# XiaokunSun/SemanticHuman

Measured on AMD Instinct MI355X. Metric: training meshes/sec at 6890 verts, batch=64, higher is better.
Workload: dtype f32

## Files before the change

### include/sh_kernels.h

```cpp
#ifndef SH_KERNELS_H
#define SH_KERNELS_H

#include <stddef.h>
#include <stdint.h>

#ifdef __cplusplus
extern "C" {
#endif

typedef void* sh_stream_t;

#if defined(__GNUC__)
#define SH_API __attribute__((visibility("default")))
#else
#define SH_API
#endif

enum sh_status {
    SH_OK = 0,
    SH_ERR_INVALID_ARG = -1,
    SH_ERR_UNSUPPORTED = -2,
    SH_ERR_WORKSPACE = -3,
    SH_ERR_LAUNCH = -4
};

enum sh_act {
    SH_ACT_IDENTITY = 0,
    SH_ACT_RELU = 1,
    SH_ACT_ELU = 2,
    SH_ACT_LEAKY_RELU = 3,
    SH_ACT_SIGMOID = 4,
    SH_ACT_TANH = 5
};

SH_API int sh_version(void);
SH_API const char* sh_last_error(void);
SH_API const char* sh_build_id(void);

enum sh_mma_mode { SH_MMA_EXACT = 0, SH_MMA_SPLIT3 = 1, SH_MMA_PLANES3 = 2 };

SH_API int sh_clock_probe(unsigned long long* out, int n_workgroups, int iters, sh_stream_t stream);
SH_API int sh_profile_enable(int on);
SH_API int sh_profile_count(void);
SH_API int sh_profile_get(int i, char* name, int name_len, float* ms);

SH_API int sh_spiral_conv_fwd(const float* x, int64_t x_sv, int64_t x_sb,
                       const int32_t* table, const float* weight, const float* bias,
                       float* y, int64_t y_sv, int64_t y_sb,
                       int B, int R, int S, int Cin, int Cout, int act, int zero_row, int mma_mode,
                       sh_stream_t stream);

SH_API int sh_spiral_conv_bwd_data(const float* dpre, int64_t dp_sv, int64_t dp_sb,
                            const int32_t* table_t, const float* weight_t,
                            float* dx, int64_t dx_sv, int64_t dx_sb,
                            const float* yprev, int64_t yp_sv, int64_t yp_sb, int act_prev, int zero_row,
                            int B, int n_in, int S, int Cin, int Cout, int mma_mode,
                            sh_stream_t stream);
SH_API int sh_spiral_conv_bwd_data_z(const float* dpre, int64_t dp_sv, int64_t dp_sb, int dpre_zero_row, const int32_t* table_t,
                                     const float* weight_t, float* dx, int64_t dx_sv, int64_t dx_sb, const float* yprev,
                                     int64_t yp_sv, int64_t yp_sb, int act_prev, int zero_row, int B, int n_in, int S, int Cin,
                                     int Cout, int mma_mode, sh_stream_t stream);

SH_API int sh_weight_transpose(const float* weight, float* weight_t, int S, int Cin, int Cout, sh_stream_t stream);

SH_API size_t sh_spiral_conv_bwd_wgt_workspace(int B, int R, int S, int Cin, int Cout);
SH_API int sh_spiral_conv_bwd_wgt(const float* dpre, int64_t dp_sv, int64_t dp_sb,
                           const float* x, int64_t x_sv, int64_t x_sb, const int32_t* table,
                           float* dW, float* dbias, void* workspace, size_t workspace_bytes,
                           int B, int R, int S, int Cin, int Cout, int mma_mode,
                           sh_stream_t stream);

SH_API int sh_spiral_conv_bwd_wgt_presum(const float* dpre, int64_t dp_sv, int64_t dp_sb, const float* x, int64_t x_sv, int64_t x_sb,
                                         const int32_t* table, float* dW, float* dbias, void* workspace, size_t workspace_bytes,
                                         const int32_t* sum_rowptr, const int32_t* sum_col, const float* sum_val, float* sum_out,
                                         void* sum_out_planes, int sum_rows, int B, int R, int S, int Cin, int Cout, int mma_mode,
                                         sh_stream_t stream);

SH_API int sh_spiral_conv_bwd_wgt_reduce_multi(int n_layers, const void* const* workspaces, float* const* dW,
                                        float* const* dbias, const int* B, const int* R, const int* S,
                                        const int* Cin, const int* Cout, sh_stream_t stream);
SH_API int sh_weight_transpose_multi(int n_layers, const float* const* weight, float* const* weight_t,
                              const int* S, const int* Cin, const int* Cout, sh_stream_t stream);

SH_API int sh_act_backward(const float* dy, int64_t dy_sv, int64_t dy_sb,
                    const float* y, int64_t y_sv, int64_t y_sb,
                    float* dpre, int64_t dp_sv, int64_t dp_sb,
                    int B, int R, int C, int act, int zero_row, sh_stream_t stream);
SH_API int sh_act_backward_tr(const float* dy, int64_t dy_sv, int64_t dy_sb, const float* y, int64_t y_sv, int64_t y_sb,
                       float* dpre, int64_t dp_sv, int64_t dp_sb, int B, int R, int C, int act, int zero_row, int n_layers,
                       const float* const* weight, float* const* weight_t, const int* S, const int* Cin, const int* Cout,
                       sh_stream_t stream);

SH_API int sh_spmm(const int32_t* rowptr, const int32_t* col, const float* val,
            const float* x, int64_t x_sv, int64_t x_sb,
            float* y, int64_t y_sv, int64_t y_sb,
            const float* yprev, int64_t yp_sv, int64_t yp_sb, int act_prev, int zero_row,
            int B, int rows, int C, sh_stream_t stream);

typedef struct sh_csr_ref { const int32_t* rowptr; const int32_t* col; const float* val; } sh_csr_ref;
typedef struct sh_stack_step {
    int kind;
    int param;
    const int32_t* table;
    const int32_t* table_t;
    int R, S, n_in, cin, cout, act, zero_row;
    int n1, n2;
    sh_csr_ref sum1, sum2;
    sh_csr_ref m, mt;
    int m_rows, m_cols;
    int extend;
    const int32_t* rag_rows;
    const int32_t* rag_pos;
    int rag_L;
    const int32_t* fg_rows; const uint32_t* fg_pos; const int32_t* fg_out; int fg_n, fg_L;
    const int32_t* bg_rows; const uint32_t* bg_pos; const int32_t* bg_out; int bg_n, bg_L;
} sh_stack_step;

enum sh_stack_form {
    SH_FORM_FWD_P3 = 1,
    SH_FORM_FWD_GRP = 2,
    SH_FORM_FWD_IMG = 4,
    SH_FORM_FWD_IMG_ONLY = 8,
    SH_FORM_BWD_GIMG = 16,
    SH_FORM_BWD_THIN = 32,
    SH_FORM_BWD_P3 = 64,
    SH_FORM_BWD_RAG = 128,
    SH_FORM_BWD_GRP = 256,
    SH_FORM_BWD_RIDE = 512,
    SH_FORM_BWD_PRESUM_IMG = 1024,
    SH_FORM_BWD_P3W = 2048,
    SH_FORM_BWD_YIMG = 4096,
    SH_FORM_BWD_IN_IMG_ONLY = 8192,
    SH_FORM_BWD_GRAD_IMG_ONLY = 16384
};
SH_API int sh_stack_plan_f32(int n_steps, const sh_stack_step* steps, int c0, int B, int x_layout, int mma_mode, int keep_fp32,
                             int need_x_grad, int* forms);

SH_API int sh_stack_forward(int n_steps, const sh_stack_step* steps, const float* x, int x_layout, int rows0, int c0, int B,
                            const float* const* weights, const float* const* biases, float* const* outs, int out_layout,
                            int mma_mode, void* const* planes, const void* const* wfrag3, int keep_fp32, sh_stream_t stream);

SH_API int sh_stack_backward(int n_steps, const sh_stack_step* steps, const float* x, int x_layout, int rows0, int c0, int B,
                             const float* const* acts, const float* g, int out_layout, const float* const* weights,
                             float* const* gin, float* dpre_last, float* const* weight_t, void* const* workspace,
                             const size_t* workspace_bytes, float* const* dW, float* const* dbias, int need_x_grad,
                             int mma_mode, void* const* gin_planes, void* dpre_last_planes, const void* const* wfrag3_t,
                             const void* const* in_planes, int acts_fp32, sh_stream_t stream);

SH_API size_t sh_linear_workspace(int M, int N, int K);
SH_API int sh_linear_fwd(const float* x, const float* weight, const float* bias, float* y, int M, int N, int K,
                  void* workspace, size_t workspace_bytes, int mma_mode, sh_stream_t stream);
SH_API int sh_linear_bwd_data(const float* dy, const float* weight, float* dx, int M, int N, int K,
                       void* workspace, size_t workspace_bytes, int mma_mode, sh_stream_t stream);
SH_API int sh_linear_bwd_wgt(const float* dy, const float* x, float* dW, float* dbias, int M, int N, int K,
                      void* workspace, size_t workspace_bytes, int mma_mode, sh_stream_t stream);
SH_API int sh_linear_bwd_wgt_adam_ok(int M, int N, int K);
SH_API int sh_linear_bwd_wgt_adam(const void* dy, int dy_dtype, const void* x, int x_dtype, float* weight, void* weight_bf16, float* exp_avg,
                           float* exp_avg_sq, const float* step, const float* lr, double beta1, double beta2, double eps,
                           double weight_decay, float* dbias, int M, int N, int K, int mma_mode, sh_stream_t stream);

SH_API int sh_grouped_linear_fwd(int G, const float* x, int64_t x_rs, const int64_t* x_off, const float* const* w,
                          const float* const* bias, float* y, int64_t y_rs, const int64_t* y_off, int M,
                          const int* N, const int* K, sh_stream_t stream);
SH_API int sh_grouped_linear_bwd_data(int G, const float* dy, int64_t y_rs, const int64_t* y_off, const float* const* w,
                               float* dx, int64_t x_rs, const int64_t* x_off, int M, const int* N, const int* K,
                               sh_stream_t stream);
SH_API int sh_grouped_linear_bwd_wgt(int G, const float* dy, int64_t y_rs, const int64_t* y_off, const float* x,
                              int64_t x_rs, const int64_t* x_off, float* const* dW, float* const* dbias, int M,
                              const int* N, const int* K, sh_stream_t stream);

SH_API size_t sh_reduce_workspace(void);

SH_API int sh_l1_loss_fwd(const float* a, const float* b, int64_t n, float* loss, void* workspace, sh_stream_t stream);
SH_API int sh_l1_loss_bwd(const float* a, const float* b, int64_t n, const float* gscale, float* grad_b, sh_stream_t stream);

SH_API int sh_vertex_l2(const float* a, const float* b, int B, int N1, int N, float scale, float* out,
                 void* workspace, sh_stream_t stream);

SH_API int sh_edge_ratio_loss_fwd(const float* x_hat, const float* x, const int32_t* faces, int B, int N1, int F,
                           float* loss, void* workspace, sh_stream_t stream);
SH_API int sh_edge_ratio_loss_bwd(const float* x_hat, const float* x, const int32_t* faces,
                           const int32_t* vptr, const int32_t* vcorner, int B, int N1, int F,
                           const float* gscale, float* grad, sh_stream_t stream);

SH_API size_t sh_recon_loss_workspace(void);
SH_API int sh_recon_loss_fwd(const float* x_hat, const float* x, const int32_t* faces, int B, int N1, int F, float edge_w,
                      float* total, float* parts, void* workspace, sh_stream_t stream);
SH_API int sh_recon_loss_bwd(const float* x_hat, const float* x, const int32_t* vptr, const int32_t* vnbr, int B, int N1, int F,
                      float edge_w, const float* gscale, float* grad, sh_stream_t stream);

SH_API int sh_part_pairdist_tile_rows(void);
SH_API int sh_part_pairdist_loss_fwd(const float* x_rec, const float* x_gt, const float* bone, const float* scale,
                              const int32_t* part_ptr, const int32_t* part_vert, const int32_t* tile_ptr,
                              const int32_t* flags, const float* w_part, int B, int N1, int P, int T, int max_part,
                              int w_mode, float w_threshold, int relat, float* loss, float* part_sum, float* part_cnt,
                              void* workspace, size_t workspace_bytes, sh_stream_t stream);
SH_API int sh_part_pairdist_loss_bwd(const float* x_rec, const float* x_gt, const float* bone, const float* scale,
                              const int32_t* part_ptr, const int32_t* part_vert, const int32_t* tile_ptr,
                              const int32_t* flags, const float* w_part, int B, int N1, int P, int T, int max_part,
                              int w_mode, float w_threshold, int relat, const float* part_cnt, const float* gscale,
                              float* grad, sh_stream_t stream);
SH_API int sh_part_pairdist_loss_fwd_grad(const float* x_rec, const float* x_gt, const float* bone, const float* scale,
                                   const int32_t* part_ptr, const int32_t* part_vert, const int32_t* tile_ptr, const int32_t* flags,
                                   const float* w_part, int B, int N1, int P, int T, int max_part, int w_mode, float w_threshold,
                                   int relat, float* loss, float* part_sum, float* part_cnt, float* grad_raw, void* workspace,
                                   size_t workspace_bytes, sh_stream_t stream);
SH_API int sh_part_pairdist_loss_bwd_scale(const float* grad_raw, const int32_t* part_ptr, const int32_t* part_vert,
                                   const float* w_part, const float* part_cnt, const float* gscale, int B, int N1, int P,
                                   int n_part_verts, float* grad, sh_stream_t stream);

SH_API int sh_measure_girth(const float* v, int64_t v_sb, const int32_t* ring_ptr, const int32_t* ring_a,
                     const int32_t* ring_b, const float* ring_f, int B, int P, float* girth, sh_stream_t stream);
SH_API int sh_bone_length(const float* kps, const int32_t* bones, int B, int K, int P, float* length, sh_stream_t stream);
SH_API int sh_measure_girth_bwd(const float* v, int64_t v_sb, const int32_t* ring_ptr, const int32_t* ring_a, const int32_t* ring_b,
                                const float* ring_f, const int32_t* pt_ring, const int32_t* vt_ptr, const int32_t* vt_pt,
                                const float* vt_w, int n_vt, const float* g_girth, int B, int P, int rows, float* g_v, sh_stream_t stream);
SH_API int sh_bone_length_bwd(const float* kps, const int32_t* bones, const int32_t* jt_ptr, const int32_t* jt_bone, const float* jt_w,
                              int n_jt, const float* g_len, int B, int K, int P, float* g_kps, sh_stream_t stream);
SH_API int sh_joint_regress_bwd(const float* g_kps, const float* J, int B, int N, int K, int rows, float* g_x, sh_stream_t stream);

SH_API int sh_nearest_points_chunks(int B, int nq, int nt);
SH_API size_t sh_nearest_points_workspace(int B, int nq, int nt, int chunks);
SH_API int sh_nearest_points(const float* q, int64_t q_sb, int nq, const int32_t* q_count, const float* t, int64_t t_sb, int nt,
                             const int32_t* t_count, const uint8_t* t_mask, int64_t mask_sb, int B, int chunks, int32_t* idx,
                             float* d2, void* workspace, size_t workspace_bytes, sh_stream_t stream);
SH_API int sh_chamfer_fwd(const float* d2_sm, int M, const int32_t* s_count, const float* d2_ms, int rows, int n,
                          const uint8_t* v_mask, int64_t mask_sb, float tau2, float w_ms, int B, float* loss, int32_t* counts,
                          sh_stream_t stream);
SH_API int sh_chamfer_bwd(const float* x, int64_t x_sb, int rows, int n, const float* s, int64_t s_sb, int M, const int32_t* s_count,
                          const int32_t* idx_sm, const float* d2_sm, const int32_t* idx_ms, const float* d2_ms, const uint8_t* v_mask,
                          int64_t mask_sb, const int32_t* counts, float tau2, float w_ms, const float* gL, int B, float* g_x,
                          sh_stream_t stream);

#define SH_SURFACE_MARGIN (1.0f + 0x1p-10f)
SH_API int sh_nearest_surface_chunks(int B, int nq, int nF);
SH_API size_t sh_nearest_surface_workspace(int B, int nq, int nF, int chunks);
SH_API int sh_nearest_surface(const float* q, int64_t q_sb, int nq, const int32_t* q_count, const float* x, int64_t x_sb, int n,
                              const int32_t* faces, int nF, const uint8_t* v_mask, int64_t mask_sb, const float* bound, int B,
                              int chunks, int cull, int32_t* face, float* d2, float* uv, uint64_t* stats, void* workspace,
                              size_t workspace_bytes, sh_stream_t stream);
SH_API int sh_chamfer_surface_bwd(const float* x, int64_t x_sb, int rows, int n, const float* s, int64_t s_sb, int M,
                                  const int32_t* s_count, const int32_t* faces, int nF, const int32_t* face, const float* d2,
                                  const float* uv, const int32_t* idx_ms, const float* d2_ms, const uint8_t* v_mask, int64_t mask_sb,
                                  const int32_t* counts, float tau2, float w_ms, const float* gL, int B, float* g_x,
                                  sh_stream_t stream);

SH_API int sh_vertex_normals(const float* x, int64_t x_sb, int n, const int32_t* faces, int nF, const int32_t* vf_ptr,
                             const int32_t* vf_idx, int B, float* normals, sh_stream_t stream);
SH_API int sh_nearest_points_gated(const float* q, int64_t q_sb, int nq, const int32_t* q_count, const float* qn, int64_t qn_sb,
                                   const float* t, int64_t t_sb, int nt, const int32_t* t_count, const float* tn, int64_t tn_sb,
                                   const uint8_t* t_mask, int64_t mask_sb, float cos_min, int B, int chunks, int32_t* idx, float* d2,
                                   void* workspace, size_t workspace_bytes, sh_stream_t stream);

SH_API int sh_face_normals(const float* x, int64_t x_sb, int n, const int32_t* faces, int nF, int B, float* normals,
                           sh_stream_t stream);
SH_API size_t sh_nearest_surface_gated_workspace(int B, int nq, int nF, int chunks);
SH_API int sh_nearest_surface_gated(const float* q, int64_t q_sb, int nq, const int32_t* q_count, const float* qn, int64_t qn_sb,
                                    const float* x, int64_t x_sb, int n, const int32_t* faces, int nF, const float* fn,
                                    const uint8_t* v_mask, int64_t mask_sb, float cos_min, const float* bound, int B, int chunks,
                                    int cull, int32_t* face, float* d2, float* uv, uint64_t* stats, void* workspace,
                                    size_t workspace_bytes, sh_stream_t stream);

#define SH_CLOUD_K_MIN 3
#define SH_CLOUD_K_MAX 64
#define SH_CLOUD_JACOBI_SWEEPS 8
#define SH_CLOUD_RANK_MIN 1e-12
SH_API int sh_cloud_normals(const float* s, int64_t s_sb, int M, const int32_t* count, int B, int k, const float* view,
                            int64_t view_sb, int64_t view_ps, float* nrm, float* var, float* r2, int32_t* cnt, void* workspace,
                            size_t workspace_bytes, sh_stream_t stream);

SH_API size_t sh_vertex_visibility_workspace(int B, int n, int nF, int chunks);
SH_API int sh_vertex_visibility(const float* x, int64_t x_sb, int n, const int32_t* faces, int nF, const float* tn, const float* view,
                                float cos_g, const uint8_t* mask, int64_t mask_sb, int B, int chunks, void* workspace,
                                size_t workspace_bytes, uint8_t* vis, sh_stream_t stream);

enum sh_align_mode { SH_ALIGN_TRANSLATION = 0, SH_ALIGN_RIGID = 1, SH_ALIGN_SIMILARITY = 2 };
#define SH_ALIGN_RANGE 2048
#define SH_ALIGN_PARTIAL 19
#define SH_ALIGN_MOMENTS 20
#define SH_ALIGN_JACOBI_SWEEPS 12
SH_API int sh_align_ranges(int M, int n, float w_ms);
SH_API size_t sh_align_partials_bytes(int B, int M, int n, float w_ms);
SH_API int sh_align_moments(const float* s, int64_t s_sb, int M, const int32_t* s_count, const float* x, int64_t x_sb, int rows, int n,
                            const uint8_t* v_mask, int64_t mask_sb, const int32_t* idx_sm, const float* d2_sm, const int32_t* idx_ms,
                            const float* d2_ms, float tau2, float w_ms, int B, double* partials, size_t partials_bytes,
                            sh_stream_t stream);
SH_API int sh_align_moments_surface(const float* s, int64_t s_sb, int M, const int32_t* s_count, const float* x, int64_t x_sb, int rows,
                                    int n, const uint8_t* v_mask, int64_t mask_sb, const int32_t* faces, int nF, const int32_t* face,
                                    const float* uv, const float* d2, const int32_t* idx_ms, const float* d2_ms, float tau2, float w_ms,
                                    int B, double* partials, size_t partials_bytes, sh_stream_t stream);
SH_API int sh_align_solve(const double* partials, int M, int n, const int32_t* s_count, float w_ms, int mode, int B,
                          const float* pose_in, const float* scale_in, float* pose_out, float* scale_out, float* inc, double* mom,
                          sh_stream_t stream);
SH_API int sh_transform_points(const float* src, int64_t src_sb, int M, const int32_t* count, const float* pose, int B, float* dst,
                               sh_stream_t stream);
#define SH_ALIGN_PLANE_PARTIAL 38
#define SH_ALIGN_PLANE_SYSTEM 37
#define SH_ALIGN_PLANE_PIVOT_MIN 1e-12
SH_API size_t sh_align_plane_partials_bytes(int B, int M, int n, float w_ms);
SH_API int sh_align_plane_moments(const float* s, int64_t s_sb, int M, const int32_t* s_count, const float* x, int64_t x_sb, int rows,
                                  int n, const uint8_t* v_mask, int64_t mask_sb, const float* tn, const int32_t* idx_sm,
                                  const float* d2_sm, const int32_t* idx_ms, const float* d2_ms, float tau2, float w_ms, int B,
                                  double* partials, size_t partials_bytes, sh_stream_t stream);
SH_API int sh_align_plane_moments_surface(const float* s, int64_t s_sb, int M, const int32_t* s_count, const float* x, int64_t x_sb,
                                          int rows, int n, const uint8_t* v_mask, int64_t mask_sb, const float* tn,
                                          const int32_t* faces, int nF, const int32_t* face, const float* uv, const float* d2,
                                          const int32_t* idx_ms, const float* d2_ms, float tau2, float w_ms, int B, double* partials,
                                          size_t partials_bytes, sh_stream_t stream);
SH_API int sh_align_plane_solve(const double* partials, int M, int n, const int32_t* s_count, float w_ms, int mode, int B,
                                const float* pose_in, const float* scale_in, float* pose_out, float* scale_out, double* sys,
                                int32_t* solved, sh_stream_t stream);

enum sh_robust { SH_ROBUST_NONE = 0, SH_ROBUST_GEMAN_MCCLURE = 1, SH_ROBUST_HUBER = 2 };
SH_API int sh_chamfer_fwd_robust(const float* d2_sm, int M, const int32_t* s_count, const float* d2_ms, int rows, int n,
                                 const uint8_t* v_mask, int64_t mask_sb, float tau2, float w_ms, int B, float* loss, int32_t* counts,
                                 sh_stream_t stream, int robust, float scale2);
SH_API int sh_chamfer_bwd_robust(const float* x, int64_t x_sb, int rows, int n, const float* s, int64_t s_sb, int M,
                                 const int32_t* s_count, const int32_t* idx_sm, const float* d2_sm, const int32_t* idx_ms,
                                 const float* d2_ms, const uint8_t* v_mask, int64_t mask_sb, const int32_t* counts, float tau2,
                                 float w_ms, const float* gL, int B, float* g_x, sh_stream_t stream, int robust, float scale2);
SH_API int sh_chamfer_surface_bwd_robust(const float* x, int64_t x_sb, int rows, int n, const float* s, int64_t s_sb, int M,
                                         const int32_t* s_count, const int32_t* faces, int nF, const int32_t* face, const float* d2,
                                         const float* uv, const int32_t* idx_ms, const float* d2_ms, const uint8_t* v_mask,
                                         int64_t mask_sb, const int32_t* counts, float tau2, float w_ms, const float* gL, int B,
                                         float* g_x, sh_stream_t stream, int robust, float scale2);
SH_API int sh_align_moments_robust(const float* s, int64_t s_sb, int M, const int32_t* s_count, const float* x, int64_t x_sb, int rows,
                                   int n, const uint8_t* v_mask, int64_t mask_sb, const int32_t* idx_sm, const float* d2_sm,
                                   const int32_t* idx_ms, const float* d2_ms, float tau2, float w_ms, int B, double* partials,
                                   size_t partials_bytes, sh_stream_t stream, int robust, float scale2);
SH_API int sh_align_moments_surface_robust(const float* s, int64_t s_sb, int M, const int32_t* s_count, const float* x, int64_t x_sb,
                                           int rows, int n, const uint8_t* v_mask, int64_t mask_sb, const int32_t* faces, int nF,
                                           const int32_t* face, const float* uv, const float* d2, const int32_t* idx_ms,
                                           const float* d2_ms, float tau2, float w_ms, int B, double* partials, size_t partials_bytes,
                                           sh_stream_t stream, int robust, float scale2);
SH_API int sh_align_plane_moments_robust(const float* s, int64_t s_sb, int M, const int32_t* s_count, const float* x, int64_t x_sb,
                                         int rows, int n, const uint8_t* v_mask, int64_t mask_sb, const float* tn, const int32_t* idx_sm,
                                         const float* d2_sm, const int32_t* idx_ms, const float* d2_ms, float tau2, float w_ms, int B,
                                         double* partials, size_t partials_bytes, sh_stream_t stream, int robust, float scale2);
SH_API int sh_align_plane_moments_surface_robust(const float* s, int64_t s_sb, int M, const int32_t* s_count, const float* x,
                                                 int64_t x_sb, int rows, int n, const uint8_t* v_mask, int64_t mask_sb, const float* tn,
                                                 const int32_t* faces, int nF, const int32_t* face, const float* uv, const float* d2,
                                                 const int32_t* idx_ms, const float* d2_ms, float tau2, float w_ms, int B,
                                                 double* partials, size_t partials_bytes, sh_stream_t stream, int robust,
                                                 float scale2);

enum sh_norm_flags {
    SH_NORM_ZEROMEAN = 1, SH_NORM_ZEROROOT = 2, SH_NORM_ONELENGTH = 4, SH_NORM_SMALL = 8, SH_NORM_GASS = 16, SH_NORM_NORMAL = 32
};
SH_API int sh_dataset_normalize(const float* raw, float* out, int n, int N, int dummy_rows, unsigned flags,
                         const float* j_root, const float* mean, const float* stdv, const float* center,
                         const float* scale, sh_stream_t stream);
SH_API int sh_gather_meshes(const float* src, int64_t row_elems, const int64_t* idx, int b, float* out, sh_stream_t stream);

SH_API int sh_adam_step(int n_tensors, float* const* params, const float* const* grads, float* const* exp_avg,
                 float* const* exp_avg_sq, float* const* steps, const int64_t* numel, const float* lr,
                 double beta1, double beta2, double eps, double weight_decay, sh_stream_t stream);
SH_API int sh_adam_bump(int n_tensors, float* const* steps, sh_stream_t stream);

SH_API int sh_joint_regress(const float* x, int64_t x_bs, const float* J, int B, int N, int K, float* kps, sh_stream_t stream);
SH_API int sh_joint_l1_loss_fwd(const float* x, int64_t x_bs, const float* J, const int32_t* keep, const float* target, int B,
                                int N, int K, int Kk, float* kps, float* loss, sh_stream_t stream);
SH_API int sh_joint_l1_loss_bwd(const float* kps, const int32_t* keep, const float* target, const float* J, int B, int N1, int N,
                                int K, int Kk, const float* gscale, float* grad, sh_stream_t stream);
SH_API int sh_part_volume_loss_fwd(const float* x_rec, const float* x_gt, int64_t x_bs, const int32_t* faces,
                                   const int32_t* pf_ptr, const int32_t* pf, int B, int P, float* vol, float* loss,
                                   sh_stream_t stream);
SH_API int sh_part_volume_loss_bwd(const float* x_rec, int64_t x_bs, const int32_t* faces, const int32_t* face_slot,
                                   const int32_t* vptr, const int32_t* vcorner, const float* vol, int B, int P, int N1,
                                   const float* gscale, float* grad, sh_stream_t stream);
SH_API int sh_zpart_reg(const float* z, const float* measure, const int32_t* part_idx, const int32_t* measure_idx, int B, int P,
                        int L, int M, int n, int relat, float* loss, float* dz, const float* gscale, sh_stream_t stream);
SH_API int sh_kps2skl(const float* kps, int B, int J, const int32_t* i0, const int32_t* i1, const int32_t* i2, int n_bones, int mode,
                      float* out, sh_stream_t stream);
SH_API int sh_skl2kps(const float* skl, int B, int n_bones, int mode, const int32_t* head, const int32_t* tail, int n_joints,
                      const int32_t* keep, int n_keep, float* out, sh_stream_t stream);
SH_API int sh_weighted_sum(int n, const float* const* terms, const float* weights, float* out, const float* gscale, float* grads,
                           sh_stream_t stream);

enum sh_dtype { SH_DTYPE_F32 = 0, SH_DTYPE_BF16 = 1 };

SH_API size_t sh_conv_wfrag_bytes(int S, int Cg, int Nout);
SH_API int sh_conv_wfrag_prep_multi(int n_layers, const float* const* weight, void* const* wfrag, const int* S,
                                    const int* Cin, const int* Cout, const int* transpose, sh_stream_t stream);

SH_API int sh_spiral_conv_fwd_bf16(const void* x, int x_dtype, int64_t x_sv, int64_t x_sb, const int32_t* table,
                                   const void* wfrag, const float* bias, void* y, int y_dtype, int64_t y_sv, int64_t y_sb,
                                   int B, int R, int S, int Cin, int Cout, int act, int zero_row, sh_stream_t stream);
SH_API int sh_spiral_conv_bwd_data_bf16(const void* dpre, int dp_dtype, int64_t dp_sv, int64_t dp_sb,
                                        const int32_t* table_t, const void* wfrag_t, void* dx, int dx_dtype,
                                        int64_t dx_sv, int64_t dx_sb, const void* yprev, int64_t yp_sv, int64_t yp_sb,
                                        int act_prev, int zero_row, int B, int n_in, int S, int Cin, int Cout,
                                        sh_stream_t stream);

SH_API int sh_spiral_conv_bwd_wgt_thin_ok(int B, int n_in, int S, int Cin, int Cout, int path_dtype);
SH_API int sh_spiral_conv_bwd_wgt_thin(const float* dpre_ext, int64_t dp_sv, int64_t dp_sb, const void* x, int x_dtype, int64_t x_sv,
                                int64_t x_sb, const int32_t* table_t, void* workspace, size_t workspace_bytes,
                                const float* weight, void* dx, int64_t dx_sv, int64_t dx_sb, void* dx_planes, int act_prev,
                                int zero_prev, int B, int R, int n_in, int S, int Cin, int Cout, int path_dtype, sh_stream_t stream);

SH_API size_t sh_spiral_conv_bwd_wgt_workspace_bf16(int B, int R, int S, int Cin, int Cout);
SH_API int sh_spiral_conv_bwd_wgt_bf16(const void* dpre, int dp_dtype, int64_t dp_sv, int64_t dp_sb, const void* x, int x_dtype,
                                       int64_t x_sv, int64_t x_sb, const int32_t* table, void* workspace,
                                       size_t workspace_bytes, int B, int R, int S, int Cin, int Cout, sh_stream_t stream);
SH_API int sh_spiral_conv_bwd_wgt_reduce_multi_bf16(int n_layers, const void* const* workspaces, float* const* dW,
                                                    float* const* dbias, const int* B, const int* R, const int* S,
                                                    const int* Cin, const int* Cout, sh_stream_t stream);

SH_API size_t sh_linear_workspace_bf16(int M, int N, int K);
SH_API int sh_cast_f32_to_bf16(const float* src, void* dst, int64_t n, sh_stream_t stream);
SH_API int sh_linear_fwd_bf16(const void* x, int x_dtype, const void* weight_bf16, const float* bias, void* y, int y_dtype,
                              int M, int N, int K, void* workspace, size_t workspace_bytes, sh_stream_t stream);
SH_API int sh_linear_bwd_data_bf16(const void* dy, int dy_dtype, const void* weight_bf16, void* dx, int dx_dtype, int M, int N,
                                   int K, void* workspace, size_t workspace_bytes, sh_stream_t stream);
SH_API int sh_linear_bwd_wgt_bf16(const void* dy, int dy_dtype, const void* x, int x_dtype, float* dW, float* dbias, int M,
                                  int N, int K, sh_stream_t stream);

SH_API int sh_spmm_bf16(const int32_t* rowptr, const int32_t* col, const float* val, const void* x, int64_t x_sv, int64_t x_sb,
                        void* y, int64_t y_sv, int64_t y_sb, const void* yprev, int64_t yp_sv, int64_t yp_sb, int act_prev,
                        int zero_row, int B, int rows, int C, sh_stream_t stream);
SH_API int sh_act_backward_bf16(const void* dy, int64_t dy_sv, int64_t dy_sb, const void* y, int64_t y_sv, int64_t y_sb,
                                void* dpre, int64_t dp_sv, int64_t dp_sb, int B, int R, int C, int act, int zero_row,
                                sh_stream_t stream);

SH_API int sh_adam_step_bf16(int n_tensors, float* const* params, const float* const* grads, float* const* exp_avg,
                             float* const* exp_avg_sq, float* const* steps, void* const* shadow_bf16, const int64_t* numel,
                             const float* lr, double beta1, double beta2, double eps, double weight_decay, sh_stream_t stream);

SH_API int sh_stack_forward_bf16(int n_steps, const sh_stack_step* steps, const void* x, int x_dtype, int x_layout, int rows0,
                                 int c0, int B, const float* const* weights, const float* const* biases, void* const* wfrag,
                                 int wfrag_ready, void* const* outs, int out_dtype, int out_layout, sh_stream_t stream);
SH_API int sh_stack_backward_bf16(int n_steps, const sh_stack_step* steps, const void* x, int x_dtype, int x_layout, int rows0,
                                  int c0, int B, const void* const* acts, const void* g, int out_dtype, int out_layout,
                                  const float* const* weights, void* const* gin, int gx_dtype, void* dpre_last,
                                  void* const* wfrag_t, int wfrag_ready, void* const* workspace,
                                  const size_t* workspace_bytes, float* const* dW, float* const* dbias, int need_x_grad,
                                  sh_stream_t stream);

SH_API size_t sh_p3_bytes(int rows, int B, int C);
SH_API int sh_to_p3(const float* x, int64_t x_sv, int64_t x_sb, void* planes, int B, int rows, int C, sh_stream_t stream);
SH_API size_t sh_conv_wfrag3_bytes(int S, int Cg, int Nout);
SH_API int sh_conv_wfrag3_prep_multi(int n_layers, const float* const* weight, void* const* wfrag3, const int* S, const int* Cin,
                                     const int* Cout, const int* transpose, sh_stream_t stream);
SH_API int sh_spiral_conv_p3_ok(int B, int S, int Cg, int Nout);
SH_API int sh_spiral_conv_p3_kind(int B, int S, int Cg, int Nout);
SH_API int64_t sh_p3_launch_count(void);
SH_API int sh_spmm_p3(const int32_t* rowptr, const int32_t* col, const float* val, const float* x, int64_t x_sv, int64_t x_sb,
                      float* y, int64_t y_sv, int64_t y_sb, void* y_planes, const float* yprev, int64_t yp_sv, int64_t yp_sb,
                      int act_prev, int zero_row, int B, int rows, int C, sh_stream_t stream);
SH_API int sh_spiral_conv_fwd_img(const float* x, int64_t x_sv, int64_t x_sb, const int32_t* table, const float* weight,
                                  const float* bias, float* y, int64_t y_sv, int64_t y_sb, void* y_planes, int B, int R, int S, int Cin,
                                  int Cout, int act, int zero_row, int mma_mode, sh_stream_t stream);
SH_API int sh_act_backward_tr_img(const float* dy, int64_t dy_sv, int64_t dy_sb, const float* y, int64_t y_sv, int64_t y_sb, float* dpre,
                                  int64_t dp_sv, int64_t dp_sb, void* dpre_planes, int B, int R, int C, int act, int zero_row, int n_layers,
                                  const float* const* weight, float* const* weight_t, const int* S, const int* Cin, const int* Cout,
                                  sh_stream_t stream);
SH_API int sh_spiral_conv_fwd_p3(const void* xp, const int32_t* table, const void* wfrag3, const float* bias, float* y, int64_t y_sv,
                                 int64_t y_sb, void* yp, int B, int R, int S, int Cin, int Cout, int act, int zero_row,
                                 sh_stream_t stream);
SH_API int sh_spiral_conv_bwd_data_p3(const void* dprep, int dpre_zero_row, const float* dpre_f32, int64_t dp_sv, int64_t dp_sb,
                                      int n_image_rows, const int32_t* table_t, const void* wfrag3_t, float* dx, int64_t dx_sv,
                                      int64_t dx_sb, void* dxp, const float* yprev, int64_t yp_sv, int64_t yp_sb,
                                      const void* yprev_planes, int act_prev, int zero_row, int B, int n_in, int S, int Cin, int Cout,
                                      sh_stream_t stream);

SH_API int sh_spiral_conv_p3_rag_ok(int B, int S, int Cg, int Nout, int rag_L);
SH_API int sh_spiral_conv_bwd_data_p3_rag(const void* dprep, const int32_t* rag_rows, const int32_t* rag_pos, int rag_L, const void* wfrag3_t,
                                          float* dx, int64_t dx_sv, int64_t dx_sb, void* dxp, const float* yprev, int64_t yp_sv,
                                          int64_t yp_sb, const void* yprev_planes, int act_prev, int zero_row, int B, int n_in, int S,
                                          int Cin, int Cout, sh_stream_t stream);

SH_API int sh_spiral_conv_p3_grp_ok(int B, int S, int Cg, int Nout, int g_L);
SH_API int sh_spiral_conv_p3_grp_members(int B, int S, int Cg, int Nout);
SH_API int sh_spiral_conv_p3_grp_pays(int B, int n_groups);
SH_API int sh_spiral_conv_p3_grp(const void* xp, const int32_t* g_rows, const uint32_t* g_pos, const int32_t* g_out, int n_groups, int g_L,
                                 const void* wfrag3, const float* bias, float* y, int64_t y_sv, int64_t y_sb, void* yp, const float* yprev,
                                 int64_t yp_sv, int64_t yp_sb, const void* yprev_planes, int act, int zero_row, int backward, int B, int R,
                                 int S, int Cg, int Nout, sh_stream_t stream);

SH_API int sh_spiral_conv_bf16_rag_ok(int B, int S, int Cg, int Nout, int rag_L);
SH_API int sh_spiral_conv_bwd_data_bf16_rag(const void* dpre, int64_t dp_sv, int64_t dp_sb, const int32_t* rag_rows, const int32_t* rag_pos,
                                            int rag_L, const void* wfrag_t, void* dx, int64_t dx_sv, int64_t dx_sb, const void* yprev,
                                            int64_t yp_sv, int64_t yp_sb, int act_prev, int zero_row, int B, int n_in, int S, int Cin,
                                            int Cout, sh_stream_t stream);

SH_API int sh_spiral_conv_bwd_wgt_p3_ok(int B, int R, int S, int Cin, int Cout);
SH_API size_t sh_spiral_conv_bwd_wgt_p3_workspace(int B, int R, int S, int Cin, int Cout);
SH_API int sh_spiral_conv_bwd_wgt_p3(const void* dpre_planes, int dpre_zero_row, const void* x_planes, const int32_t* table, void* workspace,
                                     size_t workspace_bytes, int B, int R, int S, int Cin, int Cout, sh_stream_t stream);
SH_API int sh_spiral_conv_bwd_wgt_p3_presum(const void* dpre_planes, int dpre_zero_row, const void* x_planes, const int32_t* table,
                                            void* workspace, size_t workspace_bytes, const float* dpre, int64_t dp_sv, int64_t dp_sb,
                                            const int32_t* sum_rowptr, const int32_t* sum_col, const float* sum_val, float* sum_out,
                                            void* sum_out_planes, int sum_rows, int B, int R, int S, int Cin, int Cout,
                                            sh_stream_t stream);
SH_API int sh_spiral_conv_bwd_wgt_reduce_multi_kinds(int n_layers, const void* const* workspaces, float* const* dW, float* const* dbias,
                                                     const int* B, const int* R, const int* S, const int* Cin, const int* Cout,
                                                     const int* kinds, sh_stream_t stream);

#ifdef __cplusplus
}
#endif
#endif
```

### semantichuman_amd/_lib.py

```python
from __future__ import annotations

import ctypes
import os
from ctypes import c_char_p, c_float, c_int, c_int64, c_size_t, c_void_p

_HERE = os.path.dirname(os.path.abspath(__file__))
LIB_PATH = os.environ.get("SH_KERNEL_LIB") or os.path.join(_HERE, "lib", "libsh_kernels.so")

ACT_IDS = {"identity": 0, "relu": 1, "elu": 2, "leaky_relu": 3, "sigmoid": 4, "tanh": 5}

_P, _I, _L = c_void_p, c_int, c_int64
SIGNATURES = {
    "sh_version": (c_int, []),
    "sh_last_error": (c_char_p, []),
    "sh_build_id": (c_char_p, []),
    "sh_clock_probe": (c_int, [_P, _I, _I, _P]),
    "sh_profile_enable": (c_int, [_I]),
    "sh_profile_count": (c_int, []),
    "sh_profile_get": (c_int, [_I, c_char_p, _I, ctypes.POINTER(c_float)]),
    "sh_spiral_conv_fwd": (c_int, [_P, _L, _L, _P, _P, _P, _P, _L, _L, _I, _I, _I, _I, _I, _I, _I, _I, _P]),
    "sh_spiral_conv_bwd_data": (c_int, [_P, _L, _L, _P, _P, _P, _L, _L, _P, _L, _L, _I, _I, _I, _I, _I, _I, _I, _I, _P]),
    "sh_spiral_conv_bwd_data_z": (c_int, [_P, _L, _L, _I, _P, _P, _P, _L, _L, _P, _L, _L, _I, _I, _I, _I, _I, _I, _I, _I, _P]),
    "sh_weight_transpose": (c_int, [_P, _P, _I, _I, _I, _P]),
    "sh_spiral_conv_bwd_wgt_workspace": (c_size_t, [_I, _I, _I, _I, _I]),
    "sh_spiral_conv_bwd_wgt": (c_int, [_P, _L, _L, _P, _L, _L, _P, _P, _P, _P, c_size_t, _I, _I, _I, _I, _I, _I, _P]),
    "sh_spiral_conv_bwd_wgt_presum": (c_int, [_P, _L, _L, _P, _L, _L, _P, _P, _P, _P, c_size_t, _P, _P, _P, _P, _P, _I, _I, _I, _I, _I, _I, _I, _P]),
    "sh_spiral_conv_bwd_wgt_reduce_multi": (c_int, [_I, _P, _P, _P, _P, _P, _P, _P, _P, _P]),
    "sh_weight_transpose_multi": (c_int, [_I, _P, _P, _P, _P, _P, _P]),
    "sh_act_backward": (c_int, [_P, _L, _L, _P, _L, _L, _P, _L, _L, _I, _I, _I, _I, _I, _P]),
    "sh_act_backward_tr": (c_int, [_P, _L, _L, _P, _L, _L, _P, _L, _L, _I, _I, _I, _I, _I, _I, _P, _P, _P, _P, _P, _P]),
    "sh_spmm": (c_int, [_P, _P, _P, _P, _L, _L, _P, _L, _L, _P, _L, _L, _I, _I, _I, _I, _I, _P]),
    "sh_stack_plan_f32": (c_int, [_I, _P, _I, _I, _I, _I, _I, _I, _P]),
    "sh_stack_forward": (c_int, [_I, _P, _P, _I, _I, _I, _I, _P, _P, _P, _I, _I, _P, _P, _I, _P]),
    "sh_stack_backward": (c_int, [_I, _P, _P, _I, _I, _I, _I, _P, _P, _I, _P, _P, _P, _P, _P, _P, _P, _P, _I, _I, _P, _P, _P, _P, _I, _P]),
    "sh_linear_workspace": (c_size_t, [_I, _I, _I]),
    "sh_linear_fwd": (c_int, [_P, _P, _P, _P, _I, _I, _I, _P, c_size_t, _I, _P]),
    "sh_linear_bwd_data": (c_int, [_P, _P, _P, _I, _I, _I, _P, c_size_t, _I, _P]),
    "sh_linear_bwd_wgt": (c_int, [_P, _P, _P, _P, _I, _I, _I, _P, c_size_t, _I, _P]),
    "sh_linear_bwd_wgt_adam_ok": (c_int, [_I, _I, _I]),
    "sh_linear_bwd_wgt_adam": (c_int, [_P, _I, _P, _I] + [_P] * 6 + [ctypes.c_double] * 4 + [_P, _I, _I, _I, _I, _P]),
    "sh_adam_bump": (c_int, [_I, _P, _P]),
    "sh_grouped_linear_fwd": (c_int, [_I, _P, _L, _P, _P, _P, _P, _L, _P, _I, _P, _P, _P]),
    "sh_grouped_linear_bwd_data": (c_int, [_I, _P, _L, _P, _P, _P, _L, _P, _I, _P, _P, _P]),
    "sh_grouped_linear_bwd_wgt": (c_int, [_I, _P, _L, _P, _P, _L, _P, _P, _P, _I, _P, _P, _P]),
    "sh_reduce_workspace": (c_size_t, []),
    "sh_l1_loss_fwd": (c_int, [_P, _P, _L, _P, _P, _P]),
    "sh_l1_loss_bwd": (c_int, [_P, _P, _L, _P, _P, _P]),
    "sh_vertex_l2": (c_int, [_P, _P, _I, _I, _I, c_float, _P, _P, _P]),
    "sh_edge_ratio_loss_fwd": (c_int, [_P, _P, _P, _I, _I, _I, _P, _P, _P]),
    "sh_edge_ratio_loss_bwd": (c_int, [_P, _P, _P, _P, _P, _I, _I, _I, _P, _P, _P]),
    "sh_spiral_conv_bwd_wgt_thin_ok": (c_int, [_I, _I, _I, _I, _I, _I]),
    "sh_spiral_conv_bwd_wgt_thin": (c_int, [_P, _L, _L, _P, _I, _L, _L, _P, _P, c_size_t, _P, _P, _L, _L, _P, _I, _I, _I, _I, _I, _I, _I, _I, _I, _P]),
    "sh_recon_loss_workspace": (c_size_t, []),
    "sh_recon_loss_fwd": (c_int, [_P, _P, _P, _I, _I, _I, c_float, _P, _P, _P, _P]),
    "sh_recon_loss_bwd": (c_int, [_P, _P, _P, _P, _I, _I, _I, c_float, _P, _P, _P]),
    "sh_part_pairdist_tile_rows": (c_int, []),
    "sh_part_pairdist_loss_fwd": (c_int, [_P] * 9 + [_I] * 6 + [c_float, _I, _P, _P, _P, _P, c_size_t, _P]),
    "sh_part_pairdist_loss_bwd": (c_int, [_P] * 9 + [_I] * 6 + [c_float, _I, _P, _P, _P, _P]),
    "sh_part_pairdist_loss_fwd_grad": (c_int, [_P] * 9 + [_I] * 6 + [c_float, _I, _P, _P, _P, _P, _P, c_size_t, _P]),
    "sh_part_pairdist_loss_bwd_scale": (c_int, [_P] * 6 + [_I] * 4 + [_P, _P]),
    "sh_measure_girth": (c_int, [_P, _L, _P, _P, _P, _P, _I, _I, _P, _P]),
    "sh_bone_length": (c_int, [_P, _P, _I, _I, _I, _P, _P]),
    "sh_measure_girth_bwd": (c_int, [_P, _L, _P, _P, _P, _P, _P, _P, _P, _P, _I, _P, _I, _I, _I, _P, _P]),
    "sh_bone_length_bwd": (c_int, [_P, _P, _P, _P, _P, _I, _P, _I, _I, _I, _P, _P]),
    "sh_joint_regress_bwd": (c_int, [_P, _P, _I, _I, _I, _I, _P, _P]),
    "sh_nearest_points_chunks": (c_int, [_I, _I, _I]),
    "sh_nearest_points_workspace": (c_size_t, [_I, _I, _I, _I]),
    "sh_nearest_points": (c_int, [_P, _L, _I, _P, _P, _L, _I, _P, _P, _L, _I, _I, _P, _P, _P, c_size_t, _P]),
    "sh_chamfer_fwd": (c_int, [_P, _I, _P, _P, _I, _I, _P, _L, c_float, c_float, _I, _P, _P, _P]),
    "sh_chamfer_bwd": (c_int, [_P, _L, _I, _I, _P, _L, _I, _P, _P, _P, _P, _P, _P, _L, _P, c_float, c_float, _P, _I, _P, _P]),
    "sh_nearest_surface_chunks": (c_int, [_I, _I, _I]),
    "sh_nearest_surface_workspace": (c_size_t, [_I, _I, _I, _I]),
    "sh_nearest_surface": (c_int, [_P, _L, _I, _P, _P, _L, _I, _P, _I, _P, _L, _P, _I, _I, _I, _P, _P, _P, _P, _P, c_size_t, _P]),
    "sh_chamfer_surface_bwd": (c_int, [_P, _L, _I, _I, _P, _L, _I, _P, _P, _I, _P, _P, _P, _P, _P, _P, _L, _P, c_float, c_float, _P, _I, _P, _P]),
    "sh_vertex_normals": (c_int, [_P, _L, _I, _P, _I, _P, _P, _I, _P, _P]),
    "sh_nearest_points_gated": (c_int, [_P, _L, _I, _P, _P, _L, _P, _L, _I, _P, _P, _L, _P, _L, c_float, _I, _I, _P, _P, _P, c_size_t, _P]),
    "sh_face_normals": (c_int, [_P, _L, _I, _P, _I, _I, _P, _P]),
    "sh_nearest_surface_gated_workspace": (c_size_t, [_I, _I, _I, _I]),
    "sh_nearest_surface_gated": (c_int, [_P, _L, _I, _P, _P, _L, _P, _L, _I, _P, _I, _P, _P, _L, c_float, _P, _I, _I, _I, _P, _P, _P, _P, _P,
                                         c_size_t, _P]),
    "sh_cloud_normals": (c_int, [_P, _L, _I, _P, _I, _I, _P, _L, _L, _P, _P, _P, _P, _P, c_size_t, _P]),
    "sh_vertex_visibility_workspace": (c_size_t, [_I, _I, _I, _I]),
    "sh_vertex_visibility": (c_int, [_P, _L, _I, _P, _I, _P, _P, c_float, _P, _L, _I, _I, _P, c_size_t, _P, _P]),
    "sh_align_ranges": (c_int, [_I, _I, c_float]),
    "sh_align_partials_bytes": (c_size_t, [_I, _I, _I, c_float]),
    "sh_align_moments": (c_int, [_P, _L, _I, _P, _P, _L, _I, _I, _P, _L, _P, _P, _P, _P, c_float, c_float, _I, _P, c_size_t, _P]),
    "sh_align_moments_surface": (c_int, [_P, _L, _I, _P, _P, _L, _I, _I, _P, _L, _P, _I, _P, _P, _P, _P, _P, c_float, c_float, _I, _P, c_size_t, _P]),
    "sh_align_solve": (c_int, [_P, _I, _I, _P, c_float, _I, _I, _P, _P, _P, _P, _P, _P, _P]),
    "sh_transform_points": (c_int, [_P, _L, _I, _P, _P, _I, _P, _P]),
    "sh_align_plane_partials_bytes": (c_size_t, [_I, _I, _I, c_float]),
    "sh_align_plane_moments": (c_int, [_P, _L, _I, _P, _P, _L, _I, _I, _P, _L, _P, _P, _P, _P, _P, c_float, c_float, _I, _P, c_size_t, _P]),
    "sh_align_plane_moments_surface": (c_int, [_P, _L, _I, _P, _P, _L, _I, _I, _P, _L, _P, _P, _I, _P, _P, _P, _P, _P, c_float, c_float, _I, _P,
                                               c_size_t, _P]),
    "sh_align_plane_solve": (c_int, [_P, _I, _I, _P, c_float, _I, _I, _P, _P, _P, _P, _P, _P, _P]),
    "sh_chamfer_fwd_robust": (c_int, [_P, _I, _P, _P, _I, _I, _P, _L, c_float, c_float, _I, _P, _P, _P, _I, c_float]),
    "sh_chamfer_bwd_robust": (c_int, [_P, _L, _I, _I, _P, _L, _I, _P, _P, _P, _P, _P, _P, _L, _P, c_float, c_float, _P, _I, _P, _P, _I, c_float]),
    "sh_chamfer_surface_bwd_robust": (c_int, [_P, _L, _I, _I, _P, _L, _I, _P, _P, _I, _P, _P, _P, _P, _P, _P, _L, _P, c_float, c_float, _P, _I, _P, _P,
                                              _I, c_float]),
    "sh_align_moments_robust": (c_int, [_P, _L, _I, _P, _P, _L, _I, _I, _P, _L, _P, _P, _P, _P, c_float, c_float, _I, _P, c_size_t, _P, _I, c_float]),
    "sh_align_moments_surface_robust": (c_int, [_P, _L, _I, _P, _P, _L, _I, _I, _P, _L, _P, _I, _P, _P, _P, _P, _P, c_float, c_float, _I, _P, c_size_t, _P,
                                                _I, c_float]),
    "sh_align_plane_moments_robust": (c_int, [_P, _L, _I, _P, _P, _L, _I, _I, _P, _L, _P, _P, _P, _P, _P, c_float, c_float, _I, _P, c_size_t, _P, _I,
                                              c_float]),
    "sh_align_plane_moments_surface_robust": (c_int, [_P, _L, _I, _P, _P, _L, _I, _I, _P, _L, _P, _P, _I, _P, _P, _P, _P, _P, c_float, c_float, _I, _P,
                                                      c_size_t, _P, _I, c_float]),
    "sh_dataset_normalize": (c_int, [_P, _P, _I, _I, _I, ctypes.c_uint, _P, _P, _P, _P, _P, _P]),
    "sh_gather_meshes": (c_int, [_P, _L, _P, _I, _P, _P]),
    "sh_adam_step": (c_int, [_I, _P, _P, _P, _P, _P, _P, _P] + [ctypes.c_double] * 4 + [_P]),
    "sh_joint_regress": (c_int, [_P, _L, _P, _I, _I, _I, _P, _P]),
    "sh_joint_l1_loss_fwd": (c_int, [_P, _L, _P, _P, _P, _I, _I, _I, _I, _P, _P, _P]),
    "sh_joint_l1_loss_bwd": (c_int, [_P, _P, _P, _P, _I, _I, _I, _I, _I, _P, _P, _P]),
    "sh_part_volume_loss_fwd": (c_int, [_P, _P, _L, _P, _P, _P, _I, _I, _P, _P, _P]),
    "sh_part_volume_loss_bwd": (c_int, [_P, _L, _P, _P, _P, _P, _P, _I, _I, _I, _P, _P, _P]),
    "sh_zpart_reg": (c_int, [_P, _P, _P, _P, _I, _I, _I, _I, _I, _I, _P, _P, _P, _P]),
    "sh_kps2skl": (c_int, [_P, _I, _I, _P, _P, _P, _I, _I, _P, _P]),
    "sh_skl2kps": (c_int, [_P, _I, _I, _I, _P, _P, _I, _P, _I, _P, _P]),
    "sh_weighted_sum": (c_int, [_I, _P, _P, _P, _P, _P, _P]),
    "sh_conv_wfrag_bytes": (c_size_t, [_I, _I, _I]),
    "sh_conv_wfrag_prep_multi": (c_int, [_I, _P, _P, _P, _P, _P, _P, _P]),
    "sh_spiral_conv_fwd_bf16": (c_int, [_P, _I, _L, _L, _P, _P, _P, _P, _I, _L, _L, _I, _I, _I, _I, _I, _I, _I, _P]),
    "sh_spiral_conv_bwd_data_bf16": (c_int, [_P, _I, _L, _L, _P, _P, _P, _I, _L, _L, _P, _L, _L, _I, _I, _I, _I, _I, _I, _I, _P]),
    "sh_spiral_conv_bwd_wgt_workspace_bf16": (c_size_t, [_I, _I, _I, _I, _I]),
    "sh_spiral_conv_bwd_wgt_bf16": (c_int, [_P, _I, _L, _L, _P, _I, _L, _L, _P, _P, c_size_t, _I, _I, _I, _I, _I, _P]),
    "sh_spiral_conv_bwd_wgt_reduce_multi_bf16": (c_int, [_I, _P, _P, _P, _P, _P, _P, _P, _P, _P]),
    "sh_linear_workspace_bf16": (c_size_t, [_I, _I, _I]),
    "sh_cast_f32_to_bf16": (c_int, [_P, _P, _L, _P]),
    "sh_linear_fwd_bf16": (c_int, [_P, _I, _P, _P, _P, _I, _I, _I, _I, _P, c_size_t, _P]),
    "sh_linear_bwd_data_bf16": (c_int, [_P, _I, _P, _P, _I, _I, _I, _I, _P, c_size_t, _P]),
    "sh_linear_bwd_wgt_bf16": (c_int, [_P, _I, _P, _I, _P, _P, _I, _I, _I, _P]),
    "sh_spmm_bf16": (c_int, [_P, _P, _P, _P, _L, _L, _P, _L, _L, _P, _L, _L, _I, _I, _I, _I, _I, _P]),
    "sh_act_backward_bf16": (c_int, [_P, _L, _L, _P, _L, _L, _P, _L, _L, _I, _I, _I, _I, _I, _P]),
    "sh_adam_step_bf16": (c_int, [_I, _P, _P, _P, _P, _P, _P, _P, _P] + [ctypes.c_double] * 4 + [_P]),
    "sh_stack_forward_bf16": (c_int, [_I, _P, _P, _I, _I, _I, _I, _I, _P, _P, _P, _I, _P, _I, _I, _P]),
    "sh_stack_backward_bf16": (c_int, [_I, _P, _P, _I, _I, _I, _I, _I, _P, _P, _I, _I, _P, _P, _I, _P, _P, _I, _P, _P, _P, _P, _I, _P]),
    "sh_p3_bytes": (c_size_t, [_I, _I, _I]),
    "sh_to_p3": (c_int, [_P, _L, _L, _P, _I, _I, _I, _P]),
    "sh_conv_wfrag3_bytes": (c_size_t, [_I, _I, _I]),
    "sh_conv_wfrag3_prep_multi": (c_int, [_I, _P, _P, _P, _P, _P, _P, _P]),
    "sh_spiral_conv_p3_ok": (c_int, [_I, _I, _I, _I]),
    "sh_spiral_conv_p3_kind": (c_int, [_I, _I, _I, _I]),
    "sh_p3_launch_count": (c_int64, []),
    "sh_spiral_conv_fwd_img": (c_int, [_P, _L, _L, _P, _P, _P, _P, _L, _L, _P, _I, _I, _I, _I, _I, _I, _I, _I, _P]),
    "sh_act_backward_tr_img": (c_int, [_P, _L, _L, _P, _L, _L, _P, _L, _L, _P, _I, _I, _I, _I, _I, _I, _P, _P, _P, _P, _P, _P]),
    "sh_spmm_p3": (c_int, [_P, _P, _P, _P, _L, _L, _P, _L, _L, _P, _P, _L, _L, _I, _I, _I, _I, _I, _P]),
    "sh_spiral_conv_fwd_p3": (c_int, [_P, _P, _P, _P, _P, _L, _L, _P, _I, _I, _I, _I, _I, _I, _I, _P]),
    "sh_spiral_conv_bwd_data_p3": (c_int, [_P, _I, _P, _L, _L, _I, _P, _P, _P, _L, _L, _P, _P, _L, _L, _P, _I, _I, _I, _I, _I, _I, _I, _P]),
    "sh_spiral_conv_p3_rag_ok": (c_int, [_I, _I, _I, _I, _I]),
    "sh_spiral_conv_bf16_rag_ok": (c_int, [_I, _I, _I, _I, _I]),
    "sh_spiral_conv_p3_grp_ok": (c_int, [_I, _I, _I, _I, _I]),
    "sh_spiral_conv_p3_grp_members": (c_int, [_I, _I, _I, _I]),
    "sh_spiral_conv_p3_grp_pays": (c_int, [_I, _I]),
    "sh_spiral_conv_p3_grp": (c_int, [_P, _P, _P, _P, _I, _I, _P, _P, _P, _L, _L, _P, _P, _L, _L, _P, _I, _I, _I, _I, _I, _I, _I, _I, _P]),
    "sh_spiral_conv_bwd_data_bf16_rag": (c_int, [_P, _L, _L, _P, _P, _I, _P, _P, _L, _L, _P, _L, _L, _I, _I, _I, _I, _I, _I, _I, _P]),
    "sh_spiral_conv_bwd_data_p3_rag": (c_int, [_P, _P, _P, _I, _P, _P, _L, _L, _P, _P, _L, _L, _P, _I, _I, _I, _I, _I, _I, _I, _P]),
    "sh_spiral_conv_bwd_wgt_p3_ok": (c_int, [_I, _I, _I, _I, _I]),
    "sh_spiral_conv_bwd_wgt_p3_workspace": (c_size_t, [_I, _I, _I, _I, _I]),
    "sh_spiral_conv_bwd_wgt_p3": (c_int, [_P, _I, _P, _P, _P, c_size_t, _I, _I, _I, _I, _I, _P]),
    "sh_spiral_conv_bwd_wgt_p3_presum": (c_int, [_P, _I, _P, _P, _P, c_size_t, _P, _L, _L, _P, _P, _P, _P, _P, _I, _I, _I, _I, _I, _I, _P]),
    "sh_spiral_conv_bwd_wgt_reduce_multi_kinds": (c_int, [_I, _P, _P, _P, _P, _P, _P, _P, _P, _P, _P]),
}
DTYPE_IDS = {"float32": 0, "bfloat16": 1}
FORM = {name: 1 << k for k, name in enumerate(["fwd_p3", "fwd_grp", "fwd_img", "fwd_img_only", "bwd_gimg", "bwd_thin", "bwd_p3", "bwd_rag",
                                                "bwd_grp", "bwd_ride", "bwd_presum_img", "bwd_p3w", "bwd_yimg", "bwd_in_img_only",
                                                "bwd_grad_img_only"])}



class CsrRef(ctypes.Structure):
    _fields_ = [("rowptr", c_void_p), ("col", c_void_p), ("val", c_void_p)]


class StackStep(ctypes.Structure):
    _fields_ = [("kind", c_int), ("param", c_int), ("table", c_void_p), ("table_t", c_void_p),
                ("R", c_int), ("S", c_int), ("n_in", c_int), ("cin", c_int), ("cout", c_int), ("act", c_int), ("zero_row", c_int),
                ("n1", c_int), ("n2", c_int), ("sum1", CsrRef), ("sum2", CsrRef), ("m", CsrRef), ("mt", CsrRef),
                ("m_rows", c_int), ("m_cols", c_int), ("extend", c_int),
                ("rag_rows", c_void_p), ("rag_pos", c_void_p), ("rag_L", c_int),
                ("fg_rows", c_void_p), ("fg_pos", c_void_p), ("fg_out", c_void_p), ("fg_n", c_int), ("fg_L", c_int),
                ("bg_rows", c_void_p), ("bg_pos", c_void_p), ("bg_out", c_void_p), ("bg_n", c_int), ("bg_L", c_int)]


_lib = None


class KernelLibraryError(RuntimeError):
    pass


def load(path: str | None = None):
    global _lib
    if _lib is not None and path is None:
        return _lib
    p = path or LIB_PATH
    if not os.path.exists(p):
        raise KernelLibraryError(
            "semantichuman_amd: HIP kernel library not found at %s. Build it with "
            "`python -c 'import __graft_entry__ as g; g.build()'` (or `make -C semantichuman_amd/csrc`). "
            "There is no CPU fallback." % p)
    try:
        lib = ctypes.CDLL(p)
    except OSError as e:
        raise KernelLibraryError("semantichuman_amd: cannot load %s: %s" % (p, e)) from e
    for name, (res, args) in SIGNATURES.items():
        try:
            fn = getattr(lib, name)
        except AttributeError as e:
            raise KernelLibraryError("semantichuman_amd: %s does not export %s" % (p, name)) from e
        fn.restype, fn.argtypes = res, args
    if path is None:
        _lib = lib
    return lib


def check(rc: int, what: str):
    if rc != 0:
        msg = load().sh_last_error()
        raise RuntimeError("%s failed (status %d): %s" % (what, rc, msg.decode() if msg else ""))


def stream_ptr():
    import torch
    return c_void_p(torch.cuda.current_stream().cuda_stream)


def profile_enable(on: bool):
    check(load().sh_profile_enable(1 if on else 0), "sh_profile_enable")


def profile_records():
    lib = load()
    out = []
    buf = ctypes.create_string_buffer(128)
    ms = c_float(0)
    for i in range(lib.sh_profile_count()):
        check(lib.sh_profile_get(i, buf, 128, ctypes.byref(ms)), "sh_profile_get")
        out.append((buf.value.decode(), ms.value))
    return out


def profile_records_by_kernel():
    return [(n.split("|")[0], n.split("|")[1] if "|" in n else "", ms) for n, ms in profile_records()]


def build_id() -> str:
    return load().sh_build_id().decode()


def env_overrides() -> dict:
    return {k: v for k, v in sorted(os.environ.items()) if k.startswith("SH_") and not k.startswith(("SH_BENCH_", "SH_KERNEL_LIB"))}


MMA_MODES = {"exact": 0, "split3": 1, "planes3": 2}


def _mma_default() -> str:
    v = os.environ.get("SH_F32_MMA", "exact").strip().lower()
    if v in MMA_MODES:
        return v
    return {"0": "exact", "1": "split3", "2": "planes3"}.get(v, "exact")


_mma_mode = _mma_default()


def set_f32_mma_mode(mode: str):
    global _mma_mode
    if mode not in MMA_MODES:
        raise ValueError("f32 mma mode must be one of %s" % sorted(MMA_MODES))
    _mma_mode = mode


def get_f32_mma_mode() -> str:
    return _mma_mode


def mma_id(mode: str | None = None) -> int:
    return MMA_MODES[_mma_mode if mode is None else mode]


def ptr(t):
    return c_void_p(0 if t is None else t.data_ptr())
```

### semantichuman_amd/csrc/p3_conv.hip

```cpp
#include "sh_bf16.h"

#include <atomic>
#include <type_traits>

namespace {

std::atomic<long> g_p3_launches{0};

struct P3Params {
    const char* xp; long x_vb, x_bgb;
    const int* table;
    const u32x4* wfrag;
    const float* bias;
    float* y; long y_sv, y_sb;
    char* yp; long yp_vb, yp_bgb;
    const float* yprev; long yv_sv, yv_sb;
    const char* yprev_img; long yvi_vb, yvi_bgb;
    const int* rag_rows; const int* rag_pos; int rag_L;
    const int* g_rows; const unsigned* g_pos; const int* g_out; int g_L, n_grp;
    int B, R, S, Cg, Nout, nks, nt_tot, ncg;
    int act, zero_row;
    int n_vg, n_tiles, nsplit;
    int skip_row;
    const float* xf; long xf_sv, xf_sb; int n_img;
};

#ifndef P3_BUDGET
#define P3_BUDGET 88
#endif
#ifndef P3_DCAP
#define P3_DCAP 4
#endif
constexpr int p3_depth(int NT, int RT) {
    const int d = (P3_BUDGET - NT * RT * 4 - 12) / (RT * 12);
    return d < 2 ? 2 : d > P3_DCAP ? P3_DCAP : d;
}

__device__ __forceinline__ f32x4 p3_quad_from_image(const char* img, long vb, long bgb, int v, int bs, int r16, int c0, int nch) {
    const bool o16 = nch == 16;
    const char* src = img + (long)v * vb + (long)bs * bgb +
                      (o16 ? ((c0 >> 3) * 16 + r16) * 16 : (c0 >> 5) * 3072 + (((c0 & 31) >> 3) * 16 + r16) * 16) + ((c0 >> 2) & 1) * 8;
    const int opb = o16 ? 512 : 1024;
    const u32x2 h = *reinterpret_cast<const u32x2*>(src), m = *reinterpret_cast<const u32x2*>(src + opb), l = *reinterpret_cast<const u32x2*>(src + 2 * opb);
    f32x4 y;
#pragma unroll
    for (int i = 0; i < 2; ++i) {
        y[2 * i] = (__builtin_bit_cast(float, h[i] << 16) + __builtin_bit_cast(float, m[i] << 16)) + __builtin_bit_cast(float, l[i] << 16);
        y[2 * i + 1] = (__builtin_bit_cast(float, h[i] & 0xFFFF0000u) + __builtin_bit_cast(float, m[i] & 0xFFFF0000u)) +
                       __builtin_bit_cast(float, l[i] & 0xFFFF0000u);
    }
    return y;
}

template <int J, int D, class F>
__device__ __forceinline__ bool p3_ring_steps(int ks, int nks, F&& f) {
    f(std::integral_constant<int, J>{}, ks + J);
    if constexpr (J + 1 < D) {
        if (ks + J + 1 >= nks) return false;
        return p3_ring_steps<J + 1, D>(ks, nks, f);
    } else {
        return true;
    }
}

#ifndef P3_WAVES_PER_EU
#define P3_WAVES_PER_EU 4
#endif
#ifndef P3_ABLATE
#define P3_ABLATE 0
#endif
template <int NT, int RT, bool C16, bool BWD, int NP, bool F32R = false>
__global__ __launch_bounds__(1024) __attribute__((amdgpu_waves_per_eu(P3_WAVES_PER_EU, 8))) void conv_p3_kernel(const P3Params p) {
    constexpr int D = p3_depth(NT, RT);
    extern __shared__ __attribute__((aligned(16))) char smem[];
    const u32x4* Wl = reinterpret_cast<const u32x4*>(smem);
    const int tid = threadIdx.x, lane = tid & 63, wave = tid >> 6, nw = blockDim.x >> 6;
    const int xcd = blockIdx.x & 7, li = blockIdx.x >> 3;
    const int nwg_x = ((int)gridDim.x - xcd + 7) >> 3;
    const int slice = li % p.nsplit, lj = li / p.nsplit;
    const int ngrp = nwg_x / p.nsplit;
    const int q8 = p.n_tiles >> 3, r8 = p.n_tiles & 7;
    const int t_begin = xcd < r8 ? xcd * (q8 + 1) : r8 * (q8 + 1) + (xcd - r8) * q8;
    const int t_end = t_begin + (xcd < r8 ? q8 + 1 : q8);
    const int stride = ngrp * nw;
    const int r16 = lane & 15, kq = lane >> 4;
    const int S = p.S, sl = lane < S ? lane : S - 1;
    const f32x4 zero4 = {0.f, 0.f, 0.f, 0.f};

    const unsigned rowmul = (unsigned)(p.x_vb >> 4);
    const int skip_key = F32R ? p.skip_row : (int)((unsigned)p.skip_row * rowmul);
    auto load_table = [&](int t, int (&tv)[RT]) {
        const int tt = t < t_end ? t : (t_end > 0 ? t_end - 1 : 0);
        const int vg = tt % p.n_vg;
#pragma unroll
        for (int m = 0; m < RT; ++m) {
            const int v = vg * RT + m < p.R ? vg * RT + m : p.R - 1;
            tv[m] = F32R ? p.table[(long)v * S + sl] : (int)((unsigned)p.table[(long)v * S + sl] * rowmul);
        }
    };

    int t = t_begin + lj * nw + wave;
    int tv[RT], tvn[RT];
    load_table(t, tv);
    {
        typedef __attribute__((address_space(3))) char* lptr_t;
        const unsigned wl_lds = __builtin_amdgcn_readfirstlane((unsigned)(uintptr_t)(lptr_t)smem);
        const int nfrag = p.nks * NT * 3;
        for (int f = __builtin_amdgcn_readfirstlane(wave); f < nfrag; f += nw) {
            const int pl = f % 3, n = (f / 3) % NT, ks = f / (3 * NT);
            const char* src = reinterpret_cast<const char*>(p.wfrag + (((long)ks * p.nt_tot + slice * NT + n) * 3 + pl) * 64 + lane);
            asm volatile("s_mov_b32 m0, %1\n\ts_nop 0\n\tglobal_load_lds_dwordx4 %0, off" : : "v"(src), "s"(__builtin_amdgcn_readfirstlane(wl_lds + (unsigned)f * 1024u)) : "memory", "m0");
        }
        asm volatile("s_waitcnt vmcnt(0)" ::: "memory");
    }
    __syncthreads();
    constexpr int PB = C16 ? 512 : 1024;
    for (; t < t_end; t += stride) {
        load_table(t + stride, tvn);
        const int bs = t / p.n_vg, vg = t - bs * p.n_vg;
        const int v0 = vg * RT;
        const char* xl = p.xp + (long)bs * p.x_bgb + (C16 ? ((kq & 1) * 16 + r16) * 16 : lane * 16);

        int ls = 0, lc = 0;
        u32x4 ring[D][RT][3];
        auto issue = [&](u32x4 (&a)[RT][3]) {
            if constexpr (!C16) {
                const int s = ls < S ? ls : S - 1;
#pragma unroll
                for (int m = 0; m < RT; ++m) {
                    const int row = __builtin_amdgcn_readlane(tv[m], s);
                    const bool f32row = F32R && row >= p.n_img;
                    const char* src = f32row ? reinterpret_cast<const char*>(p.xf + (long)row * p.xf_sv + (long)(bs * 16 + r16) * p.xf_sb + lc * 32 + kq * 8)
                                             : xl + (F32R ? (long)row * p.x_vb : (long)((unsigned long)(unsigned)row << 4)) + (long)lc * 3072;
                    const int o1 = f32row ? 16 : PB, o2 = f32row ? 0 : 2 * PB;
                    if constexpr (P3_ABLATE == 1) {
                        a[m][0] = a[m][1] = a[m][2] = (u32x4){(unsigned)row, (unsigned)lane, (unsigned)lc, 0x3f803f80u};
                    } else {
                    a[m][0] = *reinterpret_cast<const u32x4*>(src);
                    a[m][1] = *reinterpret_cast<const u32x4*>(src + o1);
                    a[m][2] = *reinterpret_cast<const u32x4*>(src + o2);
                    }
                }
                if (++lc >= p.ncg) { lc = 0; ++ls; }
            } else {
                const int s0 = ls < S ? ls : S - 1, s1 = ls + 1 < S ? ls + 1 : S - 1;
#pragma unroll
                for (int m = 0; m < RT; ++m) {
                    const int r0 = __builtin_amdgcn_readlane(tv[m], s0), r1 = __builtin_amdgcn_readlane(tv[m], s1);
                    const int row = (kq & 2) ? r1 : r0;
                    const bool f32row = F32R && row >= p.n_img;
                    const char* src = f32row ? reinterpret_cast<const char*>(p.xf + (long)row * p.xf_sv + (long)(bs * 16 + r16) * p.xf_sb + (kq & 1) * 8)
                                             : xl + (F32R ? (long)row * p.x_vb : (long)((unsigned long)(unsigned)row << 4));
                    const int o1 = f32row ? 16 : PB, o2 = f32row ? 0 : 2 * PB;
                    a[m][0] = *reinterpret_cast<const u32x4*>(src);
                    a[m][1] = *reinterpret_cast<const u32x4*>(src + o1);
                    a[m][2] = *reinterpret_cast<const u32x4*>(src + o2);
                }
                ls += 2;
            }
        };
        f32x4 acc[RT][NT];
#pragma unroll
        for (int m = 0; m < RT; ++m)
#pragma unroll
            for (int n = 0; n < NT; ++n) acc[m][n] = zero4;
        int cs = 0, cc = 0;
        auto compute = [&](int ks, u32x4 (&a)[RT][3]) {
            bool live[RT];
            bool any = false;
            const int cs_was = cs;
#pragma unroll
            for (int m = 0; m < RT; ++m) {
                live[m] = true;
                if constexpr (BWD) {
                    if (p.skip_row >= 0) {
                        if constexpr (!C16) {
                            live[m] = __builtin_amdgcn_readlane(tv[m], cs) != skip_key;
                        } else {
                            const int s1 = cs + 1 < S ? cs + 1 : cs;
                            live[m] = __builtin_amdgcn_readlane(tv[m], cs) != skip_key || __builtin_amdgcn_readlane(tv[m], s1) != skip_key;
                        }
                    }
                }
                any = any || live[m];
            }
            if constexpr (BWD) {
                if constexpr (C16) { cs += 2; if (cs >= S) cs = S - 1; }
                else if (++cc >= p.ncg) { cc = 0; if (cs + 1 < S) ++cs; }
            }
            if (!any) return;
#pragma unroll
            for (int m = 0; m < RT; ++m) {
                if constexpr (F32R) {
                    bool f32row;
                    if constexpr (!C16) {
                        f32row = __builtin_amdgcn_readlane(tv[m], cs_was) >= p.n_img;
                    } else {
                        const int s1 = cs_was + 1 < S ? cs_was + 1 : cs_was;
                        const int r0 = __builtin_amdgcn_readlane(tv[m], cs_was), r1 = __builtin_amdgcn_readlane(tv[m], s1);
                        f32row = ((kq & 2) ? r1 : r0) >= p.n_img;
                    }
                    if (__builtin_amdgcn_ballot_w64(f32row)) {
                        u32x4 h, mm, l;
                        sh_split3(*reinterpret_cast<const f32x4*>(&a[m][0]), *reinterpret_cast<const f32x4*>(&a[m][1]), h, mm, l);
                        if (f32row) { a[m][0] = h; a[m][1] = mm; a[m][2] = l; }
                    }
                }
            }
            if constexpr (P3_ABLATE == 2) {
#pragma unroll
                for (int m = 0; m < RT; ++m) acc[m][0][0] += __builtin_bit_cast(float, a[m][0][0] ^ a[m][1][1] ^ a[m][2][2]);
                return;
            }
            const u32x4* wk = Wl + ((long)ks * NT) * 192 + lane;
#pragma unroll
            for (int n = 0; n < NT; ++n) {
                u32x4 r0, r1, r2;
                if constexpr (P3_ABLATE == 4) {
                    r0 = (u32x4){(unsigned)lane, 0x3f803f80u, (unsigned)n, 1u}; r1 = r0; r2 = r0;
                } else {
                    r0 = wk[n * 192]; r1 = wk[n * 192 + 64]; r2 = wk[n * 192 + 128];
                }
                if constexpr (P3_ABLATE == 3) {
#pragma unroll
                    for (int m = 0; m < RT; ++m) acc[m][n][0] += __builtin_bit_cast(float, r0[0] ^ r1[1] ^ r2[2] ^ a[m][0][0] ^ a[m][1][1] ^ a[m][2][2]);
                    continue;
                }
                const bf16x8 wh = *reinterpret_cast<const bf16x8*>(&r0), wm = *reinterpret_cast<const bf16x8*>(&r1),
                             wl = *reinterpret_cast<const bf16x8*>(&r2);
#pragma unroll
                for (int m = 0; m < RT; ++m) {
                    if (RT > 1 && !live[m]) continue;
                    const bf16x8 xh = *reinterpret_cast<const bf16x8*>(&a[m][0]), xm = *reinterpret_cast<const bf16x8*>(&a[m][1]),
                                 xl2 = *reinterpret_cast<const bf16x8*>(&a[m][2]);
                    f32x4 c = acc[m][n];
                    if constexpr (NP == 9) {
                        c = __builtin_amdgcn_mfma_f32_16x16x32_bf16(wl, xl2, c, 0, 0, 0);
                        c = __builtin_amdgcn_mfma_f32_16x16x32_bf16(wl, xm, c, 0, 0, 0);
                        c = __builtin_amdgcn_mfma_f32_16x16x32_bf16(wm, xl2, c, 0, 0, 0);
                    }
                    c = __builtin_amdgcn_mfma_f32_16x16x32_bf16(wl, xh, c, 0, 0, 0);
                    c = __builtin_amdgcn_mfma_f32_16x16x32_bf16(wh, xl2, c, 0, 0, 0);
                    c = __builtin_amdgcn_mfma_f32_16x16x32_bf16(wm, xm, c, 0, 0, 0);
                    c = __builtin_amdgcn_mfma_f32_16x16x32_bf16(wm, xh, c, 0, 0, 0);
                    c = __builtin_amdgcn_mfma_f32_16x16x32_bf16(wh, xm, c, 0, 0, 0);
                    c = __builtin_amdgcn_mfma_f32_16x16x32_bf16(wh, xh, c, 0, 0, 0);
                    acc[m][n] = c;
                }
            }
        };

#pragma unroll
        for (int d = 0; d < D - 1; ++d) issue(ring[d]);
        auto step = [&](auto J, int ks) {
            constexpr int j = decltype(J)::value;
            issue(ring[(j + D - 1) % D]);
            __builtin_amdgcn_sched_barrier(0);
            compute(ks, ring[j]);
        };
        for (int ks = 0; ks < p.nks; ks += D)
            if (!p3_ring_steps<0, D>(ks, p.nks, step)) break;

        const int b = bs * 16 + r16;
#pragma unroll
        for (int m = 0; m < RT; ++m) {
            const int v = v0 + m;
            if (v >= p.R || b >= p.B) continue;
            const bool zero = v == p.zero_row;
#pragma unroll
            for (int n = 0; n < NT; ++n) {
                const int c0 = (slice * NT + n) * 16 + kq * 4;
                if (c0 >= p.Nout) continue;
                f32x4 a = acc[m][n];
                if (!BWD) {
                    if (p.bias) a += *reinterpret_cast<const f32x4*>(p.bias + c0);
                    a = sh_act_fwd4(a, p.act);
                } else if (p.yprev_img) {
                    const f32x4 yv = p3_quad_from_image(p.yprev_img, p.yvi_vb, p.yvi_bgb, v, bs, r16, c0, p.Nout);
#pragma unroll
                    for (int j = 0; j < 4; ++j) a[j] *= sh_act_grad_from_out(yv[j], p.act);
                } else if (p.yprev) {
                    const f32x4 yv = *reinterpret_cast<const f32x4*>(p.yprev + (long)v * p.yv_sv + (long)b * p.yv_sb + c0);
#pragma unroll
                    for (int j = 0; j < 4; ++j) a[j] *= sh_act_grad_from_out(yv[j], p.act);
                }
                if (zero) a = zero4;
                if (p.y) *reinterpret_cast<f32x4*>(p.y + (long)v * p.y_sv + (long)b * p.y_sb + c0) = a;
                if (p.yp) {
                    u32x2 h, mm, l;
                    sh_split3_quad(a, h, mm, l);
                    const bool o16 = p.Nout == 16;
                    char* dst = p.yp + (long)v * p.yp_vb + (long)bs * p.yp_bgb +
                                (o16 ? ((c0 >> 3) * 16 + r16) * 16 : (c0 >> 5) * 3072 + (((c0 & 31) >> 3) * 16 + r16) * 16) + (kq & 1) * 8;
                    const int opb = o16 ? 512 : 1024;
                    *reinterpret_cast<u32x2*>(dst) = h;
                    *reinterpret_cast<u32x2*>(dst + opb) = mm;
                    *reinterpret_cast<u32x2*>(dst + 2 * opb) = l;
                }
            }
        }
#pragma unroll
        for (int m = 0; m < RT; ++m) tv[m] = tvn[m];
    }
}

template <int NT, int NP>
__global__ __launch_bounds__(1024) __attribute__((amdgpu_waves_per_eu(P3_WAVES_PER_EU, 8))) void conv_p3r_kernel(const P3Params p) {
    constexpr int D = p3_depth(NT, 1);
    extern __shared__ __attribute__((aligned(16))) char smem[];
    const u32x4* Wl = reinterpret_cast<const u32x4*>(smem);
    const int tid = threadIdx.x, lane = tid & 63, wave = tid >> 6, nw = blockDim.x >> 6;
    const int xcd = blockIdx.x & 7, li = blockIdx.x >> 3;
    const int nwg_x = ((int)gridDim.x - xcd + 7) >> 3;
    const int slice = li % p.nsplit, lj = li / p.nsplit;
    const int ngrp = nwg_x / p.nsplit;
    const int q8 = p.n_tiles >> 3, r8 = p.n_tiles & 7;
    const int t_begin = xcd < r8 ? xcd * (q8 + 1) : r8 * (q8 + 1) + (xcd - r8) * q8;
    const int t_end = t_begin + (xcd < r8 ? q8 + 1 : q8);
    const int stride = ngrp * nw;
    const int r16 = lane & 15, kq = lane >> 4;
    const int Lp = p.rag_L, ll = lane < Lp ? lane : Lp - 1;
    const f32x4 zero4 = {0.f, 0.f, 0.f, 0.f};
    const unsigned rowmul = (unsigned)(p.x_vb >> 4);
    auto load_list = [&](int t, int& rows, int& pos) {
        const int tt = t < t_end ? t : (t_end > 0 ? t_end - 1 : 0);
        const int v = tt % p.n_vg;
        rows = (int)((unsigned)p.rag_rows[(long)v * Lp + ll] * rowmul);
        pos = lane < Lp ? p.rag_pos[(long)v * Lp + ll] : -1;
    };
    int t = t_begin + lj * nw + wave;
    int tv, tp, tvn, tpn;
    load_list(t, tv, tp);
    {
        typedef __attribute__((address_space(3))) char* lptr_t;
        const unsigned wl_lds = __builtin_amdgcn_readfirstlane((unsigned)(uintptr_t)(lptr_t)smem);
        const int nfrag = p.nks * NT * 3;
        for (int f = __builtin_amdgcn_readfirstlane(wave); f < nfrag; f += nw) {
            const int pl = f % 3, n = (f / 3) % NT, ks = f / (3 * NT);
            const char* src = reinterpret_cast<const char*>(p.wfrag + (((long)ks * p.nt_tot + slice * NT + n) * 3 + pl) * 64 + lane);
            asm volatile("s_mov_b32 m0, %1\n\ts_nop 0\n\tglobal_load_lds_dwordx4 %0, off" : : "v"(src), "s"(__builtin_amdgcn_readfirstlane(wl_lds + (unsigned)f * 1024u)) : "memory", "m0");
        }
        asm volatile("s_waitcnt vmcnt(0)" ::: "memory");
    }
    __syncthreads();
    for (; t < t_end; t += stride) {
        load_list(t + stride, tvn, tpn);
        const int bs = t / p.n_vg, v = t - bs * p.n_vg;
        const char* xl = p.xp + (long)bs * p.x_bgb + lane * 16;
        const int L = __builtin_popcountll(__builtin_amdgcn_ballot_w64(tp >= 0));
        const int nks = L * p.ncg;
        int lj2 = 0, lc = 0;
        u32x4 ring[D][3];
        auto issue = [&](u32x4 (&a)[3]) {
            const int j = lj2 < L ? lj2 : (L > 0 ? L - 1 : 0);
            const int row = __builtin_amdgcn_readlane(tv, j);
            const char* src = xl + (long)((unsigned long)(unsigned)row << 4) + (long)lc * 3072;
            a[0] = *reinterpret_cast<const u32x4*>(src);
            a[1] = *reinterpret_cast<const u32x4*>(src + 1024);
            a[2] = *reinterpret_cast<const u32x4*>(src + 2048);
            if (++lc >= p.ncg) { lc = 0; ++lj2; }
        };
        f32x4 acc[NT];
#pragma unroll
        for (int n = 0; n < NT; ++n) acc[n] = zero4;
        int cj = 0, cc = 0;
        auto compute = [&](u32x4 (&a)[3]) {
            const int s = __builtin_amdgcn_readlane(tp, cj);
            const u32x4* wk = Wl + ((long)(s * p.ncg + cc) * NT) * 192 + lane;
            if (++cc >= p.ncg) { cc = 0; ++cj; }
            const bf16x8 xh = *reinterpret_cast<const bf16x8*>(&a[0]), xm = *reinterpret_cast<const bf16x8*>(&a[1]),
                         xl2 = *reinterpret_cast<const bf16x8*>(&a[2]);
#pragma unroll
            for (int n = 0; n < NT; ++n) {
                const u32x4 r0 = wk[n * 192], r1 = wk[n * 192 + 64], r2 = wk[n * 192 + 128];
                const bf16x8 wh = *reinterpret_cast<const bf16x8*>(&r0), wm = *reinterpret_cast<const bf16x8*>(&r1),
                             wl = *reinterpret_cast<const bf16x8*>(&r2);
                f32x4 c = acc[n];
                if constexpr (NP == 9) {
                    c = __builtin_amdgcn_mfma_f32_16x16x32_bf16(wl, xl2, c, 0, 0, 0);
                    c = __builtin_amdgcn_mfma_f32_16x16x32_bf16(wl, xm, c, 0, 0, 0);
                    c = __builtin_amdgcn_mfma_f32_16x16x32_bf16(wm, xl2, c, 0, 0, 0);
                }
                c = __builtin_amdgcn_mfma_f32_16x16x32_bf16(wl, xh, c, 0, 0, 0);
                c = __builtin_amdgcn_mfma_f32_16x16x32_bf16(wh, xl2, c, 0, 0, 0);
                c = __builtin_amdgcn_mfma_f32_16x16x32_bf16(wm, xm, c, 0, 0, 0);
                c = __builtin_amdgcn_mfma_f32_16x16x32_bf16(wm, xh, c, 0, 0, 0);
                c = __builtin_amdgcn_mfma_f32_16x16x32_bf16(wh, xm, c, 0, 0, 0);
                c = __builtin_amdgcn_mfma_f32_16x16x32_bf16(wh, xh, c, 0, 0, 0);
                acc[n] = c;
            }
        };
#pragma unroll
        for (int d = 0; d < D - 1; ++d) issue(ring[d]);
        auto step = [&](auto J, int ks) {
            constexpr int j = decltype(J)::value;
            issue(ring[(j + D - 1) % D]);
            __builtin_amdgcn_sched_barrier(0);
            compute(ring[j]);
        };
        for (int ks = 0; ks < nks; ks += D)
            if (!p3_ring_steps<0, D>(ks, nks, step)) break;

        const int b = bs * 16 + r16;
        if (v < p.R && b < p.B) {
            const bool zero = v == p.zero_row;
#pragma unroll
            for (int n = 0; n < NT; ++n) {
                const int c0 = (slice * NT + n) * 16 + kq * 4;
                if (c0 >= p.Nout) continue;
                f32x4 a = acc[n];
                if (p.yprev_img) {
                    const f32x4 yv = p3_quad_from_image(p.yprev_img, p.yvi_vb, p.yvi_bgb, v, bs, r16, c0, p.Nout);
#pragma unroll
                    for (int j = 0; j < 4; ++j) a[j] *= sh_act_grad_from_out(yv[j], p.act);
                } else if (p.yprev) {
                    const f32x4 yv = *reinterpret_cast<const f32x4*>(p.yprev + (long)v * p.yv_sv + (long)b * p.yv_sb + c0);
#pragma unroll
                    for (int j = 0; j < 4; ++j) a[j] *= sh_act_grad_from_out(yv[j], p.act);
                }
                if (zero) a = zero4;
                if (p.y) *reinterpret_cast<f32x4*>(p.y + (long)v * p.y_sv + (long)b * p.y_sb + c0) = a;
                if (p.yp) {
                    u32x2 h, mm, l;
                    sh_split3_quad(a, h, mm, l);
                    const bool o16 = p.Nout == 16;
                    char* dst = p.yp + (long)v * p.yp_vb + (long)bs * p.yp_bgb +
                                (o16 ? ((c0 >> 3) * 16 + r16) * 16 : (c0 >> 5) * 3072 + (((c0 & 31) >> 3) * 16 + r16) * 16) + (kq & 1) * 8;
                    const int opb = o16 ? 512 : 1024;
                    *reinterpret_cast<u32x2*>(dst) = h;
                    *reinterpret_cast<u32x2*>(dst + opb) = mm;
                    *reinterpret_cast<u32x2*>(dst + 2 * opb) = l;
                }
            }
        }
        tv = tvn; tp = tpn;
    }
}

template <int NT, int G, bool BWD, int NP, bool C16 = false>
__global__ __launch_bounds__(1024) __attribute__((amdgpu_waves_per_eu(P3_WAVES_PER_EU, 8))) void conv_p3g_kernel(const P3Params p) {
    constexpr int D = p3_depth(NT * G, 1) < 3 ? 3 : p3_depth(NT * G, 1);
    constexpr int PB = C16 ? 512 : 1024;
    extern __shared__ __attribute__((aligned(16))) char smem[];
    const u32x4* Wl = reinterpret_cast<const u32x4*>(smem);
    const int tid = threadIdx.x, lane = tid & 63, wave = tid >> 6, nw = blockDim.x >> 6;
    const int xcd = blockIdx.x & 7, li = blockIdx.x >> 3;
    const int nwg_x = ((int)gridDim.x - xcd + 7) >> 3;
    const int slice = li % p.nsplit, lj = li / p.nsplit;
    const int ngrp = nwg_x / p.nsplit;
    const int q8 = p.n_tiles >> 3, r8 = p.n_tiles & 7;
    const int t_begin = xcd < r8 ? xcd * (q8 + 1) : r8 * (q8 + 1) + (xcd - r8) * q8;
    const int t_end = t_begin + (xcd < r8 ? q8 + 1 : q8);
    const int stride = ngrp * nw;
    const int r16 = lane & 15, kq = lane >> 4;
    const int Lp = p.g_L, ll = lane < Lp ? lane : Lp - 1;
    const f32x4 zero4 = {0.f, 0.f, 0.f, 0.f};
    const unsigned rowmul = (unsigned)(p.x_vb >> 4);
    auto load_list = [&](int t, int& rows, unsigned& pos) {
        const int tt = t < t_end ? t : (t_end > 0 ? t_end - 1 : 0);
        const int g = tt % p.n_vg;
        rows = (int)((unsigned)p.g_rows[(long)g * Lp + ll] * rowmul);
        pos = lane < Lp ? p.g_pos[(long)g * Lp + ll] : 0xFFFFFFFFu;
    };
    int t = t_begin + lj * nw + wave;
    int tv, tvn;
    unsigned tp, tpn;
    load_list(t, tv, tp);
    {
        typedef __attribute__((address_space(3))) char* lptr_t;
        const unsigned wl_lds = __builtin_amdgcn_readfirstlane((unsigned)(uintptr_t)(lptr_t)smem);
        const int nfrag = p.nks * NT * 3;
        for (int f = __builtin_amdgcn_readfirstlane(wave); f < nfrag; f += nw) {
            const int pl = f % 3, n = (f / 3) % NT, ks = f / (3 * NT);
            const char* src = reinterpret_cast<const char*>(p.wfrag + (((long)ks * p.nt_tot + slice * NT + n) * 3 + pl) * 64 + lane);
            asm volatile("s_mov_b32 m0, %1\n\ts_nop 0\n\tglobal_load_lds_dwordx4 %0, off" : : "v"(src), "s"(__builtin_amdgcn_readfirstlane(wl_lds + (unsigned)f * 1024u)) : "memory", "m0");
        }
        asm volatile("s_waitcnt vmcnt(0)" ::: "memory");
    }
    __syncthreads();
    for (; t < t_end; t += stride) {
        load_list(t + stride, tvn, tpn);
        const int bs = t / p.n_vg, grp = t - bs * p.n_vg;
        const char* xl = p.xp + (long)bs * p.x_bgb + (C16 ? ((kq & 1) * 16 + r16) * 16 : lane * 16);
        const int L = __builtin_popcountll(__builtin_amdgcn_ballot_w64(tp != 0xFFFFFFFFu));
        const int nks = C16 ? (L + 1) >> 1 : L * p.ncg;
        int lj2 = 0, lc = 0;
        u32x4 ring[D][3];
        auto issue = [&](u32x4 (&a)[3]) {
            const int j = lj2 < L ? lj2 : (L > 0 ? L - 1 : 0);
            int row = __builtin_amdgcn_readlane(tv, j);
            if constexpr (C16) {
                const int j1 = lj2 + 1 < L ? lj2 + 1 : j;
                const int row1 = __builtin_amdgcn_readlane(tv, j1);
                row = (kq & 2) ? row1 : row;
            }
            const char* src = xl + (long)((unsigned long)(unsigned)row << 4) + (C16 ? 0L : (long)lc * 3072);
            a[0] = *reinterpret_cast<const u32x4*>(src);
            a[1] = *reinterpret_cast<const u32x4*>(src + PB);
            a[2] = *reinterpret_cast<const u32x4*>(src + 2 * PB);
            if constexpr (C16) lj2 += 2;
            else if (++lc >= p.ncg) { lc = 0; ++lj2; }
        };
        f32x4 acc[G][NT];
#pragma unroll
        for (int g = 0; g < G; ++g)
#pragma unroll
            for (int n = 0; n < NT; ++n) acc[g][n] = zero4;
        int cj = 0, cc = 0;
        auto compute = [&](u32x4 (&a)[3]) {
            const unsigned pk = (unsigned)__builtin_amdgcn_readlane((int)tp, cj);
            unsigned pk1 = 0xFFFFFFFFu;
            const int ccw = cc;
            if constexpr (C16) {
                if (cj + 1 < L) pk1 = (unsigned)__builtin_amdgcn_readlane((int)tp, cj + 1);
                cj += 2;
            } else if (++cc >= p.ncg) { cc = 0; ++cj; }
            bf16x8 xh = *reinterpret_cast<const bf16x8*>(&a[0]), xm = *reinterpret_cast<const bf16x8*>(&a[1]),
                   xl2 = *reinterpret_cast<const bf16x8*>(&a[2]);
#pragma unroll
            for (int g = 0; g < G; ++g) {
                const int s = (int)((pk >> (8 * g)) & 0xFFu);
                const u32x4* wk;
                if constexpr (C16) {
                    const int s1 = (int)((pk1 >> (8 * g)) & 0xFFu);
                    if (s == 0xFF && s1 == 0xFF) continue;
                    const int q = (kq & 2) ? (s1 == 0xFF ? 0 : s1) : (s == 0xFF ? 0 : s);
                    wk = Wl + ((long)(q >> 1) * NT) * 192 + (r16 + 16 * (2 * (q & 1) + (kq & 1)));
                    if (s == 0xFF || s1 == 0xFF) {
                        const bool dead = (kq & 2) ? s1 == 0xFF : s == 0xFF;
                        const u32x4 z = {0u, 0u, 0u, 0u};
                        const u32x4 h4 = dead ? z : a[0], m4 = dead ? z : a[1], l4 = dead ? z : a[2];
                        xh = *reinterpret_cast<const bf16x8*>(&h4); xm = *reinterpret_cast<const bf16x8*>(&m4); xl2 = *reinterpret_cast<const bf16x8*>(&l4);
                    } else {
                        xh = *reinterpret_cast<const bf16x8*>(&a[0]); xm = *reinterpret_cast<const bf16x8*>(&a[1]); xl2 = *reinterpret_cast<const bf16x8*>(&a[2]);
                    }
                } else {
                    if (s == 0xFF) continue;
                    wk = Wl + ((long)(s * p.ncg + ccw) * NT) * 192 + lane;
                }
#pragma unroll
                for (int n = 0; n < NT; ++n) {
                    const u32x4 r0 = wk[n * 192], r1 = wk[n * 192 + 64], r2 = wk[n * 192 + 128];
                    const bf16x8 wh = *reinterpret_cast<const bf16x8*>(&r0), wm = *reinterpret_cast<const bf16x8*>(&r1),
                                 wl = *reinterpret_cast<const bf16x8*>(&r2);
                    f32x4 c = acc[g][n];
                    if constexpr (NP == 9) {
                        c = __builtin_amdgcn_mfma_f32_16x16x32_bf16(wl, xl2, c, 0, 0, 0);
                        c = __builtin_amdgcn_mfma_f32_16x16x32_bf16(wl, xm, c, 0, 0, 0);
                        c = __builtin_amdgcn_mfma_f32_16x16x32_bf16(wm, xl2, c, 0, 0, 0);
                    }
                    c = __builtin_amdgcn_mfma_f32_16x16x32_bf16(wl, xh, c, 0, 0, 0);
                    c = __builtin_amdgcn_mfma_f32_16x16x32_bf16(wh, xl2, c, 0, 0, 0);
                    c = __builtin_amdgcn_mfma_f32_16x16x32_bf16(wm, xm, c, 0, 0, 0);
                    c = __builtin_amdgcn_mfma_f32_16x16x32_bf16(wm, xh, c, 0, 0, 0);
                    c = __builtin_amdgcn_mfma_f32_16x16x32_bf16(wh, xm, c, 0, 0, 0);
                    c = __builtin_amdgcn_mfma_f32_16x16x32_bf16(wh, xh, c, 0, 0, 0);
                    acc[g][n] = c;
                }
            }
        };
#pragma unroll
        for (int d = 0; d < D - 1; ++d) issue(ring[d]);
        auto step = [&](auto J, int ks) {
            constexpr int j = decltype(J)::value;
            issue(ring[(j + D - 1) % D]);
            __builtin_amdgcn_sched_barrier(0);
            compute(ring[j]);
        };
        for (int ks = 0; ks < nks; ks += D)
            if (!p3_ring_steps<0, D>(ks, nks, step)) break;

        const int b = bs * 16 + r16;
#pragma unroll
        for (int g = 0; g < G; ++g) {
            const int v = p.g_out[(long)grp * 4 + g];
            if (v < 0 || v >= p.R || b >= p.B) continue;
            const bool zero = v == p.zero_row;
#pragma unroll
            for (int n = 0; n < NT; ++n) {
                const int c0 = (slice * NT + n) * 16 + kq * 4;
                if (c0 >= p.Nout) continue;
                f32x4 a = acc[g][n];
                if (!BWD) {
                    if (p.bias) a += *reinterpret_cast<const f32x4*>(p.bias + c0);
                    a = sh_act_fwd4(a, p.act);
                } else if (p.yprev_img) {
                    const f32x4 yv = p3_quad_from_image(p.yprev_img, p.yvi_vb, p.yvi_bgb, v, bs, r16, c0, p.Nout);
#pragma unroll
                    for (int j = 0; j < 4; ++j) a[j] *= sh_act_grad_from_out(yv[j], p.act);
                } else if (p.yprev) {
                    const f32x4 yv = *reinterpret_cast<const f32x4*>(p.yprev + (long)v * p.yv_sv + (long)b * p.yv_sb + c0);
#pragma unroll
                    for (int j = 0; j < 4; ++j) a[j] *= sh_act_grad_from_out(yv[j], p.act);
                }
                if (zero) a = zero4;
                if (p.y) *reinterpret_cast<f32x4*>(p.y + (long)v * p.y_sv + (long)b * p.y_sb + c0) = a;
                if (p.yp) {
                    u32x2 h, mm, l;
                    sh_split3_quad(a, h, mm, l);
                    const bool o16 = p.Nout == 16;
                    char* dst = p.yp + (long)v * p.yp_vb + (long)bs * p.yp_bgb +
                                (o16 ? ((c0 >> 3) * 16 + r16) * 16 : (c0 >> 5) * 3072 + (((c0 & 31) >> 3) * 16 + r16) * 16) + (kq & 1) * 8;
                    const int opb = o16 ? 512 : 1024;
                    *reinterpret_cast<u32x2*>(dst) = h;
                    *reinterpret_cast<u32x2*>(dst + opb) = mm;
                    *reinterpret_cast<u32x2*>(dst + 2 * opb) = l;
                }
            }
        }
        tv = tvn; tp = tpn;
    }
}

constexpr int P3S_NT = 4, P3S_KC = 4;

template <int RT, bool BWD, int NP, int NT = P3S_NT>
__global__ __launch_bounds__(1024 / RT) void conv_p3s_kernel(const P3Params p) {
    constexpr int D = P3S_KC, WAVES = 16 / RT, WF = P3S_KC * NT * 3 / WAVES;
    static_assert(WF * WAVES == P3S_KC * NT * 3, "a chunk's fragments must divide evenly over the waves");
    extern __shared__ __attribute__((aligned(16))) char smem[];
    u32x4* Wl = reinterpret_cast<u32x4*>(smem);
    constexpr int CHUNK_PIECES = P3S_KC * NT * 192;
    const int tid = threadIdx.x, lane = tid & 63, wave = tid >> 6;
    const int xcd = blockIdx.x & 7, li = blockIdx.x >> 3;
    const int nwg_x = ((int)gridDim.x - xcd + 7) >> 3;
    const int slice = li % p.nsplit, lj = li / p.nsplit;
    const int ngrp = nwg_x / p.nsplit;
    const int q8 = p.n_tiles >> 3, r8 = p.n_tiles & 7;
    const int t_begin = xcd < r8 ? xcd * (q8 + 1) : r8 * (q8 + 1) + (xcd - r8) * q8;
    const int t_end = t_begin + (xcd < r8 ? q8 + 1 : q8);
    const int stride = ngrp * WAVES;
    const int r16 = lane & 15, kq = lane >> 4;
    const int S = p.S, sl = lane < S ? lane : S - 1;
    const f32x4 zero4 = {0.f, 0.f, 0.f, 0.f};
    const int nch = p.nks / P3S_KC;
    int wsrc[WF], wdst[WF];
#pragma unroll
    for (int j = 0; j < WF; ++j) {
        const int f = WF * wave + j, pl = f % 3, n = (f / 3) % NT, kk = f / (3 * NT);
        wsrc[j] = ((kk * p.nt_tot + slice * NT + n) * 3 + pl) * 64 + lane;
        wdst[j] = f * 64 + lane;
    }
    const int wchunk = P3S_KC * p.nt_tot * 192;
    const unsigned rowmul = (unsigned)(p.x_vb >> 4);
    const int skip_key = (int)((unsigned)p.skip_row * rowmul);
    const int rounds = (t_end - t_begin - lj * WAVES + stride - 1) / stride;
    int t = t_begin + lj * WAVES + wave;
    for (int rd = 0; rd < rounds; ++rd, t += stride) {
        const bool live = t < t_end;
        const int tt = live ? t : t_end - 1;
        const int bs = tt / p.n_vg, vg = tt - bs * p.n_vg;
        const int v0 = vg * RT;
        int tv[RT];
#pragma unroll
        for (int m = 0; m < RT; ++m) tv[m] = (int)((unsigned)p.table[(long)(v0 + m < p.R ? v0 + m : p.R - 1) * S + sl] * rowmul);
        const char* xl = p.xp + (long)bs * p.x_bgb + lane * 16;
        int ls = 0, lc = 0;
        u32x4 ring[D][RT][3];
        auto issue = [&](u32x4 (&a)[RT][3]) {
            const int s = ls < S ? ls : S - 1;
#pragma unroll
            for (int m = 0; m < RT; ++m) {
                const int row = __builtin_amdgcn_readlane(tv[m], s);
                const bool f32row = false;
                const char* src = f32row ? reinterpret_cast<const char*>(p.xf + (long)row * p.xf_sv + (long)(bs * 16 + r16) * p.xf_sb + lc * 32 + kq * 8)
                                         : xl + (long)((unsigned long)(unsigned)row << 4) + (long)lc * 3072;
                const int o1 = f32row ? 16 : 1024, o2 = f32row ? 0 : 2048;
                a[m][0] = *reinterpret_cast<const u32x4*>(src);
                a[m][1] = *reinterpret_cast<const u32x4*>(src + o1);
                a[m][2] = *reinterpret_cast<const u32x4*>(src + o2);
            }
            if (++lc >= p.ncg) { lc = 0; ++ls; }
        };
        f32x4 acc[RT][NT];
#pragma unroll
        for (int m = 0; m < RT; ++m)
#pragma unroll
            for (int n = 0; n < NT; ++n) acc[m][n] = zero4;
        int cs = 0, cc = 0;
        auto compute = [&](const u32x4* wk, u32x4 (&a)[RT][3]) {
            bool live[RT];
            bool any = false;
#pragma unroll
            for (int m = 0; m < RT; ++m) {
                const int row = BWD ? __builtin_amdgcn_readlane(tv[m], cs) : 0;
                live[m] = !BWD || p.skip_row < 0 || row != skip_key;
                any = any || live[m];
            }
            if (BWD && ++cc >= p.ncg) { cc = 0; if (cs + 1 < S) ++cs; }
            if (!any) return;
            constexpr int PW[9] = {2, 2, 1, 2, 0, 1, 1, 0, 0}, PX[9] = {2, 1, 2, 0, 2, 1, 0, 1, 0};
#pragma unroll
            for (int n = 0; n < NT; ++n) {
                const u32x4 r0 = wk[n * 192], r1 = wk[n * 192 + 64], r2 = wk[n * 192 + 128];
                const bf16x8 w[3] = {*reinterpret_cast<const bf16x8*>(&r0), *reinterpret_cast<const bf16x8*>(&r1),
                                     *reinterpret_cast<const bf16x8*>(&r2)};
#pragma unroll
                for (int m = 0; m < RT; ++m) {
                    if (RT > 1 && !live[m]) continue;
                    f32x4 c = acc[m][n];
#pragma unroll
                    for (int q = 9 - NP; q < 9; ++q)
                        c = __builtin_amdgcn_mfma_f32_16x16x32_bf16(w[PW[q]], *reinterpret_cast<const bf16x8*>(&a[m][PX[q]]), c, 0, 0, 0);
                    acc[m][n] = c;
                }
            }
        };
        u32x4 wreg[WF];
#pragma unroll
        for (int j = 0; j < WF; ++j) wreg[j] = p.wfrag[wsrc[j]];
#pragma unroll
        for (int d = 0; d < D - 1; ++d) issue(ring[d]);
#pragma unroll
        for (int j = 0; j < WF; ++j) Wl[wdst[j]] = wreg[j];
        __syncthreads();
        for (int c = 0; c < nch; ++c) {
            const bool more = c + 1 < nch;
            if (more) {
#pragma unroll
                for (int j = 0; j < WF; ++j) wreg[j] = p.wfrag[wsrc[j] + (c + 1) * wchunk];
            }
            const u32x4* wb = Wl + (c & 1) * CHUNK_PIECES + lane;
            auto step = [&](auto J, int) {
                constexpr int j = decltype(J)::value;
                issue(ring[(j + D - 1) % D]);
                __builtin_amdgcn_sched_barrier(0);
                compute(wb + j * NT * 192, ring[j]);
            };
            p3_ring_steps<0, D>(0, D, step);
            if (more) {
                u32x4* wn = Wl + ((c + 1) & 1) * CHUNK_PIECES;
#pragma unroll
                for (int j = 0; j < WF; ++j) wn[wdst[j]] = wreg[j];
            }
            __syncthreads();
        }
        const int b = bs * 16 + r16;
#pragma unroll
        for (int m = 0; m < RT; ++m) {
            const int v = v0 + m;
            if (!live || v >= p.R || b >= p.B) continue;
            const bool zero = v == p.zero_row;
#pragma unroll
            for (int n = 0; n < NT; ++n) {
                const int c0 = (slice * NT + n) * 16 + kq * 4;
                if (c0 >= p.Nout) continue;
                f32x4 a = acc[m][n];
                if (!BWD) {
                    if (p.bias) a += *reinterpret_cast<const f32x4*>(p.bias + c0);
                    a = sh_act_fwd4(a, p.act);
                } else if (p.yprev_img) {
                    const f32x4 yv = p3_quad_from_image(p.yprev_img, p.yvi_vb, p.yvi_bgb, v, bs, r16, c0, p.Nout);
#pragma unroll
                    for (int j = 0; j < 4; ++j) a[j] *= sh_act_grad_from_out(yv[j], p.act);
                } else if (p.yprev) {
                    const f32x4 yv = *reinterpret_cast<const f32x4*>(p.yprev + (long)v * p.yv_sv + (long)b * p.yv_sb + c0);
#pragma unroll
                    for (int j = 0; j < 4; ++j) a[j] *= sh_act_grad_from_out(yv[j], p.act);
                }
                if (zero) a = zero4;
                if (p.y) *reinterpret_cast<f32x4*>(p.y + (long)v * p.y_sv + (long)b * p.y_sb + c0) = a;
                if (p.yp) {
                    u32x2 h, mm, l;
                    sh_split3_quad(a, h, mm, l);
                    const bool o16 = p.Nout == 16;
                    char* dst = p.yp + (long)v * p.yp_vb + (long)bs * p.yp_bgb +
                                (o16 ? ((c0 >> 3) * 16 + r16) * 16 : (c0 >> 5) * 3072 + (((c0 & 31) >> 3) * 16 + r16) * 16) + (kq & 1) * 8;
                    const int opb = o16 ? 512 : 1024;
                    *reinterpret_cast<u32x2*>(dst) = h;
                    *reinterpret_cast<u32x2*>(dst + opb) = mm;
                    *reinterpret_cast<u32x2*>(dst + 2 * opb) = l;
                }
            }
        }
    }
}

struct ToP3Args { const float* x; long sv, sb; char* out; int nbg, C; long total; };
__global__ __launch_bounds__(256) void to_p3_kernel(const ToP3Args a) {
    const long q = (long)blockIdx.x * 256 + threadIdx.x;
    if (q >= a.total) return;
    int l, kb, cbase; long blk; char* d; int pb;
    if (a.C == 16) {
        l = (int)(q & 31); blk = q >> 5; kb = l >> 4; cbase = kb * 8;
        d = a.out + blk * 1536 + l * 16; pb = 512;
    } else {
        l = (int)(q & 63); const long f = q >> 6; const int ncg = a.C >> 5;
        blk = f / ncg; const int cg = (int)(f - blk * ncg); kb = l >> 4; cbase = cg * 32 + kb * 8;
        d = a.out + f * 3072 + l * 16; pb = 1024;
    }
    const long v = blk / a.nbg; const int bg = (int)(blk - v * a.nbg), r = l & 15;
    const float* s = a.x + v * a.sv + (long)(bg * 16 + r) * a.sb + cbase;
    const f32x4 lo = *reinterpret_cast<const f32x4*>(s), hi = *reinterpret_cast<const f32x4*>(s + 4);
    u32x4 h, m, lw;
    sh_split3(lo, hi, h, m, lw);
    *reinterpret_cast<u32x4*>(d) = h;
    *reinterpret_cast<u32x4*>(d + pb) = m;
    *reinterpret_cast<u32x4*>(d + 2 * pb) = lw;
}

constexpr int WF3_MAX = 24;
struct WFrag3Args {
    const float* w[WF3_MAX]; u32x4* out[WF3_MAX];
    int S[WF3_MAX], Cin[WF3_MAX], Cout[WF3_MAX], tr[WF3_MAX], nks[WF3_MAX], nt_tot[WF3_MAX], block0[WF3_MAX + 1];
    int nd;
};
__global__ __launch_bounds__(256) void wfrag3_prep_kernel(const WFrag3Args a) {
    int d = 0;
    while (d + 1 < a.nd && a.block0[d + 1] <= (int)blockIdx.x) ++d;
    const long i = (long)((int)blockIdx.x - a.block0[d]) * 256 + threadIdx.x;
    const long total = (long)a.nks[d] * a.nt_tot[d] * 64;
    if (i >= total) return;
    const int lane = (int)(i & 63), f = (int)(i >> 6), nt = f % a.nt_tot[d], ks = f / a.nt_tot[d];
    const int S = a.S[d], Cin = a.Cin[d], Cout = a.Cout[d], tr = a.tr[d];
    const int Cg = tr ? Cout : Cin, Nout = tr ? Cin : Cout;
    const int row = nt * 16 + (lane & 15), k0 = 32 * ks + 8 * (lane >> 4);
    const float* w = a.w[d];
    float v[8];
#pragma unroll
    for (int j = 0; j < 8; ++j) {
        const int k = k0 + j;
        const int s = k / Cg, c = k - s * Cg;
        v[j] = 0.f;
        if (row < Nout && s < S) {
            const int co = tr ? c : row, ci = tr ? row : c;
            v[j] = w[(long)co * S * Cin + (long)s * Cin + ci];
        }
    }
    u32x4 h, m, l;
    sh_split3((f32x4){v[0], v[1], v[2], v[3]}, (f32x4){v[4], v[5], v[6], v[7]}, h, m, l);
    u32x4* o = a.out[d] + (long)f * 192 + lane;
    o[0] = h; o[64] = m; o[128] = l;
}

int p3_num_cus() {
    static int n = 0;
    if (!n) {
        int dev = 0;
        hipDeviceProp_t prop;
        if (hipGetDevice(&dev) == hipSuccess && hipGetDeviceProperties(&prop, dev) == hipSuccess) n = prop.multiProcessorCount;
        if (n <= 0) n = 256;
    }
    return n;
}

struct P3Geom { int nks, nt_tot, nt, nsplit; };
inline P3Geom p3_geom(int S, int Cg, int Nout) {
    const ShFragGeom g = sh_frag_geom(S, Cg, Nout);
    P3Geom r{g.nks, g.nt_tot, g.nt_tot > 8 ? 8 : g.nt_tot, 1};
    r.nsplit = g.nt_tot / r.nt;
    while (r.nt > 1 && (long)g.nks * r.nt * 3 > 150) { r.nt >>= 1; r.nsplit <<= 1; }
    return r;
}
inline bool p3s_shape_ok(int S, int Cg, int Nout) {
    static const int on = sh_env_int("SH_P3_STREAM", 1, 0, 1);
    static const int pad_on = sh_env_int("SH_P3S_PAD", 1, 0, 1), nt2_on = sh_env_int("SH_P3S_NT2", 1, 0, 1);
    if (!on || Cg % 32 || !(Nout % 64 == 0 || (nt2_on && Nout == 32))) return false;
    const ShFragGeom g = sh_frag_geom(S, Cg, Nout);
    return (pad_on || g.nks % P3S_KC == 0) && (Nout == 32 || g.nt_tot % P3S_NT == 0);
}
inline bool p3_resident_ok(int S, int Cg, int Nout) {
    const P3Geom g = p3_geom(S, Cg, Nout);
    static const int max_split = sh_env_int("SH_P3_MAX_SPLIT", 1, 1, 8);
    const bool built = Cg == 16 ? g.nt <= 2 : (g.nt == 1 || g.nt == 2 || g.nt == 4 || g.nt == 8);
    return (long)g.nks * g.nt * 3 <= 150 && g.nsplit <= max_split && built;
}
inline int p3_nks(int S, int Cg, int Nout) {
    const ShFragGeom g = sh_frag_geom(S, Cg, Nout);
    if (p3_resident_ok(S, Cg, Nout) || !p3s_shape_ok(S, Cg, Nout)) return g.nks;
    return (g.nks + P3S_KC - 1) / P3S_KC * P3S_KC;
}
inline bool p3_shape_ok(int B, int S, int Cg, int Nout) {
    if (B <= 0 || B % 16 || S <= 0 || S > 64 || Nout % 4) return false;
    if (!(Cg == 16 || (Cg > 0 && Cg % 32 == 0))) return false;
    return p3_resident_ok(S, Cg, Nout) || p3s_shape_ok(S, Cg, Nout);
}

template <int RT, bool BWD, int NP, int NT = P3S_NT>
int launch_p3s(P3Params& p, hipStream_t st) {
    auto kern = conv_p3s_kernel<RT, BWD, NP, NT>;
    constexpr int WAVES = 16 / RT;
    const size_t smem = (size_t)2 * P3S_KC * NT * 3072;
    static bool attr_set = false;
    if (!attr_set) {
        if (hipFuncSetAttribute(reinterpret_cast<const void*>(kern), hipFuncAttributeMaxDynamicSharedMemorySize, 160 * 1024) != hipSuccess) {
            (void)hipGetLastError();
            sh_set_error("conv_p3s: cannot raise the dynamic LDS limit to %zu bytes", smem);
            return SH_ERR_LAUNCH;
        }
        attr_set = true;
    }
    p.nsplit = p.nt_tot / NT;
    p.n_vg = sh_cdiv(p.R, RT);
    const long tiles = (long)p.n_vg * (p.B / 16);
    SH_REQUIRE(tiles < (1L << 30), SH_ERR_UNSUPPORTED, "conv_p3s: %ld work items", tiles);
    p.n_tiles = (int)tiles;
    long groups = (tiles + WAVES - 1) / WAVES;
    const long cap = (long)p3_num_cus() / p.nsplit;
    if (groups > cap) groups = cap;
    if (groups < 8) groups = 8;
    groups = (groups + 7) / 8 * 8;
    const int grid = (int)groups * p.nsplit;
    ShProfScope ps(st, "conv_p3s_kernel<%d, %s, %d, %d>|R=%d B=%d K=%d N=%d grid=%dx%d f32=%d", RT, BWD ? "true" : "false", NP, NT, p.R, p.B,
                   p.S * p.Cg, p.Nout, grid, WAVES * 64, p.y ? 1 : 0);
    SH_LAUNCH_PS(ps, kern, dim3(grid), dim3(WAVES * 64), smem, st, p);
    SH_CHECK_LAUNCH("conv_p3s");
    g_p3_launches.fetch_add(1, std::memory_order_relaxed);
    return SH_OK;
}
template <bool BWD, int NP>
int dispatch_p3s(P3Params& p, hipStream_t st) {
    static const int rt = sh_env_int("SH_P3S_RT", 2, 1, 2);
    if (p.nt_tot == 2) return launch_p3s<2, BWD, NP, 2>(p, st);
    return rt == 2 ? launch_p3s<2, BWD, NP>(p, st) : launch_p3s<1, BWD, NP>(p, st);
}

template <int NT, int RT, bool C16, bool BWD, int NP, bool F32R = false>
int launch_p3(P3Params& p, hipStream_t st) {
    auto kern = conv_p3_kernel<NT, RT, C16, BWD, NP, F32R>;
    const size_t smem = (size_t)p.nks * NT * 3072;
    static size_t attr_set = 0;
    if (smem > 65536 && smem > attr_set) {
        if (hipFuncSetAttribute(reinterpret_cast<const void*>(kern), hipFuncAttributeMaxDynamicSharedMemorySize, 160 * 1024) != hipSuccess) {
            (void)hipGetLastError();
            sh_set_error("conv_p3: cannot raise the dynamic LDS limit to %zu bytes", smem);
            return SH_ERR_LAUNCH;
        }
        attr_set = 160 * 1024;
    }
    p.n_vg = sh_cdiv(p.R, RT);
    const long tiles = (long)p.n_vg * (p.B / 16);
    SH_REQUIRE(tiles < (1L << 30), SH_ERR_UNSUPPORTED, "conv_p3: %ld work items", tiles);
    p.n_tiles = (int)tiles;
    const int per_cu = smem <= 36 * 1024 ? 4 : smem <= 76 * 1024 ? 2 : 1;
    static const int waves_cu = sh_env_int("SH_P3_WAVES_CU", 4 * P3_WAVES_PER_EU, 16, 32);
    int nw = waves_cu / per_cu;
    if (nw > 16) nw = 16;
    while (nw > 4 && (nw & 1) == 0 && (long)p3_num_cus() * per_cu * (nw >> 1) >= tiles * p.nsplit) nw >>= 1;
    long groups = (tiles + nw - 1) / nw;
    const long cap = (long)p3_num_cus() * per_cu / p.nsplit;
    if (groups > cap) groups = cap;
    if (groups < 8) groups = 8;
    groups = (groups + 7) / 8 * 8;
    const int grid = (int)groups * p.nsplit;
    ShProfScope ps(st, "conv_p3_kernel<%d, %d, %s, %s, %d, %s>|R=%d B=%d K=%d N=%d grid=%dx%d f32=%d", NT, RT, C16 ? "true" : "false",
                   BWD ? "true" : "false", NP, F32R ? "true" : "false", p.R, p.B, p.S * p.Cg, p.Nout, grid, nw * 64, p.y ? 1 : 0);
    SH_LAUNCH_PS(ps, kern, dim3(grid), dim3(nw * 64), smem, st, p);
    SH_CHECK_LAUNCH("conv_p3");
    g_p3_launches.fetch_add(1, std::memory_order_relaxed);
    return SH_OK;
}

template <int NT, int NP>
int launch_p3r(P3Params& p, hipStream_t st) {
    auto kern = conv_p3r_kernel<NT, NP>;
    const size_t smem = (size_t)p.nks * NT * 3072;
    static size_t attr_set = 0;
    if (smem > 65536 && smem > attr_set) {
        if (hipFuncSetAttribute(reinterpret_cast<const void*>(kern), hipFuncAttributeMaxDynamicSharedMemorySize, 160 * 1024) != hipSuccess) {
            (void)hipGetLastError();
            sh_set_error("conv_p3r: cannot raise the dynamic LDS limit to %zu bytes", smem);
            return SH_ERR_LAUNCH;
        }
        attr_set = 160 * 1024;
    }
    p.n_vg = p.R;
    const long tiles = (long)p.n_vg * (p.B / 16);
    SH_REQUIRE(tiles < (1L << 30), SH_ERR_UNSUPPORTED, "conv_p3r: %ld work items", tiles);
    p.n_tiles = (int)tiles;
    const int per_cu = smem <= 36 * 1024 ? 4 : smem <= 76 * 1024 ? 2 : 1;
    static const int waves_cu = sh_env_int("SH_P3_WAVES_CU", 4 * P3_WAVES_PER_EU, 16, 32);
    int nw = waves_cu / per_cu;
    if (nw > 16) nw = 16;
    while (nw > 4 && (nw & 1) == 0 && (long)p3_num_cus() * per_cu * (nw >> 1) >= tiles * p.nsplit) nw >>= 1;
    long groups = (tiles + nw - 1) / nw;
    const long cap = (long)p3_num_cus() * per_cu / p.nsplit;
    if (groups > cap) groups = cap;
    if (groups < 8) groups = 8;
    groups = (groups + 7) / 8 * 8;
    const int grid = (int)groups * p.nsplit;
    ShProfScope ps(st, "conv_p3r_kernel<%d, %d>|R=%d B=%d K=%d N=%d grid=%dx%d L=%d f32=%d", NT, NP, p.R, p.B, p.S * p.Cg, p.Nout, grid, nw * 64, p.rag_L, p.y ? 1 : 0);
    SH_LAUNCH_PS(ps, kern, dim3(grid), dim3(nw * 64), smem, st, p);
    SH_CHECK_LAUNCH("conv_p3r");
    g_p3_launches.fetch_add(1, std::memory_order_relaxed);
    return SH_OK;
}

template <int NT, int G, bool BWD, int NP, bool C16 = false>
int launch_p3g(P3Params& p, hipStream_t st) {
    auto kern = conv_p3g_kernel<NT, G, BWD, NP, C16>;
    const size_t smem = (size_t)p.nks * NT * 3072;
    static size_t attr_set = 0;
    if (smem > 65536 && smem > attr_set) {
        if (hipFuncSetAttribute(reinterpret_cast<const void*>(kern), hipFuncAttributeMaxDynamicSharedMemorySize, 160 * 1024) != hipSuccess) {
            (void)hipGetLastError();
            sh_set_error("conv_p3g: cannot raise the dynamic LDS limit to %zu bytes", smem);
            return SH_ERR_LAUNCH;
        }
        attr_set = 160 * 1024;
    }
    p.n_vg = p.n_grp;
    const long tiles = (long)p.n_grp * (p.B / 16);
    SH_REQUIRE(tiles < (1L << 30), SH_ERR_UNSUPPORTED, "conv_p3g: %ld work items", tiles);
    p.n_tiles = (int)tiles;
    const int per_cu = smem <= 36 * 1024 ? 4 : smem <= 76 * 1024 ? 2 : 1;
    static const int waves_cu = sh_env_int("SH_P3_WAVES_CU", 4 * P3_WAVES_PER_EU, 16, 32);
    int nw = waves_cu / per_cu;
    if (nw > 16) nw = 16;
    while (nw > 4 && (nw & 1) == 0 && (long)p3_num_cus() * per_cu * (nw >> 1) >= tiles * p.nsplit) nw >>= 1;
    long groups = (tiles + nw - 1) / nw;
    const long cap = (long)p3_num_cus() * per_cu / p.nsplit;
    if (groups > cap) groups = cap;
    if (groups < 8) groups = 8;
    groups = (groups + 7) / 8 * 8;
    const int grid = (int)groups * p.nsplit;
    ShProfScope ps(st, "conv_p3g_kernel<%d, %d, %s, %d, %s>|R=%d B=%d K=%d N=%d grid=%dx%d groups=%d L=%d f32=%d", NT, G, BWD ? "true" : "false", NP,
                   C16 ? "true" : "false", p.R, p.B, p.S * p.Cg, p.Nout, grid, nw * 64, p.n_grp, p.g_L, p.y ? 1 : 0);
    SH_LAUNCH_PS(ps, kern, dim3(grid), dim3(nw * 64), smem, st, p);
    SH_CHECK_LAUNCH("conv_p3g");
    g_p3_launches.fetch_add(1, std::memory_order_relaxed);
    return SH_OK;
}

template <bool C16, bool BWD, int NP, bool F32R = false>
int dispatch_p3_nt(P3Params& p, int nt, hipStream_t st) {
    const long tiles16 = (long)p.R * (p.B / 16);
    const long fill = 2L * p3_num_cus() * 16;
    static const int rt_force = sh_env_int("SH_P3_RT", 0, 0, 2);
    const bool two = rt_force ? rt_force == 2 : tiles16 / 2 >= fill;
    if (nt == 1) return two ? launch_p3<1, 2, C16, BWD, NP, F32R>(p, st) : launch_p3<1, 1, C16, BWD, NP, F32R>(p, st);
    if (nt == 2) return two ? launch_p3<2, 2, C16, BWD, NP, F32R>(p, st) : launch_p3<2, 1, C16, BWD, NP, F32R>(p, st);
    if constexpr (!C16) {
        if (nt == 4) return two ? launch_p3<4, 2, C16, BWD, NP, F32R>(p, st) : launch_p3<4, 1, C16, BWD, NP, F32R>(p, st);
        if (nt == 8) return launch_p3<8, 1, C16, BWD, NP, F32R>(p, st);
    }
    sh_set_error("conv_p3: %d channel tiles per workgroup with %d gathered channels is not built", nt, p.Cg);
    return SH_ERR_UNSUPPORTED;
}

template <bool BWD>
int dispatch_p3(P3Params& p, hipStream_t st) {
    SH_REQUIRE(p3_shape_ok(p.B, p.S, p.Cg, p.Nout), SH_ERR_UNSUPPORTED,
               "conv_p3: B=%d S=%d gathered channels=%d output channels=%d is outside the three-plane kernels (sh_spiral_conv_p3_ok)",
               p.B, p.S, p.Cg, p.Nout);
    const P3Geom g = p3_geom(p.S, p.Cg, p.Nout);
    p.nks = g.nks; p.nt_tot = g.nt_tot; p.nsplit = g.nsplit; p.ncg = p.Cg / 32;
    const int nbg = p.B / 16;
    p.x_bgb = p.Cg == 16 ? 1536 : (long)p.ncg * 3072;
    p.x_vb = p.x_bgb * nbg;
    if (p.yp) {
        SH_REQUIRE(p.Nout == 16 || p.Nout % 32 == 0, SH_ERR_UNSUPPORTED, "conv_p3: a plane image has 16 or a multiple of 32 channels (%d)", p.Nout);
        p.yp_bgb = p.Nout == 16 ? 1536 : (long)(p.Nout / 32) * 3072;
        p.yp_vb = p.yp_bgb * nbg;
    }
    SH_REQUIRE(p.y || p.yp, SH_ERR_INVALID_ARG, "conv_p3: no output");
    SH_REQUIRE(((reinterpret_cast<uintptr_t>(p.xp) | reinterpret_cast<uintptr_t>(p.yp) | reinterpret_cast<uintptr_t>(p.y) |
                 reinterpret_cast<uintptr_t>(p.yprev) | reinterpret_cast<uintptr_t>(p.bias)) & 15) == 0 &&
               ((p.y_sv | p.y_sb | p.yv_sv | p.yv_sb) & 3) == 0, SH_ERR_INVALID_ARG, "conv_p3: tensors must be 16-byte aligned with strides %% 4 == 0");
    static const int np = sh_env_int("SH_P3_NP", 6, 6, 9);
    if (!p3_resident_ok(p.S, p.Cg, p.Nout)) {
        p.nks = p3_nks(p.S, p.Cg, p.Nout);
        SH_REQUIRE(!p.xf, SH_ERR_UNSUPPORTED, "conv_p3: the weight-streaming form takes imaged rows only (sh_spiral_conv_p3_kind() == 2)");
        return np == 9 ? dispatch_p3s<BWD, 9>(p, st) : dispatch_p3s<BWD, 6>(p, st);
    }
    if constexpr (BWD) {
        if (p.xf) {
            SH_REQUIRE(np == 6, SH_ERR_UNSUPPORTED, "conv_p3: fp32 rows are built for the six-product form (SH_P3_NP=6)");
            return p.Cg == 16 ? dispatch_p3_nt<true, true, 6, true>(p, g.nt, st) : dispatch_p3_nt<false, true, 6, true>(p, g.nt, st);
        }
    }
    if (p.Cg == 16) return np == 9 ? dispatch_p3_nt<true, BWD, 9>(p, g.nt, st) : dispatch_p3_nt<true, BWD, 6>(p, g.nt, st);
    return np == 9 ? dispatch_p3_nt<false, BWD, 9>(p, g.nt, st) : dispatch_p3_nt<false, BWD, 6>(p, g.nt, st);
}

}

extern "C" {

size_t sh_p3_bytes(int rows, int B, int C) {
    if (rows <= 0 || B <= 0 || B % 16 || !(C == 16 || (C > 0 && C % 32 == 0))) return 0;
    return (size_t)rows * (B / 16) * (C == 16 ? 1536 : (size_t)(C / 32) * 3072);
}

int sh_to_p3(const float* x, int64_t x_sv, int64_t x_sb, void* planes, int B, int rows, int C, sh_stream_t stream) {
    SH_REQUIRE(x && planes && rows > 0, SH_ERR_INVALID_ARG, "sh_to_p3: null pointer or no rows");
    SH_REQUIRE(sh_p3_bytes(rows, B, C) > 0, SH_ERR_UNSUPPORTED, "sh_to_p3: B=%d C=%d has no plane image (B %% 16 == 0; C == 16 or C %% 32 == 0)", B, C);
    SH_REQUIRE(((reinterpret_cast<uintptr_t>(x) | reinterpret_cast<uintptr_t>(planes)) & 15) == 0 && ((x_sv | x_sb) & 3) == 0,
               SH_ERR_INVALID_ARG, "sh_to_p3: tensors must be 16-byte aligned with strides %% 4 == 0");
    ToP3Args a{x, (long)x_sv, (long)x_sb, static_cast<char*>(planes), B / 16, C, (long)rows * (B / 16) * (C == 16 ? 32 : (C / 32) * 64)};
    hipStream_t st = static_cast<hipStream_t>(stream);
    const long blocks = (a.total + 255) / 256;
    SH_REQUIRE(blocks < (1L << 31), SH_ERR_UNSUPPORTED, "sh_to_p3: tensor too large");
    ShProfScope ps(st, "to_p3_kernel|rows=%d B=%d C=%d", rows, B, C);
    SH_LAUNCH_PS(ps, to_p3_kernel, dim3((unsigned)blocks), dim3(256), 0, st, a);
    SH_CHECK_LAUNCH("to_p3");
    return SH_OK;
}

size_t sh_conv_wfrag3_bytes(int S, int Cg, int Nout) {
    if (S <= 0 || Cg <= 0 || Nout <= 0) return 0;
    const ShFragGeom g = sh_frag_geom(S, Cg, Nout);
    return (size_t)p3_nks(S, Cg, Nout) * g.nt_tot * 3072;
}

int sh_conv_wfrag3_prep_multi(int n_layers, const float* const* weight, void* const* wfrag3, const int* S, const int* Cin,
                              const int* Cout, const int* transpose, sh_stream_t stream) {
    SH_REQUIRE(n_layers > 0 && weight && wfrag3 && S && Cin && Cout && transpose, SH_ERR_INVALID_ARG, "sh_conv_wfrag3_prep_multi: bad argument");
    hipStream_t st = static_cast<hipStream_t>(stream);
    for (int l0 = 0; l0 < n_layers; l0 += WF3_MAX) {
        WFrag3Args a{};
        a.nd = n_layers - l0 < WF3_MAX ? n_layers - l0 : WF3_MAX;
        int blocks = 0;
        for (int i = 0; i < a.nd; ++i) {
            const int k = l0 + i;
            SH_REQUIRE(weight[k] && wfrag3[k] && S[k] > 0 && Cin[k] > 0 && Cout[k] > 0, SH_ERR_INVALID_ARG,
                       "sh_conv_wfrag3_prep_multi: bad layer %d", k);
            SH_REQUIRE((reinterpret_cast<uintptr_t>(wfrag3[k]) & 15) == 0, SH_ERR_INVALID_ARG, "sh_conv_wfrag3_prep_multi: wfrag3 %d misaligned", k);
            const int Cg = transpose[k] ? Cout[k] : Cin[k];
            SH_REQUIRE(Cg % 8 == 0, SH_ERR_UNSUPPORTED, "sh_conv_wfrag3_prep_multi: %d gathered channels", Cg);
            const ShFragGeom g = transpose[k] ? sh_frag_geom(S[k], Cout[k], Cin[k]) : sh_frag_geom(S[k], Cin[k], Cout[k]);
            a.w[i] = weight[k]; a.out[i] = static_cast<u32x4*>(wfrag3[k]);
            const int nks = transpose[k] ? p3_nks(S[k], Cout[k], Cin[k]) : p3_nks(S[k], Cin[k], Cout[k]);
            a.S[i] = S[k]; a.Cin[i] = Cin[k]; a.Cout[i] = Cout[k]; a.tr[i] = transpose[k] ? 1 : 0; a.nks[i] = nks; a.nt_tot[i] = g.nt_tot;
            a.block0[i] = blocks;
            blocks += (nks * g.nt_tot * 64 + 255) / 256;
        }
        a.block0[a.nd] = blocks;
        ShProfScope ps(st, "wfrag3_prep_kernel|layers=%d", a.nd);
        SH_LAUNCH_PS(ps, wfrag3_prep_kernel, dim3(blocks), dim3(256), 0, st, a);
        SH_CHECK_LAUNCH("wfrag3_prep");
    }
    return SH_OK;
}

int64_t sh_p3_launch_count(void) { return (int64_t)g_p3_launches.load(std::memory_order_relaxed); }

int sh_spiral_conv_p3_ok(int B, int S, int Cg, int Nout) { return p3_shape_ok(B, S, Cg, Nout) ? 1 : 0; }
int sh_spiral_conv_p3_kind(int B, int S, int Cg, int Nout) {
    if (!p3_shape_ok(B, S, Cg, Nout)) return 0;
    return p3_resident_ok(S, Cg, Nout) ? 1 : 2;
}

int sh_spiral_conv_fwd_p3(const void* xp, const int32_t* table, const void* wfrag3, const float* bias, float* y, int64_t y_sv,
                          int64_t y_sb, void* yp, int B, int R, int S, int Cin, int Cout, int act, int zero_row, sh_stream_t stream) {
    SH_REQUIRE(xp && table && wfrag3, SH_ERR_INVALID_ARG, "sh_spiral_conv_fwd_p3: null pointer");
    SH_REQUIRE(B > 0 && R > 0 && S > 0 && Cin > 0 && Cout > 0, SH_ERR_INVALID_ARG, "sh_spiral_conv_fwd_p3: non-positive size");
    SH_REQUIRE(act >= SH_ACT_IDENTITY && act <= SH_ACT_TANH, SH_ERR_INVALID_ARG, "sh_spiral_conv_fwd_p3: unknown activation %d", act);
    P3Params p{};
    p.xp = static_cast<const char*>(xp); p.table = table; p.wfrag = static_cast<const u32x4*>(wfrag3); p.bias = bias;
    p.y = y; p.y_sv = y_sv; p.y_sb = y_sb; p.yp = static_cast<char*>(yp);
    p.B = B; p.R = R; p.S = S; p.Cg = Cin; p.Nout = Cout; p.act = act; p.zero_row = zero_row; p.skip_row = -1; p.n_img = 0x7fffffff;
    return dispatch_p3<false>(p, static_cast<hipStream_t>(stream));
}

int sh_spiral_conv_bwd_data_p3(const void* dprep, int dpre_zero_row, const float* dpre_f32, int64_t dp_sv, int64_t dp_sb, int n_image_rows,
                               const int32_t* table_t, const void* wfrag3_t, float* dx, int64_t dx_sv, int64_t dx_sb, void* dxp,
                               const float* yprev, int64_t yp_sv, int64_t yp_sb, const void* yprev_planes, int act_prev, int zero_row, int B,
                               int n_in, int S, int Cin, int Cout, sh_stream_t stream) {
    SH_REQUIRE(dprep && table_t && wfrag3_t, SH_ERR_INVALID_ARG, "sh_spiral_conv_bwd_data_p3: null pointer");
    SH_REQUIRE(B > 0 && n_in > 0 && S > 0 && Cin > 0 && Cout > 0, SH_ERR_INVALID_ARG, "sh_spiral_conv_bwd_data_p3: non-positive size");
    SH_REQUIRE(act_prev >= SH_ACT_IDENTITY && act_prev <= SH_ACT_TANH, SH_ERR_INVALID_ARG, "sh_spiral_conv_bwd_data_p3: unknown activation");
    P3Params p{};
    p.xp = static_cast<const char*>(dprep); p.table = table_t; p.wfrag = static_cast<const u32x4*>(wfrag3_t); p.bias = nullptr;
    p.y = dx; p.y_sv = dx_sv; p.y_sb = dx_sb; p.yp = static_cast<char*>(dxp);
    p.yprev = yprev; p.yv_sv = yp_sv; p.yv_sb = yp_sb;
    if (yprev_planes) {
        SH_REQUIRE(sh_p3_bytes(1, B, Cin) && (reinterpret_cast<uintptr_t>(yprev_planes) & 15) == 0, SH_ERR_UNSUPPORTED,
                   "sh_spiral_conv_bwd_data_p3: B=%d Cin=%d has no plane image (yprev_planes)", B, Cin);
        p.yprev_img = static_cast<const char*>(yprev_planes);
        p.yvi_bgb = Cin == 16 ? 1536 : (long)(Cin / 32) * 3072; p.yvi_vb = p.yvi_bgb * (B / 16);
    }
    p.B = B; p.R = n_in; p.S = S; p.Cg = Cout; p.Nout = Cin; p.act = act_prev; p.zero_row = zero_row;
    static const int skip_on = sh_env_int("SH_P3_SKIP", 1, 0, 1);
    p.skip_row = skip_on ? dpre_zero_row : -1;
    p.n_img = 0x7fffffff;
    if (dpre_f32) {
        SH_REQUIRE(n_image_rows >= 0 && (reinterpret_cast<uintptr_t>(dpre_f32) & 15) == 0 && ((dp_sv | dp_sb) & 3) == 0, SH_ERR_INVALID_ARG,
                   "sh_spiral_conv_bwd_data_p3: the fp32 gradient must be 16-byte aligned with strides %% 4 == 0");
        p.xf = dpre_f32; p.xf_sv = dp_sv; p.xf_sb = dp_sb; p.n_img = n_image_rows;
    }
    return dispatch_p3<true>(p, static_cast<hipStream_t>(stream));
}

int sh_spiral_conv_p3_rag_ok(int B, int S, int Cg, int Nout, int rag_L) {
    return p3_shape_ok(B, S, Cg, Nout) && p3_resident_ok(S, Cg, Nout) && p3_geom(S, Cg, Nout).nt <= 4 && Cg % 32 == 0 && rag_L > 0 && rag_L <= 64;
}

int sh_spiral_conv_bwd_data_p3_rag(const void* dprep, const int32_t* rag_rows, const int32_t* rag_pos, int rag_L, const void* wfrag3_t, float* dx,
                                   int64_t dx_sv, int64_t dx_sb, void* dxp, const float* yprev, int64_t yp_sv, int64_t yp_sb,
                                   const void* yprev_planes, int act_prev, int zero_row, int B, int n_in, int S, int Cin, int Cout,
                                   sh_stream_t stream) {
    SH_REQUIRE(dprep && rag_rows && rag_pos && wfrag3_t, SH_ERR_INVALID_ARG, "sh_spiral_conv_bwd_data_p3_rag: null pointer");
    SH_REQUIRE(B > 0 && n_in > 0 && S > 0 && Cin > 0 && Cout > 0, SH_ERR_INVALID_ARG, "sh_spiral_conv_bwd_data_p3_rag: non-positive size");
    SH_REQUIRE(act_prev >= SH_ACT_IDENTITY && act_prev <= SH_ACT_TANH, SH_ERR_INVALID_ARG, "sh_spiral_conv_bwd_data_p3_rag: unknown activation");
    SH_REQUIRE(sh_spiral_conv_p3_rag_ok(B, S, Cout, Cin, rag_L), SH_ERR_UNSUPPORTED,
               "sh_spiral_conv_bwd_data_p3_rag: B=%d S=%d gathered channels=%d output channels=%d lists of %d is not taken (resident three-plane "
               "weight, gathered channels %% 32 == 0, lists of at most 64 sources)", B, S, Cout, Cin, rag_L);
    P3Params p{};
    p.xp = static_cast<const char*>(dprep); p.wfrag = static_cast<const u32x4*>(wfrag3_t);
    p.y = dx; p.y_sv = dx_sv; p.y_sb = dx_sb; p.yp = static_cast<char*>(dxp);
    p.yprev = yprev; p.yv_sv = yp_sv; p.yv_sb = yp_sb;
    p.B = B; p.R = n_in; p.S = S; p.Cg = Cout; p.Nout = Cin; p.act = act_prev; p.zero_row = zero_row;
    p.rag_rows = rag_rows; p.rag_pos = rag_pos; p.rag_L = rag_L;
    if (yprev_planes) {
        SH_REQUIRE(sh_p3_bytes(1, B, Cin) && (reinterpret_cast<uintptr_t>(yprev_planes) & 15) == 0, SH_ERR_UNSUPPORTED,
                   "sh_spiral_conv_bwd_data_p3_rag: B=%d Cin=%d has no plane image (yprev_planes)", B, Cin);
        p.yprev_img = static_cast<const char*>(yprev_planes);
        p.yvi_bgb = Cin == 16 ? 1536 : (long)(Cin / 32) * 3072; p.yvi_vb = p.yvi_bgb * (B / 16);
    }
    const P3Geom g = p3_geom(p.S, p.Cg, p.Nout);
    p.nks = g.nks; p.nt_tot = g.nt_tot; p.nsplit = g.nsplit; p.ncg = p.Cg / 32;
    const int nbg = B / 16;
    p.x_bgb = (long)p.ncg * 3072; p.x_vb = p.x_bgb * nbg;
    if (p.yp) {
        SH_REQUIRE(p.Nout == 16 || p.Nout % 32 == 0, SH_ERR_UNSUPPORTED, "conv_p3r: a plane image has 16 or a multiple of 32 channels (%d)", p.Nout);
        p.yp_bgb = p.Nout == 16 ? 1536 : (long)(p.Nout / 32) * 3072; p.yp_vb = p.yp_bgb * nbg;
    }
    SH_REQUIRE(p.y || p.yp, SH_ERR_INVALID_ARG, "conv_p3r: no output");
    SH_REQUIRE(((reinterpret_cast<uintptr_t>(p.xp) | reinterpret_cast<uintptr_t>(p.yp) | reinterpret_cast<uintptr_t>(p.y) | reinterpret_cast<uintptr_t>(p.yprev)) & 15) == 0 &&
               ((p.y_sv | p.y_sb | p.yv_sv | p.yv_sb) & 3) == 0, SH_ERR_INVALID_ARG, "conv_p3r: tensors must be 16-byte aligned with strides %% 4 == 0");
    static const int np = sh_env_int("SH_P3_NP", 6, 6, 9);
    hipStream_t st = static_cast<hipStream_t>(stream);
    const int nt = g.nt;
#define SH_P3R_CASE(N) (np == 9 ? launch_p3r<N, 9>(p, st) : launch_p3r<N, 6>(p, st))
    if (nt == 1) return SH_P3R_CASE(1);
    if (nt == 2) return SH_P3R_CASE(2);
    if (nt == 4) return SH_P3R_CASE(4);
#undef SH_P3R_CASE
    sh_set_error("conv_p3r: %d channel tiles per workgroup is not built", nt);
    return SH_ERR_UNSUPPORTED;
}

int sh_spiral_conv_p3_grp_ok(int B, int S, int Cg, int Nout, int g_L) {
    static const int c16_on = sh_env_int("SH_P3_GRP_C16", 1, 0, 1);
    if (!(Cg % 32 == 0 || (Cg == 16 && c16_on && p3_geom(S, Cg, Nout).nt <= 2))) return 0;
    return p3_shape_ok(B, S, Cg, Nout) && p3_resident_ok(S, Cg, Nout) && p3_geom(S, Cg, Nout).nt <= 4 && S < 255 && g_L > 0 && g_L <= 64;
}

int sh_spiral_conv_p3_grp_members(int B, int S, int Cg, int Nout) {
    if (!sh_spiral_conv_p3_grp_ok(B, S, Cg, Nout, 1)) return 0;
    return p3_geom(S, Cg, Nout).nt <= 2 ? 4 : 2;
}

int sh_spiral_conv_p3_grp_pays(int B, int n_groups) {
    static const int min_per_cu = sh_env_int("SH_P3_GRP_MIN_ITEMS_PER_CU", 12, 0, 1 << 20);
    return B >= 16 && (long)n_groups * (B / 16) >= (long)min_per_cu * p3_num_cus();
}

int sh_spiral_conv_p3_grp(const void* xp, const int32_t* g_rows, const uint32_t* g_pos, const int32_t* g_out, int n_groups, int g_L,
                          const void* wfrag3, const float* bias, float* y, int64_t y_sv, int64_t y_sb, void* yp, const float* yprev,
                          int64_t yp_sv, int64_t yp_sb, const void* yprev_planes, int act, int zero_row, int backward, int B, int R, int S,
                          int Cg, int Nout, sh_stream_t stream) {
    SH_REQUIRE(xp && g_rows && g_pos && g_out && wfrag3, SH_ERR_INVALID_ARG, "sh_spiral_conv_p3_grp: null pointer");
    SH_REQUIRE(B > 0 && R > 0 && S > 0 && Cg > 0 && Nout > 0 && n_groups > 0, SH_ERR_INVALID_ARG, "sh_spiral_conv_p3_grp: non-positive size");
    SH_REQUIRE(act >= SH_ACT_IDENTITY && act <= SH_ACT_TANH, SH_ERR_INVALID_ARG, "sh_spiral_conv_p3_grp: unknown activation");
    SH_REQUIRE(sh_spiral_conv_p3_grp_ok(B, S, Cg, Nout, g_L), SH_ERR_UNSUPPORTED,
               "sh_spiral_conv_p3_grp: B=%d S=%d gathered channels=%d output channels=%d lists of %d is not taken (resident three-plane weight, "
               "gathered channels 16 or %% 32 == 0, lists of at most 64 rows)", B, S, Cg, Nout, g_L);
    SH_REQUIRE(backward || !(yprev || yprev_planes), SH_ERR_INVALID_ARG, "sh_spiral_conv_p3_grp: yprev belongs to the backward form");
    P3Params p{};
    p.xp = static_cast<const char*>(xp); p.wfrag = static_cast<const u32x4*>(wfrag3); p.bias = backward ? nullptr : bias;
    p.y = y; p.y_sv = y_sv; p.y_sb = y_sb; p.yp = static_cast<char*>(yp);
    p.yprev = yprev; p.yv_sv = yp_sv; p.yv_sb = yp_sb;
    p.B = B; p.R = R; p.S = S; p.Cg = Cg; p.Nout = Nout; p.act = act; p.zero_row = zero_row;
    p.g_rows = g_rows; p.g_pos = g_pos; p.g_out = g_out; p.g_L = g_L; p.n_grp = n_groups;
    if (yprev_planes) {
        SH_REQUIRE(sh_p3_bytes(1, B, Nout) && (reinterpret_cast<uintptr_t>(yprev_planes) & 15) == 0, SH_ERR_UNSUPPORTED,
                   "sh_spiral_conv_p3_grp: B=%d channels=%d has no plane image (yprev_planes)", B, Nout);
        p.yprev_img = static_cast<const char*>(yprev_planes);
        p.yvi_bgb = Nout == 16 ? 1536 : (long)(Nout / 32) * 3072; p.yvi_vb = p.yvi_bgb * (B / 16);
    }
    const P3Geom g = p3_geom(p.S, p.Cg, p.Nout);
    p.nks = g.nks; p.nt_tot = g.nt_tot; p.nsplit = g.nsplit; p.ncg = p.Cg / 32;
    const int nbg = B / 16;
    const bool c16 = Cg == 16;
    p.x_bgb = c16 ? 1536 : (long)p.ncg * 3072; p.x_vb = p.x_bgb * nbg;
    if (p.yp) {
        SH_REQUIRE(p.Nout == 16 || p.Nout % 32 == 0, SH_ERR_UNSUPPORTED, "conv_p3g: a plane image has 16 or a multiple of 32 channels (%d)", p.Nout);
        p.yp_bgb = p.Nout == 16 ? 1536 : (long)(p.Nout / 32) * 3072; p.yp_vb = p.yp_bgb * nbg;
    }
    SH_REQUIRE(p.y || p.yp, SH_ERR_INVALID_ARG, "conv_p3g: no output");
    SH_REQUIRE(((reinterpret_cast<uintptr_t>(p.xp) | reinterpret_cast<uintptr_t>(p.yp) | reinterpret_cast<uintptr_t>(p.y) | reinterpret_cast<uintptr_t>(p.yprev) |
                 reinterpret_cast<uintptr_t>(p.bias)) & 15) == 0 && ((p.y_sv | p.y_sb | p.yv_sv | p.yv_sb) & 3) == 0, SH_ERR_INVALID_ARG,
               "conv_p3g: tensors must be 16-byte aligned with strides %% 4 == 0");
    static const int np = sh_env_int("SH_P3_NP", 6, 6, 9);
    hipStream_t st = static_cast<hipStream_t>(stream);
    const int nt = g.nt;
#define SH_P3G_CASE(N, GG) (backward ? (np == 9 ? launch_p3g<N, GG, true, 9>(p, st) : launch_p3g<N, GG, true, 6>(p, st)) \
                                     : (np == 9 ? launch_p3g<N, GG, false, 9>(p, st) : launch_p3g<N, GG, false, 6>(p, st)))
#define SH_P3G_CASE16(N) (backward ? (np == 9 ? launch_p3g<N, 4, true, 9, true>(p, st) : launch_p3g<N, 4, true, 6, true>(p, st)) \
                                   : (np == 9 ? launch_p3g<N, 4, false, 9, true>(p, st) : launch_p3g<N, 4, false, 6, true>(p, st)))
    if (c16 && nt == 1) return SH_P3G_CASE16(1);
    if (c16 && nt == 2) return SH_P3G_CASE16(2);
#undef SH_P3G_CASE16
    if (nt == 1) return SH_P3G_CASE(1, 4);
    if (nt == 2) return SH_P3G_CASE(2, 4);
    if (nt == 4) return SH_P3G_CASE(4, 2);
#undef SH_P3G_CASE
    sh_set_error("conv_p3g: %d channel tiles per workgroup is not built", nt);
    return SH_ERR_UNSUPPORTED;
}

}
```

### semantichuman_amd/csrc/stack_exec.hip

```cpp
#include "sh_common.h"

namespace {

struct Lay { long sv, sb; };
inline Lay lay(int layout, int rows, int B, int C) {
    return layout == 0 ? Lay{(long)B * C, (long)C} : Lay{(long)C, (long)rows * C};
}
inline int out_rows(const sh_stack_step& s) { return s.kind == 0 ? s.R : s.m_rows; }
inline bool is_last_step(int i, int n) { return i == n - 1; }
inline int in_rows(const sh_stack_step& s) { return s.kind == 0 ? s.n_in : s.m_cols; }

int check_tensor_sizes(int n, const sh_stack_step* st, int rows0, int c0, int B, const char* what) {
    long rows = rows0;
    int c = c0;
    for (int i = 0; i <= n; ++i) {
        long extra = 0;
        if (i > 0 && st[i - 1].kind == 0) extra = (long)st[i - 1].n1 + st[i - 1].n2;
        SH_REQUIRE((rows + extra) * (long)B * c < (1L << 32), SH_ERR_UNSUPPORTED,
                   "%s: the tensor %s step %d has %ld rows x %d batch entries x %d channels >= 2^32 elements - split the batch", what,
                   i < n ? "entering" : "leaving", i < n ? i : n - 1, rows + extra, B, c);
        if (i == n) break;
        rows = st[i].kind == 0 ? st[i].R : (st[i].extend ? (long)st[i].m_cols + st[i].m_rows : st[i].m_rows);
        if (st[i].kind == 0) c = st[i].cout;
    }
    return SH_OK;
}

int check_steps(int n, const sh_stack_step* st, int c0, const char* what) {
    SH_REQUIRE(n > 0 && st, SH_ERR_INVALID_ARG, "%s: no steps", what);
    int c = c0;
    for (int i = 0; i < n; ++i) {
        SH_REQUIRE(st[i].kind == 0 || st[i].kind == 1, SH_ERR_INVALID_ARG, "%s: step %d has kind %d", what, i, st[i].kind);
        if (st[i].kind == 0) {
            SH_REQUIRE(st[i].cin == c, SH_ERR_INVALID_ARG, "%s: step %d takes %d channels, its input has %d", what, i, st[i].cin, c);
            SH_REQUIRE(st[i].table && st[i].param >= 0, SH_ERR_INVALID_ARG, "%s: step %d incomplete", what, i);
            c = st[i].cout;
        } else {
            SH_REQUIRE(st[i].m.rowptr && st[i].m.col && st[i].m.val, SH_ERR_INVALID_ARG, "%s: step %d has no matrix", what, i);
        }
    }
    return SH_OK;
}

int check_call(int n, const sh_stack_step* st, int rows0, int c0, int B, bool pointers, const char* what) {
    int rc = check_steps(n, st, c0, what);
    if (rc != SH_OK) return rc;
    if (B > 0 && (rc = check_tensor_sizes(n, st, rows0, c0, B, what)) != SH_OK) return rc;
    SH_REQUIRE(pointers && B > 0, SH_ERR_INVALID_ARG, "%s: null pointer or empty batch", what);
    SH_REQUIRE(n <= 64, SH_ERR_UNSUPPORTED, "%s: more than 64 steps", what);
    return SH_OK;
}

void fill_cin_of(int n, const sh_stack_step* st, int c0, int* cin_of) {
    for (int i = 0, c = c0; i < n; ++i) { cin_of[i] = c; if (st[i].kind == 0) c = st[i].cout; }
}

int prep_wfrags(int n_steps, const sh_stack_step* steps, const float* const* weights, void* const* frag, int transpose, bool skip_first,
                bool ready, const char* what, sh_stream_t stream) {
    const float* w[64]; void* wf[64]; int S[64], Ci[64], Co[64], tr[64];
    int n = 0;
    for (int i = skip_first ? 1 : 0; i < n_steps; ++i) {
        if (steps[i].kind != 0) continue;
        SH_REQUIRE(frag && frag[i], SH_ERR_INVALID_ARG, "%s: no weight-fragment buffer for step %d", what, i);
        w[n] = weights[steps[i].param]; wf[n] = frag[i]; S[n] = steps[i].S; Ci[n] = steps[i].cin; Co[n] = steps[i].cout; tr[n] = transpose;
        ++n;
    }
    return n && !ready ? sh_conv_wfrag_prep_multi(n, w, wf, S, Ci, Co, tr, stream) : SH_OK;
}

struct ReduceJobs {
    typedef int (*Reduce)(int, const void* const*, float* const*, float* const*, const int*, const int*, const int*, const int*, const int*,
                          const int*, sh_stream_t);
    const void* ws[64]; float* dW[64]; float* db[64]; int B[64], R[64], S[64], Ci[64], Co[64], kind[64];
    int n = 0;
    void add(const void* workspace, float* dw, float* dbias, int b, const sh_stack_step& s, int k) {
        ws[n] = workspace; dW[n] = dw; db[n] = dbias; B[n] = b; R[n] = s.R; S[n] = s.S; Ci[n] = s.cin; Co[n] = s.cout; kind[n] = k;
        ++n;
    }
    int flush(Reduce reduce, sh_stream_t stream) const {
        for (int k = 0; k < n; k += 16) {
            const int rc = reduce(n - k < 16 ? n - k : 16, ws + k, dW + k, db + k, B + k, R + k, S + k, Ci + k, Co + k, kind + k, stream);
            if (rc != SH_OK) return rc;
        }
        return SH_OK;
    }
};
int reduce_bf16(int n, const void* const* ws, float* const* dW, float* const* db, const int* B, const int* R, const int* S, const int* Ci,
                const int* Co, const int*, sh_stream_t stream) {
    return sh_spiral_conv_bwd_wgt_reduce_multi_bf16(n, ws, dW, db, B, R, S, Ci, Co, stream);
}

struct Switches { int n16_maxb, bwd, wgrad, yprev_img, drop_fp32, ragged, grouped, presum_img, tr_ride; };
const Switches& switches() {
    static const Switches s{sh_env_int("SH_P3_N16_MAXB", 256, 0, 1 << 30), sh_env_int("SH_P3_BWD", 1, 0, 1), sh_env_int("SH_P3_WGRAD", 1, 0, 1),
                            sh_env_int("SH_P3_YPREV_IMG", 1, 0, 1),        sh_env_int("SH_P3_DROP_FP32", 1, 0, 1),
                            sh_env_int("SH_P3_RAGGED", 1, 0, 1),           sh_env_int("SH_P3_GROUPED", 1, 0, 1),
                            sh_env_int("SH_P3_PRESUM_IMG", 2, 0, 2),       sh_env_int("SH_TR_RIDE", 1, 0, 1)};
    return s;
}

enum { BD_F32 = 0, BD_TABLE, BD_RAG, BD_GRP };
struct Forms {
    bool f_p3;
    bool f_grp;
    bool f_img;
    bool f_img_only;
    bool b_gimg;
    bool b_thin;
    int b_data;
    bool b_ride;
    bool b_presum_img;
    bool b_p3w;
    bool b_yimg;
    bool b_in_img_only;
    bool b_grad_img_only;
};

inline int consumer_conv(int n, const sh_stack_step* st, int i) {
    int j = i + 1;
    if (j < n && st[j].kind == 1 && st[j].extend) ++j;
    return (j < n && st[j].kind == 0) ? j : -1;
}

void plan_f32(int n, const sh_stack_step* st, int B, int x_layout, bool planes3, int keep_fp32, bool need_x_grad, Forms* f) {
    const Switches& sw = switches();
    for (int i = 0; i < n; ++i) f[i] = Forms{};
    for (int i = 1; i < n && planes3; ++i) {
        const sh_stack_step& s = st[i];
        if (s.kind != 0) continue;
        f[i].f_p3 = !(s.cout <= 16 && B > sw.n16_maxb) && sh_spiral_conv_p3_ok(B, s.S, s.cin, s.cout);
        f[i].f_grp = f[i].f_p3 && sw.grouped && s.fg_rows && s.fg_pos && s.fg_out && s.fg_n > 0 &&
                     sh_spiral_conv_p3_grp_ok(B, s.S, s.cin, s.cout, s.fg_L) && sh_spiral_conv_p3_grp_pays(B, s.fg_n);
    }
    for (int i = 0; i + 1 < n; ++i) {
        const int c = consumer_conv(n, st, i);
        f[i].f_img = c >= 0 && f[c].f_p3;
    }
    for (int i = 0; i < n; ++i) {
        const sh_stack_step& s = st[i];
        Forms& q = f[i];
        if (s.kind != 0 || !(i > 0 || need_x_grad) || !s.table_t) continue;
        q.b_gimg = planes3 && sw.bwd && sh_spiral_conv_p3_ok(B, s.S, s.cout, s.cin);
        q.b_thin = s.R == s.n_in && (i > 0 || x_layout == 0) && sh_spiral_conv_bwd_wgt_thin_ok(B, s.n_in, s.S, s.cin, s.cout, SH_DTYPE_F32);
        if (q.b_gimg) {
            const bool grp = sw.ragged && sw.grouped && s.bg_rows && s.bg_pos && s.bg_out && s.bg_n > 0 &&
                             sh_spiral_conv_p3_grp_ok(B, s.S, s.cout, s.cin, s.bg_L) && sh_spiral_conv_p3_grp_pays(B, s.bg_n);
            const bool rag = sw.ragged && s.rag_rows && s.rag_pos && sh_spiral_conv_p3_rag_ok(B, s.S, s.cout, s.cin, s.rag_L);
            q.b_data = grp ? BD_GRP : rag ? BD_RAG : BD_TABLE;
            q.b_presum_img = sw.presum_img == 1 ||
                             !(sh_spiral_conv_p3_kind(B, s.S, s.cout, s.cin) == 1 && (sw.presum_img == 0 || 2 * (s.n1 + s.n2) >= s.R));
        }
        const bool p3 = q.b_data != BD_F32 && !q.b_thin;
        q.b_ride = !q.b_thin && q.b_data < BD_RAG && (s.n1 || s.n2);
        q.b_p3w = p3 && sw.wgrad && i > 0 && f[i - 1].f_img && sh_spiral_conv_bwd_wgt_p3_ok(B, s.R, s.S, s.cin, s.cout) &&
                  (((long)s.R * (B / 16)) % 2 == 0 || s.zero_row >= 0);
        q.b_yimg = q.b_data != BD_F32 && sw.wgrad && sw.yprev_img && i > 0 && st[i - 1].kind == 0 && f[i - 1].f_img;
        q.b_in_img_only = keep_fp32 == 2 && sw.drop_fp32 && sw.yprev_img && q.b_p3w;
        q.b_grad_img_only = q.b_in_img_only && (q.b_data >= BD_RAG || (s.n1 == 0 && s.n2 == 0));
    }
    for (int i = 0; i + 1 < n; ++i) {
        const int c = consumer_conv(n, st, i);
        f[i].f_img_only = f[i].f_img && (keep_fp32 == 0 || f[c].b_in_img_only) && (st[i].kind == 1 || (f[i].f_p3 && c == i + 1));
    }
}

}

extern "C" {

int sh_stack_plan_f32(int n_steps, const sh_stack_step* steps, int c0, int B, int x_layout, int mma_mode, int keep_fp32, int need_x_grad,
                      int* forms) {
    int rc = check_steps(n_steps, steps, c0, "sh_stack_plan_f32");
    if (rc != SH_OK) return rc;
    SH_REQUIRE(forms && B > 0 && n_steps <= 64 && sh_mma_mode_valid(mma_mode) && keep_fp32 >= 0 && keep_fp32 <= 2, SH_ERR_INVALID_ARG,
               "sh_stack_plan_f32: null pointer, empty batch, more than 64 steps, mma_mode %d or keep_fp32 %d", mma_mode, keep_fp32);
    Forms f[64];
    plan_f32(n_steps, steps, B, x_layout, mma_mode == SH_MMA_PLANES3, keep_fp32, need_x_grad != 0, f);
    for (int i = 0; i < n_steps; ++i) {
        const Forms& q = f[i];
        const int bd = q.b_thin ? BD_F32 : q.b_data;
        const bool on[15] = {q.f_p3, q.f_grp, q.f_img, q.f_img_only, q.b_gimg, q.b_thin, bd != BD_F32, bd == BD_RAG, bd == BD_GRP, q.b_ride,
                             bd != BD_F32 && q.b_presum_img, q.b_p3w, q.b_yimg, q.b_in_img_only, q.b_grad_img_only};
        forms[i] = 0;
        for (int k = 0; k < 15; ++k) forms[i] |= on[k] ? 1 << k : 0;
    }
    return SH_OK;
}

int sh_stack_forward(int n_steps, const sh_stack_step* steps, const float* x, int x_layout, int rows0, int c0, int B,
                     const float* const* weights, const float* const* biases, float* const* outs, int out_layout, int mma_mode,
                     void* const* planes, const void* const* wfrag3, int keep_fp32, sh_stream_t stream) {
    int rc = check_call(n_steps, steps, rows0, c0, B, x && weights && outs, "sh_stack_forward");
    if (rc != SH_OK) return rc;
    SH_REQUIRE(sh_mma_mode_valid(mma_mode), SH_ERR_INVALID_ARG, "sh_stack_forward: unknown mma_mode %d", mma_mode);
    SH_REQUIRE(keep_fp32 >= 0 && keep_fp32 <= 2, SH_ERR_INVALID_ARG, "sh_stack_forward: keep_fp32 = %d (0, 1 or 2)", keep_fp32);
    Forms f[64];
    plan_f32(n_steps, steps, B, x_layout, mma_mode == SH_MMA_PLANES3 && planes && wfrag3, keep_fp32, false, f);
    for (int i = 0; i < n_steps; ++i) {
        SH_REQUIRE(outs[i], SH_ERR_INVALID_ARG, "sh_stack_forward: no output buffer for step %d", i);
        SH_REQUIRE(!f[i].f_img || planes[i], SH_ERR_INVALID_ARG, "sh_stack_forward: step %d writes the image of its output: planes[%d] is NULL", i, i);
        SH_REQUIRE(!f[i].f_p3 || wfrag3[i], SH_ERR_INVALID_ARG, "sh_stack_forward: step %d runs on planes: wfrag3[%d] is NULL", i, i);
    }
    const float* cur = x;
    Lay cl = lay(x_layout, rows0, B, c0);
    int c = c0;
    for (int i = 0; i < n_steps; ++i) {
        const sh_stack_step& s = steps[i];
        const Forms& q = f[i];
        const int co = s.kind == 0 ? s.cout : c;
        const Lay ol = lay(i == n_steps - 1 ? out_layout : 0, out_rows(s), B, co);
        void* img = q.f_img ? planes[i] : nullptr;
        if (s.kind == 0) {
            const float* bias = biases ? biases[s.param] : nullptr;
            float* y = q.f_img_only ? nullptr : outs[i];
            if (q.f_grp)
                rc = sh_spiral_conv_p3_grp(planes[i - 1], s.fg_rows, s.fg_pos, s.fg_out, s.fg_n, s.fg_L, wfrag3[i], bias, y, ol.sv, ol.sb, img, nullptr,
                                           0, 0, nullptr, s.act, s.zero_row, 0, B, s.R, s.S, s.cin, s.cout, stream);
            else if (q.f_p3)
                rc = sh_spiral_conv_fwd_p3(planes[i - 1], s.table, wfrag3[i], bias, y, ol.sv, ol.sb, img, B, s.R, s.S, s.cin, s.cout, s.act,
                                           s.zero_row, stream);
            else
                rc = sh_spiral_conv_fwd_img(cur, cl.sv, cl.sb, s.table, weights[s.param], bias, outs[i], ol.sv, ol.sb, img, B, s.R, s.S, s.cin,
                                            s.cout, s.act, s.zero_row, mma_mode, stream);
        } else if (s.extend) {
            SH_REQUIRE(i > 0 && !is_last_step(i, n_steps) && outs[i] == outs[i - 1] && cl.sb == c, SH_ERR_INVALID_ARG,
                       "sh_stack_forward: step %d appends to its input, which must be the vertex-major output buffer of step %d", i, i - 1);
            SH_REQUIRE(!img || planes[i] == planes[i - 1], SH_ERR_INVALID_ARG, "sh_stack_forward: step %d appends to its input: same image buffer", i);
            float* dst = q.f_img_only ? nullptr : outs[i] + (long)s.m_cols * cl.sv;
            rc = sh_spmm_p3(s.m.rowptr, s.m.col, s.m.val, cur, cl.sv, cl.sb, dst, cl.sv, cl.sb,
                            img ? static_cast<char*>(img) + sh_p3_bytes(s.m_cols, B, c) : nullptr, nullptr, 0, 0, 0, -1, B, s.m_rows, c, stream);
        } else {
            rc = sh_spmm_p3(s.m.rowptr, s.m.col, s.m.val, cur, cl.sv, cl.sb, q.f_img_only ? nullptr : outs[i], ol.sv, ol.sb, img, nullptr, 0, 0, 0,
                            -1, B, s.m_rows, c, stream);
        }
        if (rc != SH_OK) return rc;
        cur = outs[i]; cl = ol; c = co;
    }
    return SH_OK;
}

int sh_stack_backward(int n_steps, const sh_stack_step* steps, const float* x, int x_layout, int rows0, int c0, int B,
                      const float* const* acts, const float* g, int out_layout, const float* const* weights,
                      float* const* gin, float* dpre_last, float* const* weight_t, void* const* workspace,
                      const size_t* workspace_bytes, float* const* dW, float* const* dbias, int need_x_grad, int mma_mode,
                      void* const* gin_planes, void* dpre_last_planes, const void* const* wfrag3_t, const void* const* in_planes,
                      int acts_fp32, sh_stream_t stream) {
    int rc = check_call(n_steps, steps, rows0, c0, B, x && acts && g && weights && gin && dW, "sh_stack_backward");
    if (rc != SH_OK) return rc;
    SH_REQUIRE(sh_mma_mode_valid(mma_mode), SH_ERR_INVALID_ARG, "sh_stack_backward: unknown mma_mode %d", mma_mode);
    const bool planes3 = mma_mode == SH_MMA_PLANES3 && gin_planes && wfrag3_t;
    SH_REQUIRE(acts_fp32 == 1 || (acts_fp32 == 2 && planes3 && in_planes), SH_ERR_INVALID_ARG,
               "sh_stack_backward: acts_fp32 = %d (1: every activation has its fp32 rows; 2, three-plane form with gin_planes, wfrag3_t and "
               "in_planes: the forward pass ran with keep_fp32 == 2)", acts_fp32);
    const int last = n_steps - 1;
    Forms f[64];
    plan_f32(n_steps, steps, B, x_layout, planes3, acts_fp32, need_x_grad != 0, f);
    for (int i = 0; i < n_steps; ++i) {
        SH_REQUIRE(!f[i].b_gimg || (wfrag3_t[i] && (i == last ? dpre_last_planes : gin_planes[i + 1])), SH_ERR_INVALID_ARG,
                   "sh_stack_backward: step %d runs backward-data on planes: wfrag3_t[%d] and the image buffer of its gradient (%s) are required",
                   i, i, i == last ? "dpre_last_planes" : "gin_planes[i + 1]");
        SH_REQUIRE(!in_planes || !(f[i].b_p3w || f[i].b_yimg) || in_planes[i], SH_ERR_INVALID_ARG,
                   "sh_stack_backward: step %d reads the image of its input: in_planes[%d] is NULL", i, i);
    }
    const Switches& sw = switches();
    int cin_of[64];
    fill_cin_of(n_steps, steps, c0, cin_of);
    const float* tr_w[32]; float* tr_wt[32]; int tr_S[32], tr_Ci[32], tr_Co[32];
    int n_tr = 0;
    for (int i = 0; i < n_steps; ++i) {
        if (steps[i].kind != 0 || !(i > 0 || need_x_grad) || (f[i].b_gimg && !f[i].b_thin)) continue;
        SH_REQUIRE(weight_t && weight_t[i], SH_ERR_INVALID_ARG, "sh_stack_backward: no weight_t buffer for step %d", i);
        SH_REQUIRE(n_tr < 32, SH_ERR_UNSUPPORTED, "sh_stack_backward: more than 32 conv steps");
        tr_w[n_tr] = weights[steps[i].param]; tr_wt[n_tr] = weight_t[i]; tr_S[n_tr] = steps[i].S; tr_Ci[n_tr] = steps[i].cin; tr_Co[n_tr] = steps[i].cout;
        ++n_tr;
    }
    if (n_tr && !(sw.tr_ride && steps[last].kind == 0)) {
        rc = sh_weight_transpose_multi(n_tr, tr_w, tr_wt, tr_S, tr_Ci, tr_Co, stream);
        if (rc != SH_OK) return rc;
        n_tr = 0;
    }
    const float* cur; Lay cl;
    void* cur_img = nullptr;
    bool cur_img_done = false;
    {
        const sh_stack_step& s = steps[last];
        if (s.kind == 0) {
            SH_REQUIRE(dpre_last, SH_ERR_INVALID_ARG, "sh_stack_backward: no dpre_last buffer");
            const Lay ol = lay(out_layout, s.R, B, s.cout), dl = lay(0, 0, B, s.cout);
            cur_img = f[last].b_gimg ? dpre_last_planes : nullptr;
            const bool img_in = cur_img && s.cout % 4 == 0 && s.cout > 8;
            rc = sh_act_backward_tr_img(g, ol.sv, ol.sb, acts[last], ol.sv, ol.sb, dpre_last, dl.sv, dl.sb, img_in ? cur_img : nullptr, B, s.R,
                                        s.cout, s.act, s.zero_row, n_tr, tr_w, tr_wt, tr_S, tr_Ci, tr_Co, stream);
            if (rc != SH_OK) return rc;
            cur = dpre_last; cl = dl;
            cur_img_done = img_in;
        } else {
            cur = g; cl = lay(out_layout, s.m_rows, B, cin_of[last]);
        }
    }
    ReduceJobs jobs;
    for (int i = last; i >= 0; --i) {
        const sh_stack_step& s = steps[i];
        const Forms& q = f[i];
        const bool want_in = i > 0 || need_x_grad;
        const float* inp = i == 0 ? x : acts[i - 1];
        const Lay il = i == 0 ? lay(x_layout, rows0, B, c0) : lay(0, 0, B, cin_of[i]);
        float* gi = want_in ? gin[i] : nullptr;
        SH_REQUIRE(!want_in || gi, SH_ERR_INVALID_ARG, "sh_stack_backward: no gradient buffer for the input of step %d", i);
        const Lay gl = il;
        const float* yprev = nullptr; Lay yl{0, 0}; int act_prev = 0, zero_prev = -1;
        if (i > 0 && steps[i - 1].kind == 0) {
            yprev = acts[i - 1]; yl = lay(0, 0, B, steps[i - 1].cout); act_prev = steps[i - 1].act; zero_prev = steps[i - 1].zero_row;
        }
        void* gi_img = (i > 0 && steps[i - 1].kind == 0 && f[i - 1].b_gimg) ? gin_planes[i] : nullptr;
        float* gi_f = (gi_img && f[i - 1].b_grad_img_only) ? nullptr : gi;
        bool gi_img_done = false;
        if (s.kind == 0) {
            SH_REQUIRE(workspace && workspace[i], SH_ERR_INVALID_ARG, "sh_stack_backward: no workspace for step %d", i);
            const bool wgrad = dW[s.param] != nullptr;
            SH_REQUIRE(wgrad || !dbias || !dbias[s.param], SH_ERR_INVALID_ARG,
                       "sh_stack_backward: parameter %d has a dbias buffer but no dW buffer", s.param);
            const bool thin = wgrad && q.b_thin;
            const int bd = thin ? BD_F32 : q.b_data;
            const bool p3 = bd != BD_F32, rag = bd >= BD_RAG;
            const bool ride = wgrad && q.b_ride;
            char* pimg0 = (p3 && q.b_presum_img) ? static_cast<char*>(cur_img) : nullptr;
            float* mut0 = const_cast<float*>(cur);
            if (ride && s.n1 && s.n2) {
                rc = sh_spmm_p3(s.sum1.rowptr, s.sum1.col, s.sum1.val, cur, cl.sv, cl.sb, mut0 + (long)s.R * cl.sv, cl.sv, cl.sb,
                                pimg0 ? pimg0 + sh_p3_bytes(s.R, B, s.cout) : nullptr, nullptr, 0, 0, 0, -1, B, s.n1, s.cout, stream);
                if (rc != SH_OK) return rc;
            }
            const bool p3w = wgrad && q.b_p3w && in_planes && workspace_bytes[i] >= sh_spiral_conv_bwd_wgt_p3_workspace(B, s.R, s.S, s.cin, s.cout);
            SH_REQUIRE(!q.b_in_img_only || p3w, SH_ERR_INVALID_ARG,
                       "sh_stack_backward: step %d: the forward pass kept only the image of its input (keep_fp32 == 2) but this pass cannot run "
                       "the step on images (a frozen layer, or a workspace smaller than sh_spiral_conv_bwd_wgt_p3_workspace)", i);
            if (wgrad && !thin) {
                const sh_csr_ref& lm = s.n2 ? s.sum2 : s.sum1;
                const int ln = ride ? (s.n2 ? s.n2 : s.n1) : 0;
                float* lout = mut0 + (long)(s.R + (s.n2 ? s.n1 : 0)) * cl.sv;
                void* limg = (ln && pimg0) ? pimg0 + sh_p3_bytes(s.R + (s.n2 ? s.n1 : 0), B, s.cout) : nullptr;
                if (p3w) {
                    if (!cur_img_done) {
                        rc = sh_to_p3(cur, cl.sv, cl.sb, cur_img, B, s.R, s.cout, stream);
                        if (rc != SH_OK) return rc;
                        cur_img_done = true;
                    }
                    rc = sh_spiral_conv_bwd_wgt_p3_presum(cur_img, s.zero_row, in_planes[i], s.table, workspace[i], workspace_bytes[i], cur, cl.sv, cl.sb,
                                                          ln ? lm.rowptr : nullptr, ln ? lm.col : nullptr, ln ? lm.val : nullptr,
                                                          ln ? lout : nullptr, limg, ln, B, s.R, s.S, s.cin, s.cout, stream);
                } else {
                    rc = sh_spiral_conv_bwd_wgt_presum(cur, cl.sv, cl.sb, inp, il.sv, il.sb, s.table, nullptr, nullptr, workspace[i],
                                                       workspace_bytes[i], ln ? lm.rowptr : nullptr, ln ? lm.col : nullptr,
                                                       ln ? lm.val : nullptr, ln ? lout : nullptr, limg, ln, B, s.R, s.S, s.cin, s.cout, mma_mode,
                                                       stream);
                }
                if (rc != SH_OK) return rc;
            }
            if (wgrad) jobs.add(workspace[i], dW[s.param], dbias ? dbias[s.param] : nullptr, B, s, p3w ? 2 : 0);
            if (want_in) {
                SH_REQUIRE(s.table_t, SH_ERR_INVALID_ARG, "sh_stack_backward: step %d has no transposed table", i);
                float* mut = const_cast<float*>(cur);
                char* pimg = pimg0;
                if (s.n1 && !ride && !rag) {
                    rc = sh_spmm_p3(s.sum1.rowptr, s.sum1.col, s.sum1.val, cur, cl.sv, cl.sb, mut + (long)s.R * cl.sv, cl.sv, cl.sb,
                                    pimg ? pimg + sh_p3_bytes(s.R, B, s.cout) : nullptr, nullptr, 0, 0, 0, -1, B, s.n1, s.cout, stream);
                    if (rc != SH_OK) return rc;
                }
                if (s.n2 && !ride && !rag) {
                    rc = sh_spmm_p3(s.sum2.rowptr, s.sum2.col, s.sum2.val, cur, cl.sv, cl.sb, mut + (long)(s.R + s.n1) * cl.sv,
                                    cl.sv, cl.sb, pimg ? pimg + sh_p3_bytes(s.R + s.n1, B, s.cout) : nullptr, nullptr, 0, 0, 0, -1, B, s.n2,
                                    s.cout, stream);
                    if (rc != SH_OK) return rc;
                }
                if (thin) {
                    rc = sh_spiral_conv_bwd_wgt_thin(cur, cl.sv, cl.sb, inp, SH_DTYPE_F32, il.sv, il.sb, s.table_t, workspace[i],
                                                     workspace_bytes[i], weights[s.param], gi, gl.sv, gl.sb, gi_img, yprev ? act_prev : SH_ACT_IDENTITY,
                                                     zero_prev, B, s.R, s.n_in, s.S, s.cin, s.cout, SH_DTYPE_F32, stream);
                    gi_img_done = gi_img != nullptr;
                } else if (p3) {
                    if (!cur_img_done) {
                        rc = sh_to_p3(cur, cl.sv, cl.sb, cur_img, B, s.R, s.cout, stream);
                        if (rc != SH_OK) return rc;
                    }
                    const void* yimg = (q.b_yimg && in_planes) ? in_planes[i] : nullptr;
                    if (bd == BD_GRP)
                        rc = sh_spiral_conv_p3_grp(cur_img, s.bg_rows, s.bg_pos, s.bg_out, s.bg_n, s.bg_L, wfrag3_t[i], nullptr, gi_f, gl.sv, gl.sb,
                                                   gi_img, yprev, yl.sv, yl.sb, yimg, act_prev, zero_prev, 1, B, s.n_in, s.S, s.cout, s.cin, stream);
                    else if (bd == BD_RAG)
                        rc = sh_spiral_conv_bwd_data_p3_rag(cur_img, s.rag_rows, s.rag_pos, s.rag_L, wfrag3_t[i], gi_f, gl.sv, gl.sb, gi_img, yprev,
                                                            yl.sv, yl.sb, yimg, act_prev, zero_prev, B, s.n_in, s.S, s.cin, s.cout, stream);
                    else
                        rc = sh_spiral_conv_bwd_data_p3(cur_img, s.zero_row, q.b_presum_img ? nullptr : cur, cl.sv, cl.sb, s.R, s.table_t, wfrag3_t[i],
                                                        gi_f, gl.sv, gl.sb, gi_img, yprev, yl.sv, yl.sb, yimg, act_prev, zero_prev, B, s.n_in, s.S,
                                                        s.cin, s.cout, stream);
                    gi_img_done = gi_img != nullptr;
                } else {
                    rc = sh_spiral_conv_bwd_data_z(cur, cl.sv, cl.sb, s.zero_row, s.table_t, weight_t[i], gi, gl.sv, gl.sb, yprev, yl.sv,
                                                   yl.sb, act_prev, zero_prev, B, s.n_in, s.S, s.cin, s.cout, mma_mode, stream);
                }
                if (rc != SH_OK) return rc;
            }
        } else if (want_in) {
            SH_REQUIRE(s.mt.rowptr && s.mt.col && s.mt.val, SH_ERR_INVALID_ARG, "sh_stack_backward: step %d has no transposed matrix", i);
            rc = sh_spmm_p3(s.mt.rowptr, s.mt.col, s.mt.val, cur, cl.sv, cl.sb, gi_f, gl.sv, gl.sb, gi_img, yprev, yl.sv, yl.sb,
                            act_prev, zero_prev, B, s.m_cols, cin_of[i], stream);
            if (rc != SH_OK) return rc;
            gi_img_done = gi_img != nullptr;
        }
        if (want_in) { cur = gi; cl = gl; cur_img = gi_img; cur_img_done = gi_img_done; }
    }
    return jobs.flush(sh_spiral_conv_bwd_wgt_reduce_multi_kinds, stream);
}

static inline long esz_of(int dtype) { return dtype == SH_DTYPE_BF16 ? 2 : 4; }

int sh_stack_forward_bf16(int n_steps, const sh_stack_step* steps, const void* x, int x_dtype, int x_layout, int rows0, int c0, int B,
                          const float* const* weights, const float* const* biases, void* const* wfrag, int wfrag_ready,
                          void* const* outs, int out_dtype, int out_layout, sh_stream_t stream) {
    int rc = check_call(n_steps, steps, rows0, c0, B, x && weights && outs && wfrag, "sh_stack_forward_bf16");
    if (rc != SH_OK) return rc;
    rc = prep_wfrags(n_steps, steps, weights, wfrag, 0, false, wfrag_ready != 0, "sh_stack_forward_bf16", stream);
    if (rc != SH_OK) return rc;
    const void* cur = x;
    int cd = x_dtype;
    Lay cl = lay(x_layout, rows0, B, c0);
    int c = c0;
    for (int i = 0; i < n_steps; ++i) {
        const sh_stack_step& s = steps[i];
        const bool is_last = i == n_steps - 1;
        const int co = s.kind == 0 ? s.cout : c;
        const int od = is_last ? out_dtype : SH_DTYPE_BF16;
        const Lay ol = lay(is_last ? out_layout : 0, out_rows(s), B, co);
        SH_REQUIRE(outs[i], SH_ERR_INVALID_ARG, "sh_stack_forward_bf16: no output buffer for step %d", i);
        if (s.kind == 0) {
            rc = sh_spiral_conv_fwd_bf16(cur, cd, cl.sv, cl.sb, s.table, wfrag[i], biases ? biases[s.param] : nullptr, outs[i], od, ol.sv,
                                         ol.sb, B, s.R, s.S, s.cin, s.cout, s.act, s.zero_row, stream);
        } else {
            SH_REQUIRE(cd == SH_DTYPE_BF16 && od == SH_DTYPE_BF16, SH_ERR_UNSUPPORTED,
                       "sh_stack_forward_bf16: re-sampling step %d needs bf16 on both sides", i);
            if (s.extend) {
                SH_REQUIRE(i > 0 && !is_last && outs[i] == outs[i - 1] && cl.sb == c, SH_ERR_INVALID_ARG,
                           "sh_stack_forward_bf16: step %d appends to its input, which must be the vertex-major output buffer of step %d", i, i - 1);
                rc = sh_spmm_bf16(s.m.rowptr, s.m.col, s.m.val, cur, cl.sv, cl.sb, static_cast<char*>(outs[i]) + (long)s.m_cols * cl.sv * 2, cl.sv,
                                  cl.sb, nullptr, 0, 0, 0, -1, B, s.m_rows, c, stream);
            } else {
                rc = sh_spmm_bf16(s.m.rowptr, s.m.col, s.m.val, cur, cl.sv, cl.sb, outs[i], ol.sv, ol.sb, nullptr, 0, 0, 0, -1, B, s.m_rows, c,
                                  stream);
            }
        }
        if (rc != SH_OK) return rc;
        cur = outs[i]; cd = od; cl = ol; c = co;
    }
    return SH_OK;
}

int sh_stack_backward_bf16(int n_steps, const sh_stack_step* steps, const void* x, int x_dtype, int x_layout, int rows0, int c0, int B,
                           const void* const* acts, const void* g, int out_dtype, int out_layout, const float* const* weights,
                           void* const* gin, int gx_dtype, void* dpre_last, void* const* wfrag_t, int wfrag_ready,
                           void* const* workspace, const size_t* workspace_bytes, float* const* dW, float* const* dbias, int need_x_grad,
                           sh_stream_t stream) {
    int rc = check_call(n_steps, steps, rows0, c0, B, x && acts && g && weights && gin && dW, "sh_stack_backward_bf16");
    if (rc != SH_OK) return rc;
    const int last = n_steps - 1;
    int cin_of[64];
    fill_cin_of(n_steps, steps, c0, cin_of);
    rc = prep_wfrags(n_steps, steps, weights, wfrag_t, 1, !need_x_grad, wfrag_ready != 0, "sh_stack_backward_bf16", stream);
    if (rc != SH_OK) return rc;
    const void* cur; Lay cl; int cd;
    {
        const sh_stack_step& s = steps[last];
        if (s.kind == 0) {
            SH_REQUIRE(dpre_last, SH_ERR_INVALID_ARG, "sh_stack_backward_bf16: no dpre_last buffer");
            const Lay ol = lay(out_layout, s.R, B, s.cout), dl = lay(0, 0, B, s.cout);
            if (out_dtype == SH_DTYPE_F32)
                rc = sh_act_backward(static_cast<const float*>(g), ol.sv, ol.sb, static_cast<const float*>(acts[last]), ol.sv, ol.sb,
                                     static_cast<float*>(dpre_last), dl.sv, dl.sb, B, s.R, s.cout, s.act, s.zero_row, stream);
            else
                rc = sh_act_backward_bf16(g, ol.sv, ol.sb, acts[last], ol.sv, ol.sb, dpre_last, dl.sv, dl.sb, B, s.R, s.cout, s.act, s.zero_row,
                                          stream);
            if (rc != SH_OK) return rc;
            cur = dpre_last; cl = dl; cd = out_dtype;
        } else {
            SH_REQUIRE(out_dtype == SH_DTYPE_BF16, SH_ERR_UNSUPPORTED, "sh_stack_backward_bf16: a re-sampling last step needs a bf16 gradient");
            cur = g; cl = lay(out_layout, s.m_rows, B, cin_of[last]); cd = out_dtype;
        }
    }
    ReduceJobs jobs;
    for (int i = last; i >= 0; --i) {
        const sh_stack_step& s = steps[i];
        const bool want_in = i > 0 || need_x_grad;
        const void* inp = i == 0 ? x : acts[i - 1];
        const int ind = i == 0 ? x_dtype : SH_DTYPE_BF16;
        const Lay il = i == 0 ? lay(x_layout, rows0, B, c0) : lay(0, 0, B, cin_of[i]);
        void* gi = want_in ? gin[i] : nullptr;
        const int gd = i == 0 ? gx_dtype : SH_DTYPE_BF16;
        SH_REQUIRE(!want_in || gi, SH_ERR_INVALID_ARG, "sh_stack_backward_bf16: no gradient buffer for the input of step %d", i);
        const Lay gl = i == 0 ? lay(x_layout, rows0, B, c0) : lay(0, 0, B, cin_of[i]);
        const void* yprev = nullptr; Lay yl{0, 0}; int act_prev = 0, zero_prev = -1;
        if (i > 0 && steps[i - 1].kind == 0) {
            yprev = acts[i - 1]; yl = lay(0, 0, B, steps[i - 1].cout); act_prev = steps[i - 1].act; zero_prev = steps[i - 1].zero_row;
        }
        if (s.kind == 0) {
            SH_REQUIRE(workspace && workspace[i], SH_ERR_INVALID_ARG, "sh_stack_backward_bf16: no workspace for step %d", i);
            const bool wgrad = dW[s.param] != nullptr;
            SH_REQUIRE(wgrad || !dbias || !dbias[s.param], SH_ERR_INVALID_ARG,
                       "sh_stack_backward_bf16: parameter %d has a dbias buffer but no dW buffer", s.param);
            const bool thin = wgrad && want_in && s.table_t && cd == SH_DTYPE_F32 && ind == SH_DTYPE_BF16 && s.R == s.n_in && il.sb == s.cin &&
                              il.sv == (long)B * s.cin && cl.sb == s.cout && cl.sv == (long)B * s.cout &&
                              sh_spiral_conv_bwd_wgt_thin_ok(B, s.n_in, s.S, s.cin, s.cout, SH_DTYPE_BF16);
            if (wgrad && !thin) {
                rc = sh_spiral_conv_bwd_wgt_bf16(cur, cd, cl.sv, cl.sb, inp, ind, il.sv, il.sb, s.table, workspace[i], workspace_bytes[i], B,
                                                 s.R, s.S, s.cin, s.cout, stream);
                if (rc != SH_OK) return rc;
            }
            if (wgrad) jobs.add(workspace[i], dW[s.param], dbias ? dbias[s.param] : nullptr, B, s, 0);
            if (want_in) {
                SH_REQUIRE(s.table_t, SH_ERR_INVALID_ARG, "sh_stack_backward_bf16: step %d has no transposed table", i);
                static const int rag_on = sh_env_int("SH_BF16_RAGGED", 1, 0, 1);
                const bool rag = rag_on && !thin && cd == SH_DTYPE_BF16 && gd == SH_DTYPE_BF16 && s.rag_rows && s.rag_pos &&
                                 sh_spiral_conv_bf16_rag_ok(B, s.S, s.cout, s.cin, s.rag_L);
                char* mut = static_cast<char*>(const_cast<void*>(cur));
                const long rb = cl.sv * esz_of(cd);
                for (int lev = 0; lev < 2; ++lev) {
                    const int n = lev == 0 ? s.n1 : s.n2;
                    if (!n || rag) continue;
                    const sh_csr_ref& m = lev == 0 ? s.sum1 : s.sum2;
                    void* dst = mut + (long)(s.R + (lev == 0 ? 0 : s.n1)) * rb;
                    if (cd == SH_DTYPE_F32)
                        rc = sh_spmm(m.rowptr, m.col, m.val, static_cast<const float*>(cur), cl.sv, cl.sb, static_cast<float*>(dst), cl.sv, cl.sb,
                                     nullptr, 0, 0, 0, -1, B, n, s.cout, stream);
                    else
                        rc = sh_spmm_bf16(m.rowptr, m.col, m.val, cur, cl.sv, cl.sb, dst, cl.sv, cl.sb, nullptr, 0, 0, 0, -1, B, n, s.cout, stream);
                    if (rc != SH_OK) return rc;
                }
                const bool thin_dx = thin && gd == SH_DTYPE_BF16 && gl.sb == s.cin && gl.sv == (long)B * s.cin && (!yprev || yprev == inp);
                if (thin) {
                    rc = sh_spiral_conv_bwd_wgt_thin(static_cast<const float*>(cur), cl.sv, cl.sb, inp, SH_DTYPE_BF16, il.sv, il.sb, s.table_t,
                                                     workspace[i], workspace_bytes[i], weights[s.param], thin_dx ? gi : nullptr, gl.sv, gl.sb,
                                                     nullptr, yprev ? act_prev : SH_ACT_IDENTITY, zero_prev, B, s.R, s.n_in, s.S, s.cin, s.cout,
                                                     SH_DTYPE_BF16, stream);
                    if (rc != SH_OK) return rc;
                }
                if (rag)
                    rc = sh_spiral_conv_bwd_data_bf16_rag(cur, cl.sv, cl.sb, s.rag_rows, s.rag_pos, s.rag_L, wfrag_t[i], gi, gl.sv, gl.sb, yprev, yl.sv,
                                                          yl.sb, act_prev, zero_prev, B, s.n_in, s.S, s.cin, s.cout, stream);
                else if (!thin_dx)
                    rc = sh_spiral_conv_bwd_data_bf16(cur, cd, cl.sv, cl.sb, s.table_t, wfrag_t[i], gi, gd, gl.sv, gl.sb, yprev, yl.sv, yl.sb,
                                                      act_prev, zero_prev, B, s.n_in, s.S, s.cin, s.cout, stream);
                if (rc != SH_OK) return rc;
            }
        } else if (want_in) {
            SH_REQUIRE(s.mt.rowptr && s.mt.col && s.mt.val, SH_ERR_INVALID_ARG, "sh_stack_backward_bf16: step %d has no transposed matrix", i);
            SH_REQUIRE(cd == SH_DTYPE_BF16 && gd == SH_DTYPE_BF16, SH_ERR_UNSUPPORTED,
                       "sh_stack_backward_bf16: re-sampling step %d needs bf16 on both sides", i);
            rc = sh_spmm_bf16(s.mt.rowptr, s.mt.col, s.mt.val, cur, cl.sv, cl.sb, gi, gl.sv, gl.sb, yprev, yl.sv, yl.sb, act_prev, zero_prev, B,
                              s.m_cols, cin_of[i], stream);
            if (rc != SH_OK) return rc;
        }
        if (want_in) { cur = gi; cl = gl; cd = gd; }
    }
    return jobs.flush(reduce_bf16, stream);
}

}
```

Measured before the change: 47420.

## Add split-K two-wave work items to weight-streaming spiral conv kernel

Adds a split form of the weight-streaming p3s conv kernel. Each work item is served by two waves that each take half of every K chunk, and their accumulators are combined through shared memory before the epilogue. A heuristic turns it on by default for backward-data layers whose item count is low relative to CU count, raising occupancy and latency hiding on small layers. In exchange it adds a second barrier and a shared-memory reduction per round and uses 2048/RT-thread blocks.

```diff
diff --git a/include/sh_kernels.h b/include/sh_kernels.h
--- a/include/sh_kernels.h
+++ b/include/sh_kernels.h
@@ -463,6 +463,16 @@
                                       const void* yprev_planes, int act_prev, int zero_row, int B, int n_in, int S, int Cin, int Cout,
                                       sh_stream_t stream);
 
+SH_API int sh_spiral_conv_p3s_split_pays(int B, int R, int S, int Cg, int Nout, int backward);
+SH_API int sh_spiral_conv_fwd_p3_form(const void* xp, const int32_t* table, const void* wfrag3, const float* bias, float* y, int64_t y_sv,
+                                      int64_t y_sb, void* yp, int B, int R, int S, int Cin, int Cout, int act, int zero_row, int split,
+                                      sh_stream_t stream);
+SH_API int sh_spiral_conv_bwd_data_p3_form(const void* dprep, int dpre_zero_row, const float* dpre_f32, int64_t dp_sv, int64_t dp_sb,
+                                           int n_image_rows, const int32_t* table_t, const void* wfrag3_t, float* dx, int64_t dx_sv,
+                                           int64_t dx_sb, void* dxp, const float* yprev, int64_t yp_sv, int64_t yp_sb,
+                                           const void* yprev_planes, int act_prev, int zero_row, int B, int n_in, int S, int Cin, int Cout,
+                                           int split, sh_stream_t stream);
+
 SH_API int sh_spiral_conv_p3_rag_ok(int B, int S, int Cg, int Nout, int rag_L);
 SH_API int sh_spiral_conv_bwd_data_p3_rag(const void* dprep, const int32_t* rag_rows, const int32_t* rag_pos, int rag_L, const void* wfrag3_t,
                                           float* dx, int64_t dx_sv, int64_t dx_sb, void* dxp, const float* yprev, int64_t yp_sv,
diff --git a/semantichuman_amd/_lib.py b/semantichuman_amd/_lib.py
--- a/semantichuman_amd/_lib.py
+++ b/semantichuman_amd/_lib.py
@@ -145,6 +145,9 @@
     "sh_spmm_p3": (c_int, [_P, _P, _P, _P, _L, _L, _P, _L, _L, _P, _P, _L, _L, _I, _I, _I, _I, _I, _P]),
     "sh_spiral_conv_fwd_p3": (c_int, [_P, _P, _P, _P, _P, _L, _L, _P, _I, _I, _I, _I, _I, _I, _I, _P]),
     "sh_spiral_conv_bwd_data_p3": (c_int, [_P, _I, _P, _L, _L, _I, _P, _P, _P, _L, _L, _P, _P, _L, _L, _P, _I, _I, _I, _I, _I, _I, _I, _P]),
+    "sh_spiral_conv_p3s_split_pays": (c_int, [_I, _I, _I, _I, _I, _I]),
+    "sh_spiral_conv_fwd_p3_form": (c_int, [_P, _P, _P, _P, _P, _L, _L, _P, _I, _I, _I, _I, _I, _I, _I, _I, _P]),
+    "sh_spiral_conv_bwd_data_p3_form": (c_int, [_P, _I, _P, _L, _L, _I, _P, _P, _P, _L, _L, _P, _P, _L, _L, _P, _I, _I, _I, _I, _I, _I, _I, _I, _P]),
     "sh_spiral_conv_p3_rag_ok": (c_int, [_I, _I, _I, _I, _I]),
     "sh_spiral_conv_bf16_rag_ok": (c_int, [_I, _I, _I, _I, _I]),
     "sh_spiral_conv_p3_grp_ok": (c_int, [_I, _I, _I, _I, _I]),
diff --git a/semantichuman_amd/csrc/p3_conv.hip b/semantichuman_amd/csrc/p3_conv.hip
--- a/semantichuman_amd/csrc/p3_conv.hip
+++ b/semantichuman_amd/csrc/p3_conv.hip
@@ -614,14 +614,20 @@
 
 constexpr int P3S_NT = 4, P3S_KC = 4;
 
-template <int RT, bool BWD, int NP, int NT = P3S_NT>
-__global__ __launch_bounds__(1024 / RT) void conv_p3s_kernel(const P3Params p) {
-    constexpr int D = P3S_KC, WAVES = 16 / RT, WF = P3S_KC * NT * 3 / WAVES;
-    static_assert(WF * WAVES == P3S_KC * NT * 3, "a chunk's fragments must divide evenly over the waves");
+template <int RT, bool BWD, int NP, int NT = P3S_NT, bool SPLIT = false>
+__global__ __launch_bounds__((SPLIT ? 2048 : 1024) / RT) void conv_p3s_kernel(const P3Params p) {
+    static_assert(!SPLIT || RT == 2, "the split-item form is built for two vertices per item (16 waves of 1024 threads)");
+    constexpr int HW = SPLIT ? 2 : 1;
+    constexpr int D = P3S_KC / HW;
+    constexpr int ITEMS = 16 / RT, WAVES = ITEMS * HW, NFRAG = P3S_KC * NT * 3;
+    constexpr int WF = (NFRAG + WAVES - 1) / WAVES;
+    static_assert(SPLIT || WF * WAVES == NFRAG, "a chunk's fragments must divide evenly over the waves");
+    static_assert(!SPLIT || ITEMS * RT * NT * 1024 <= 2 * NFRAG * 1024, "the handed-over accumulators must fit the chunk buffers");
     extern __shared__ __attribute__((aligned(16))) char smem[];
     u32x4* Wl = reinterpret_cast<u32x4*>(smem);
     constexpr int CHUNK_PIECES = P3S_KC * NT * 192;
-    const int tid = threadIdx.x, lane = tid & 63, wave = tid >> 6;
+    const int tid = threadIdx.x, lane = tid & 63, wave = SPLIT ? __builtin_amdgcn_readfirstlane(tid >> 6) : tid >> 6;
+    const int item = SPLIT ? wave % ITEMS : wave, half = SPLIT ? wave / ITEMS : 0;
     const int xcd = blockIdx.x & 7, li = blockIdx.x >> 3;
     const int nwg_x = ((int)gridDim.x - xcd + 7) >> 3;
     const int slice = li % p.nsplit, lj = li / p.nsplit;
@@ -629,23 +635,38 @@
     const int q8 = p.n_tiles >> 3, r8 = p.n_tiles & 7;
     const int t_begin = xcd < r8 ? xcd * (q8 + 1) : r8 * (q8 + 1) + (xcd - r8) * q8;
     const int t_end = t_begin + (xcd < r8 ? q8 + 1 : q8);
-    const int stride = ngrp * WAVES;
+    const int stride = ngrp * ITEMS;
     const int r16 = lane & 15, kq = lane >> 4;
     const int S = p.S, sl = lane < S ? lane : S - 1;
     const f32x4 zero4 = {0.f, 0.f, 0.f, 0.f};
     const int nch = p.nks / P3S_KC;
     int wsrc[WF], wdst[WF];
+    bool wown[WF];
 #pragma unroll
     for (int j = 0; j < WF; ++j) {
         const int f = WF * wave + j, pl = f % 3, n = (f / 3) % NT, kk = f / (3 * NT);
+        wown[j] = WF * WAVES == NFRAG || f < NFRAG;
         wsrc[j] = ((kk * p.nt_tot + slice * NT + n) * 3 + pl) * 64 + lane;
         wdst[j] = f * 64 + lane;
     }
+    auto wsrc_at = [&](int j) {
+        if constexpr (!SPLIT) return wsrc[j];
+        const int f = WF * wave + j, pl = f % 3, n = (f / 3) % NT, kk = f / (3 * NT);
+        return ((kk * p.nt_tot + slice * NT + n) * 3 + pl) * 64 + lane;
+    };
+    auto wdst_at = [&](int j) {
+        if constexpr (!SPLIT) return wdst[j];
+        return (WF * wave + j) * 64 + lane;
+    };
     const int wchunk = P3S_KC * p.nt_tot * 192;
     const unsigned rowmul = (unsigned)(p.x_vb >> 4);
     const int skip_key = (int)((unsigned)p.skip_row * rowmul);
-    const int rounds = (t_end - t_begin - lj * WAVES + stride - 1) / stride;
-    int t = t_begin + lj * WAVES + wave;
+    const int rounds = (t_end - t_begin - lj * ITEMS + stride - 1) / stride;
+    int t = t_begin + lj * ITEMS + item;
+    auto advance = [&](int& s, int& c, int n) {
+        c += n;
+        while (c >= p.ncg) { c -= p.ncg; ++s; }
+    };
     for (int rd = 0; rd < rounds; ++rd, t += stride) {
         const bool live = t < t_end;
         const int tt = live ? t : t_end - 1;
@@ -656,21 +677,27 @@
         for (int m = 0; m < RT; ++m) tv[m] = (int)((unsigned)p.table[(long)(v0 + m < p.R ? v0 + m : p.R - 1) * S + sl] * rowmul);
         const char* xl = p.xp + (long)bs * p.x_bgb + lane * 16;
         int ls = 0, lc = 0;
+        if constexpr (SPLIT) advance(ls, lc, half * D);
         u32x4 ring[D][RT][3];
-        auto issue = [&](u32x4 (&a)[RT][3]) {
+        auto issue = [&](u32x4 (&a)[RT][3], auto PL) {
             const int s = ls < S ? ls : S - 1;
 #pragma unroll
             for (int m = 0; m < RT; ++m) {
                 const int row = __builtin_amdgcn_readlane(tv[m], s);
                 const bool f32row = false;
                 const char* src = f32row ? reinterpret_cast<const char*>(p.xf + (long)row * p.xf_sv + (long)(bs * 16 + r16) * p.xf_sb + lc * 32 + kq * 8)
-                                         : xl + (long)((unsigned long)(unsigned)row << 4) + (long)lc * 3072;
+                                  : SPLIT ? p.xp + (long)bs * p.x_bgb + (long)((unsigned long)(unsigned)row << 4) + (long)lc * 3072 + (unsigned)(lane * 16)
+                                          : xl + (long)((unsigned long)(unsigned)row << 4) + (long)lc * 3072;
                 const int o1 = f32row ? 16 : 1024, o2 = f32row ? 0 : 2048;
                 a[m][0] = *reinterpret_cast<const u32x4*>(src);
                 a[m][1] = *reinterpret_cast<const u32x4*>(src + o1);
                 a[m][2] = *reinterpret_cast<const u32x4*>(src + o2);
             }
-            if (++lc >= p.ncg) { lc = 0; ++ls; }
+            if constexpr (!SPLIT) {
+                if (++lc >= p.ncg) { lc = 0; ++ls; }
+            } else {
+                advance(ls, lc, decltype(PL)::value == D - 1 ? 1 + P3S_KC - D : 1);
+            }
         };
         f32x4 acc[RT][NT];
 #pragma unroll
@@ -678,16 +705,21 @@
 #pragma unroll
             for (int n = 0; n < NT; ++n) acc[m][n] = zero4;
         int cs = 0, cc = 0;
-        auto compute = [&](const u32x4* wk, u32x4 (&a)[RT][3]) {
+        if constexpr (SPLIT && BWD) advance(cs, cc, half * D);
+        auto compute = [&](const u32x4* wk, u32x4 (&a)[RT][3], auto PL) {
             bool live[RT];
             bool any = false;
 #pragma unroll
             for (int m = 0; m < RT; ++m) {
-                const int row = BWD ? __builtin_amdgcn_readlane(tv[m], cs) : 0;
+                const int row = BWD ? __builtin_amdgcn_readlane(tv[m], SPLIT && cs >= S ? S - 1 : cs) : 0;
                 live[m] = !BWD || p.skip_row < 0 || row != skip_key;
                 any = any || live[m];
             }
-            if (BWD && ++cc >= p.ncg) { cc = 0; if (cs + 1 < S) ++cs; }
+            if constexpr (BWD && !SPLIT) {
+                if (++cc >= p.ncg) { cc = 0; if (cs + 1 < S) ++cs; }
+            } else if constexpr (BWD) {
+                advance(cs, cc, decltype(PL)::value == D - 1 ? 1 + P3S_KC - D : 1);
+            }
             if (!any) return;
             constexpr int PW[9] = {2, 2, 1, 2, 0, 1, 1, 0, 0}, PX[9] = {2, 1, 2, 0, 2, 1, 0, 1, 0};
 #pragma unroll
@@ -704,42 +736,67 @@
                         c = __builtin_amdgcn_mfma_f32_16x16x32_bf16(w[PW[q]], *reinterpret_cast<const bf16x8*>(&a[m][PX[q]]), c, 0, 0, 0);
                     acc[m][n] = c;
                 }
+                if constexpr (SPLIT) __builtin_amdgcn_sched_barrier(0);
             }
         };
         u32x4 wreg[WF];
 #pragma unroll
-        for (int j = 0; j < WF; ++j) wreg[j] = p.wfrag[wsrc[j]];
-#pragma unroll
-        for (int d = 0; d < D - 1; ++d) issue(ring[d]);
-#pragma unroll
-        for (int j = 0; j < WF; ++j) Wl[wdst[j]] = wreg[j];
+        for (int j = 0; j < WF; ++j)
+            if (wown[j]) wreg[j] = p.wfrag[wsrc_at(j)];
+#pragma unroll
+        for (int d = 0; d < D - 1; ++d) issue(ring[d], std::integral_constant<int, 0>{});
+#pragma unroll
+        for (int j = 0; j < WF; ++j)
+            if (wown[j]) Wl[wdst_at(j)] = wreg[j];
         __syncthreads();
         for (int c = 0; c < nch; ++c) {
             const bool more = c + 1 < nch;
             if (more) {
 #pragma unroll
-                for (int j = 0; j < WF; ++j) wreg[j] = p.wfrag[wsrc[j] + (c + 1) * wchunk];
-            }
-            const u32x4* wb = Wl + (c & 1) * CHUNK_PIECES + lane;
+                for (int j = 0; j < WF; ++j)
+                    if (wown[j]) wreg[j] = p.wfrag[wsrc_at(j) + (c + 1) * wchunk];
+            }
+            const u32x4* wb = Wl + (c & 1) * CHUNK_PIECES + half * D * NT * 192 + lane;
             auto step = [&](auto J, int) {
                 constexpr int j = decltype(J)::value;
-                issue(ring[(j + D - 1) % D]);
+                issue(ring[(j + D - 1) % D], std::integral_constant<int, (j + D - 1) % D>{});
                 __builtin_amdgcn_sched_barrier(0);
-                compute(wb + j * NT * 192, ring[j]);
+                compute(wb + j * NT * 192, ring[j], J);
             };
             p3_ring_steps<0, D>(0, D, step);
             if (more) {
                 u32x4* wn = Wl + ((c + 1) & 1) * CHUNK_PIECES;
 #pragma unroll
-                for (int j = 0; j < WF; ++j) wn[wdst[j]] = wreg[j];
+                for (int j = 0; j < WF; ++j)
+                    if (wown[j]) wn[wdst_at(j)] = wreg[j];
             }
             __syncthreads();
         }
+        if constexpr (SPLIT) {
+            f32x4* hand = reinterpret_cast<f32x4*>(smem) + item * (RT * NT * 64) + lane;
+            if (half) {
+#pragma unroll
+                for (int m = 0; m < RT; ++m)
+#pragma unroll
+                    for (int n = 0; n < NT; ++n) hand[(m * NT + n) * 64] = acc[m][n];
+            }
+            __syncthreads();
+            if (!half) {
+#pragma unroll
+                for (int m = 0; m < RT; ++m)
+#pragma unroll
+                    for (int n = 0; n < NT; ++n) acc[m][n] += hand[(m * NT + n) * 64];
+            }
+            if (rd + 1 < rounds) __syncthreads();
+        }
+        int elane = lane;
+        if constexpr (SPLIT) asm volatile("" : "+v"(elane));
+        const int r16 = elane & 15, kq = elane >> 4;
         const int b = bs * 16 + r16;
 #pragma unroll
         for (int m = 0; m < RT; ++m) {
             const int v = v0 + m;
-            if (!live || v >= p.R || b >= p.B) continue;
+            if (!live || v >= p.R || b >= p.B || half) continue;
             const bool zero = v == p.zero_row;
 #pragma unroll
             for (int n = 0; n < NT; ++n) {
@@ -876,10 +933,10 @@
     return p3_resident_ok(S, Cg, Nout) || p3s_shape_ok(S, Cg, Nout);
 }
 
-template <int RT, bool BWD, int NP, int NT = P3S_NT>
+template <int RT, bool BWD, int NP, int NT = P3S_NT, bool SPLIT = false>
 int launch_p3s(P3Params& p, hipStream_t st) {
-    auto kern = conv_p3s_kernel<RT, BWD, NP, NT>;
-    constexpr int WAVES = 16 / RT;
+    auto kern = conv_p3s_kernel<RT, BWD, NP, NT, SPLIT>;
+    constexpr int ITEMS = 16 / RT, WAVES = ITEMS * (SPLIT ? 2 : 1);
     const size_t smem = (size_t)2 * P3S_KC * NT * 3072;
     static bool attr_set = false;
     if (!attr_set) {
@@ -895,22 +952,23 @@
     const long tiles = (long)p.n_vg * (p.B / 16);
     SH_REQUIRE(tiles < (1L << 30), SH_ERR_UNSUPPORTED, "conv_p3s: %ld work items", tiles);
     p.n_tiles = (int)tiles;
-    long groups = (tiles + WAVES - 1) / WAVES;
+    long groups = (tiles + ITEMS - 1) / ITEMS;
     const long cap = (long)p3_num_cus() / p.nsplit;
     if (groups > cap) groups = cap;
     if (groups < 8) groups = 8;
     groups = (groups + 7) / 8 * 8;
     const int grid = (int)groups * p.nsplit;
-    ShProfScope ps(st, "conv_p3s_kernel<%d, %s, %d, %d>|R=%d B=%d K=%d N=%d grid=%dx%d f32=%d", RT, BWD ? "true" : "false", NP, NT, p.R, p.B,
-                   p.S * p.Cg, p.Nout, grid, WAVES * 64, p.y ? 1 : 0);
+    ShProfScope ps(st, "conv_p3s_kernel<%d, %s, %d, %d%s>|R=%d B=%d K=%d N=%d grid=%dx%d f32=%d", RT, BWD ? "true" : "false", NP, NT,
+                   SPLIT ? ", true" : "", p.R, p.B, p.S * p.Cg, p.Nout, grid, WAVES * 64, p.y ? 1 : 0);
     SH_LAUNCH_PS(ps, kern, dim3(grid), dim3(WAVES * 64), smem, st, p);
     SH_CHECK_LAUNCH("conv_p3s");
     g_p3_launches.fetch_add(1, std::memory_order_relaxed);
     return SH_OK;
 }
 template <bool BWD, int NP>
-int dispatch_p3s(P3Params& p, hipStream_t st) {
+int dispatch_p3s(P3Params& p, hipStream_t st, bool split) {
     static const int rt = sh_env_int("SH_P3S_RT", 2, 1, 2);
+    if (split) return p.nt_tot == 2 ? launch_p3s<2, BWD, NP, 2, true>(p, st) : launch_p3s<2, BWD, NP, P3S_NT, true>(p, st);
     if (p.nt_tot == 2) return launch_p3s<2, BWD, NP, 2>(p, st);
     return rt == 2 ? launch_p3s<2, BWD, NP>(p, st) : launch_p3s<1, BWD, NP>(p, st);
 }
@@ -1039,7 +1097,7 @@
 }
 
 template <bool BWD>
-int dispatch_p3(P3Params& p, hipStream_t st) {
+int dispatch_p3(P3Params& p, hipStream_t st, bool split = false) {
     SH_REQUIRE(p3_shape_ok(p.B, p.S, p.Cg, p.Nout), SH_ERR_UNSUPPORTED,
                "conv_p3: B=%d S=%d gathered channels=%d output channels=%d is outside the three-plane kernels (sh_spiral_conv_p3_ok)",
                p.B, p.S, p.Cg, p.Nout);
@@ -1061,8 +1119,9 @@
     if (!p3_resident_ok(p.S, p.Cg, p.Nout)) {
         p.nks = p3_nks(p.S, p.Cg, p.Nout);
         SH_REQUIRE(!p.xf, SH_ERR_UNSUPPORTED, "conv_p3: the weight-streaming form takes imaged rows only (sh_spiral_conv_p3_kind() == 2)");
-        return np == 9 ? dispatch_p3s<BWD, 9>(p, st) : dispatch_p3s<BWD, 6>(p, st);
-    }
+        return np == 9 ? dispatch_p3s<BWD, 9>(p, st, split) : dispatch_p3s<BWD, 6>(p, st, split);
+    }
+    SH_REQUIRE(!split, SH_ERR_UNSUPPORTED, "conv_p3: the split-item form belongs to the weight-streaming kernels (sh_spiral_conv_p3_kind() == 2)");
     if constexpr (BWD) {
         if (p.xf) {
             SH_REQUIRE(np == 6, SH_ERR_UNSUPPORTED, "conv_p3: fp32 rows are built for the six-product form (SH_P3_NP=6)");
@@ -1141,8 +1200,22 @@
     return p3_resident_ok(S, Cg, Nout) ? 1 : 2;
 }
 
+int sh_spiral_conv_p3s_split_pays(int B, int R, int S, int Cg, int Nout, int backward) {
+    static const int on = sh_env_int("SH_P3S_SPLIT", 1, 0, 2);
+    if (!(on == 2 || (on == 1 && backward)) || R <= 0 || !p3_shape_ok(B, S, Cg, Nout) || p3_resident_ok(S, Cg, Nout)) return 0;
+    const int nt_tot = sh_frag_geom(S, Cg, Nout).nt_tot;
+    const long items = (long)sh_cdiv(R, 2) * (B / 16) * (nt_tot == 2 ? 1 : nt_tot / P3S_NT);
+    return items < 2L * 8 * p3_num_cus() ? 1 : 0;
+}
+
 int sh_spiral_conv_fwd_p3(const void* xp, const int32_t* table, const void* wfrag3, const float* bias, float* y, int64_t y_sv,
                           int64_t y_sb, void* yp, int B, int R, int S, int Cin, int Cout, int act, int zero_row, sh_stream_t stream) {
+    return sh_spiral_conv_fwd_p3_form(xp, table, wfrag3, bias, y, y_sv, y_sb, yp, B, R, S, Cin, Cout, act, zero_row, 0, stream);
+}
+
+int sh_spiral_conv_fwd_p3_form(const void* xp, const int32_t* table, const void* wfrag3, const float* bias, float* y, int64_t y_sv,
+                               int64_t y_sb, void* yp, int B, int R, int S, int Cin, int Cout, int act, int zero_row, int split,
+                               sh_stream_t stream) {
     SH_REQUIRE(xp && table && wfrag3, SH_ERR_INVALID_ARG, "sh_spiral_conv_fwd_p3: null pointer");
     SH_REQUIRE(B > 0 && R > 0 && S > 0 && Cin > 0 && Cout > 0, SH_ERR_INVALID_ARG, "sh_spiral_conv_fwd_p3: non-positive size");
     SH_REQUIRE(act >= SH_ACT_IDENTITY && act <= SH_ACT_TANH, SH_ERR_INVALID_ARG, "sh_spiral_conv_fwd_p3: unknown activation %d", act);
@@ -1150,13 +1223,21 @@
     p.xp = static_cast<const char*>(xp); p.table = table; p.wfrag = static_cast<const u32x4*>(wfrag3); p.bias = bias;
     p.y = y; p.y_sv = y_sv; p.y_sb = y_sb; p.yp = static_cast<char*>(yp);
     p.B = B; p.R = R; p.S = S; p.Cg = Cin; p.Nout = Cout; p.act = act; p.zero_row = zero_row; p.skip_row = -1; p.n_img = 0x7fffffff;
-    return dispatch_p3<false>(p, static_cast<hipStream_t>(stream));
+    return dispatch_p3<false>(p, static_cast<hipStream_t>(stream), split != 0);
 }
 
 int sh_spiral_conv_bwd_data_p3(const void* dprep, int dpre_zero_row, const float* dpre_f32, int64_t dp_sv, int64_t dp_sb, int n_image_rows,
                                const int32_t* table_t, const void* wfrag3_t, float* dx, int64_t dx_sv, int64_t dx_sb, void* dxp,
                                const float* yprev, int64_t yp_sv, int64_t yp_sb, const void* yprev_planes, int act_prev, int zero_row, int B,
                                int n_in, int S, int Cin, int Cout, sh_stream_t stream) {
+    return sh_spiral_conv_bwd_data_p3_form(dprep, dpre_zero_row, dpre_f32, dp_sv, dp_sb, n_image_rows, table_t, wfrag3_t, dx, dx_sv, dx_sb, dxp, yprev,
+                                           yp_sv, yp_sb, yprev_planes, act_prev, zero_row, B, n_in, S, Cin, Cout, 0, stream);
+}
+
+int sh_spiral_conv_bwd_data_p3_form(const void* dprep, int dpre_zero_row, const float* dpre_f32, int64_t dp_sv, int64_t dp_sb, int n_image_rows,
+                                    const int32_t* table_t, const void* wfrag3_t, float* dx, int64_t dx_sv, int64_t dx_sb, void* dxp,
+                                    const float* yprev, int64_t yp_sv, int64_t yp_sb, const void* yprev_planes, int act_prev, int zero_row,
+                                    int B, int n_in, int S, int Cin, int Cout, int split, sh_stream_t stream) {
     SH_REQUIRE(dprep && table_t && wfrag3_t, SH_ERR_INVALID_ARG, "sh_spiral_conv_bwd_data_p3: null pointer");
     SH_REQUIRE(B > 0 && n_in > 0 && S > 0 && Cin > 0 && Cout > 0, SH_ERR_INVALID_ARG, "sh_spiral_conv_bwd_data_p3: non-positive size");
     SH_REQUIRE(act_prev >= SH_ACT_IDENTITY && act_prev <= SH_ACT_TANH, SH_ERR_INVALID_ARG, "sh_spiral_conv_bwd_data_p3: unknown activation");
@@ -1179,7 +1260,7 @@
                    "sh_spiral_conv_bwd_data_p3: the fp32 gradient must be 16-byte aligned with strides %% 4 == 0");
         p.xf = dpre_f32; p.xf_sv = dp_sv; p.xf_sb = dp_sb; p.n_img = n_image_rows;
     }
-    return dispatch_p3<true>(p, static_cast<hipStream_t>(stream));
+    return dispatch_p3<true>(p, static_cast<hipStream_t>(stream), split != 0);
 }
 
 int sh_spiral_conv_p3_rag_ok(int B, int S, int Cg, int Nout, int rag_L) {
diff --git a/semantichuman_amd/csrc/stack_exec.hip b/semantichuman_amd/csrc/stack_exec.hip
--- a/semantichuman_amd/csrc/stack_exec.hip
+++ b/semantichuman_amd/csrc/stack_exec.hip
@@ -99,15 +99,35 @@
     return s;
 }
 
+}
+extern "C" {
+__attribute__((weak)) int sh_spiral_conv_p3s_split_pays(int B, int R, int S, int Cg, int Nout, int backward);
+__attribute__((weak)) int sh_spiral_conv_fwd_p3_form(const void* xp, const int32_t* table, const void* wfrag3, const float* bias, float* y, int64_t y_sv,
+                                                     int64_t y_sb, void* yp, int B, int R, int S, int Cin, int Cout, int act, int zero_row, int split,
+                                                     sh_stream_t stream);
+__attribute__((weak)) int sh_spiral_conv_bwd_data_p3_form(const void* dprep, int dpre_zero_row, const float* dpre_f32, int64_t dp_sv, int64_t dp_sb,
+                                                          int n_image_rows, const int32_t* table_t, const void* wfrag3_t, float* dx, int64_t dx_sv,
+                                                          int64_t dx_sb, void* dxp, const float* yprev, int64_t yp_sv, int64_t yp_sb,
+                                                          const void* yprev_planes, int act_prev, int zero_row, int B, int n_in, int S, int Cin,
+                                                          int Cout, int split, sh_stream_t stream);
+}
+namespace {
+inline bool split_pays(int B, int R, int S, int Cg, int Nout, bool backward) {
+    return sh_spiral_conv_p3s_split_pays && sh_spiral_conv_fwd_p3_form && sh_spiral_conv_bwd_data_p3_form &&
+           sh_spiral_conv_p3s_split_pays(B, R, S, Cg, Nout, backward ? 1 : 0);
+}
+
 enum { BD_F32 = 0, BD_TABLE, BD_RAG, BD_GRP };
 struct Forms {
     bool f_p3;
     bool f_grp;
+    bool f_split;
     bool f_img;
     bool f_img_only;
     bool b_gimg;
     bool b_thin;
     int b_data;
+    bool b_split;
     bool b_ride;
     bool b_presum_img;
     bool b_p3w;
@@ -131,6 +151,7 @@
         f[i].f_p3 = !(s.cout <= 16 && B > sw.n16_maxb) && sh_spiral_conv_p3_ok(B, s.S, s.cin, s.cout);
         f[i].f_grp = f[i].f_p3 && sw.grouped && s.fg_rows && s.fg_pos && s.fg_out && s.fg_n > 0 &&
                      sh_spiral_conv_p3_grp_ok(B, s.S, s.cin, s.cout, s.fg_L) && sh_spiral_conv_p3_grp_pays(B, s.fg_n);
+        f[i].f_split = f[i].f_p3 && !f[i].f_grp && split_pays(B, s.R, s.S, s.cin, s.cout, false);
     }
     for (int i = 0; i + 1 < n; ++i) {
         const int c = consumer_conv(n, st, i);
@@ -147,6 +168,7 @@
                              sh_spiral_conv_p3_grp_ok(B, s.S, s.cout, s.cin, s.bg_L) && sh_spiral_conv_p3_grp_pays(B, s.bg_n);
             const bool rag = sw.ragged && s.rag_rows && s.rag_pos && sh_spiral_conv_p3_rag_ok(B, s.S, s.cout, s.cin, s.rag_L);
             q.b_data = grp ? BD_GRP : rag ? BD_RAG : BD_TABLE;
+            q.b_split = q.b_data == BD_TABLE && split_pays(B, s.n_in, s.S, s.cout, s.cin, true);
             q.b_presum_img = sw.presum_img == 1 ||
                              !(sh_spiral_conv_p3_kind(B, s.S, s.cout, s.cin) == 1 && (sw.presum_img == 0 || 2 * (s.n1 + s.n2) >= s.R));
         }
@@ -216,6 +238,9 @@
             if (q.f_grp)
                 rc = sh_spiral_conv_p3_grp(planes[i - 1], s.fg_rows, s.fg_pos, s.fg_out, s.fg_n, s.fg_L, wfrag3[i], bias, y, ol.sv, ol.sb, img, nullptr,
                                            0, 0, nullptr, s.act, s.zero_row, 0, B, s.R, s.S, s.cin, s.cout, stream);
+            else if (q.f_split)
+                rc = sh_spiral_conv_fwd_p3_form(planes[i - 1], s.table, wfrag3[i], bias, y, ol.sv, ol.sb, img, B, s.R, s.S, s.cin, s.cout, s.act,
+                                                s.zero_row, 1, stream);
             else if (q.f_p3)
                 rc = sh_spiral_conv_fwd_p3(planes[i - 1], s.table, wfrag3[i], bias, y, ol.sv, ol.sb, img, B, s.R, s.S, s.cin, s.cout, s.act,
                                            s.zero_row, stream);
@@ -390,6 +415,10 @@
                     else if (bd == BD_RAG)
                         rc = sh_spiral_conv_bwd_data_p3_rag(cur_img, s.rag_rows, s.rag_pos, s.rag_L, wfrag3_t[i], gi_f, gl.sv, gl.sb, gi_img, yprev,
                                                             yl.sv, yl.sb, yimg, act_prev, zero_prev, B, s.n_in, s.S, s.cin, s.cout, stream);
+                    else if (q.b_split)
+                        rc = sh_spiral_conv_bwd_data_p3_form(cur_img, s.zero_row, q.b_presum_img ? nullptr : cur, cl.sv, cl.sb, s.R, s.table_t,
+                                                             wfrag3_t[i], gi_f, gl.sv, gl.sb, gi_img, yprev, yl.sv, yl.sb, yimg, act_prev, zero_prev, B,
+                                                             s.n_in, s.S, s.cin, s.cout, 1, stream);
                     else
                         rc = sh_spiral_conv_bwd_data_p3(cur_img, s.zero_row, q.b_presum_img ? nullptr : cur, cl.sv, cl.sb, s.R, s.table_t, wfrag3_t[i],
                                                         gi_f, gl.sv, gl.sb, gi_img, yprev, yl.sv, yl.sb, yimg, act_prev, zero_prev, B, s.n_in, s.S,
```

New measurement: 47370, median of 2. Within noise of the previous version (-0.1%).
